# tranqkhue/bugcar_image_segmentation

Measured on AMD Instinct MI355X. Metric: frames/sec ENet 640x480 segmentation -> BEV occupancy grid (synthetic), whole job, higher is better.
Workload: dtype fp32; 1 GPU; config3/5: ENet 640x480 batch 64 per GPU, preprocess + forward + argmax/LUT + fused BEV warp/occgrid (1000x1000 BEV -> 200x200 cells); global_batch=64, per_gpu_batch=64, height=480, width=640, parallelism=frame-sharded dp1, streams_per_gpu=1, hip_graph=True, ranks=1, devices=1, backend=none (one process)

## Files before the change

### bugcar_image_segmentation_amd/_native.py

```python
from __future__ import annotations

import ctypes
import os
import threading
from pathlib import Path

import torch

_PKG = Path(__file__).resolve().parent
LIB_PATH = Path(os.environ.get("BUGSEG_LIB", _PKG / "libbugseg.so"))

OK, EINVAL, ENOMEM, EHIP, EFORMAT, ESTATE = 0, -1, -2, -3, -4, -5
FP32, BF16, F16 = 0, 1, 2
OUT_LOGITS_F32, OUT_CLASS15_U8, OUT_CLASS3_U8, OUT_BINARY_U8 = 0, 1, 2, 3
PRE_ENGINE, PRE_NCHW_F64, PRE_NCHW_F32, PRE_BGR_U8 = 0, 1, 2, 3

EXPORTED = ("bugseg_version", "bugseg_create", "bugseg_destroy", "bugseg_load_weights", "bugseg_num_classes",
            "bugseg_input_bytes", "bugseg_preprocess", "bugseg_nchw_to_input", "bugseg_enet_forward",
            "bugseg_enet_forward_bgr", "bugseg_enet_forward_bgr_ops",
            "bugseg_bev_occgrid", "bugseg_bev_workspace_bytes", "bugseg_bev_occgrid_ws", "bugseg_plan_info", "bugseg_plan_op", "bugseg_plan_launch_op",
            "bugseg_last_error",
            "bugseg_dl_create", "bugseg_dl_destroy", "bugseg_dl_load_weights", "bugseg_dl_set_plan",
            "bugseg_dl_forward", "bugseg_dl_launch_op", "bugseg_dl_read_buffer", "bugseg_dl_last_error",
            "bugseg_debug_parse_pack", "bugseg_debug_polar_tables", "bugseg_debug_ctx_info", "bugseg_debug_tile_walk", "bugseg_debug_set_spans", "bugseg_debug_pool_indices",
            "bugseg_dl_debug_check_plan")
DL_OP_FIELDS = 32


class BevParams(ctypes.Structure):
    _fields_ = [("M", ctypes.c_double * 9), ("in_rows", ctypes.c_int), ("in_cols", ctypes.c_int),
                ("warp_w", ctypes.c_int), ("warp_h", ctypes.c_int), ("occ_w_px", ctypes.c_int),
                ("occ_h_px", ctypes.c_int), ("occ_w", ctypes.c_int), ("occ_h", ctypes.c_int),
                ("left_x", ctypes.c_int), ("top_y", ctypes.c_int), ("ros_layout", ctypes.c_int),
                ("variant", ctypes.c_int), ("laserscan", ctypes.c_int)]


class BugsegError(RuntimeError):
    def __init__(self, code: int, msg: str):
        super().__init__(f"bugseg error {code}: {msg}")
        self.code = code


_lib = None
_lock = threading.Lock()


def load_library(path: Path | str | None = None) -> ctypes.CDLL:
    global _lib
    with _lock:
        if _lib is not None:
            return _lib
        p = Path(path) if path else LIB_PATH
        if not p.exists():
            raise FileNotFoundError(f"{p} not found: build it with `python -m bugcar_image_segmentation_amd.build` "
                                    "(or __graft_entry__.build())")
        lib = ctypes.CDLL(str(p))
        vp, i, sz, cp = ctypes.c_void_p, ctypes.c_int, ctypes.c_size_t, ctypes.c_char_p
        proto = {
            "bugseg_version": (i, []),
            "bugseg_create": (i, [i, i, ctypes.POINTER(vp)]),
            "bugseg_destroy": (i, [vp]),
            "bugseg_load_weights": (i, [vp, vp, sz]),
            "bugseg_num_classes": (i, [vp]),
            "bugseg_input_bytes": (sz, [vp, i, i, i]),
            "bugseg_preprocess": (i, [vp, vp, i, i, i, i, i, i, vp, vp]),
            "bugseg_nchw_to_input": (i, [vp, vp, i, i, i, i, vp, vp]),
            "bugseg_enet_forward": (i, [vp, vp, i, i, i, i, vp, vp]),
            "bugseg_enet_forward_bgr": (i, [vp, vp, i, i, i, i, vp, vp]),
            "bugseg_enet_forward_bgr_ops": (i, [vp, vp, i, i, i, i, vp, i, i, vp]),
            "bugseg_bev_occgrid": (i, [vp, vp, i, ctypes.POINTER(BevParams), vp, vp]),
            "bugseg_bev_workspace_bytes": (sz, [ctypes.POINTER(BevParams), i]),
            "bugseg_bev_occgrid_ws": (i, [vp, vp, i, ctypes.POINTER(BevParams), vp, vp, sz, vp]),
            "bugseg_plan_info": (i, [vp, i, i, i, i, i, ctypes.POINTER(i), ctypes.POINTER(ctypes.c_double),
                                     ctypes.POINTER(ctypes.c_double), ctypes.POINTER(ctypes.c_double)]),
            "bugseg_plan_op": (i, [vp, i, i, i, i, cp, i, ctypes.POINTER(ctypes.c_double),
                                   ctypes.POINTER(ctypes.c_double), ctypes.POINTER(ctypes.c_double)]),
            "bugseg_plan_launch_op": (i, [vp, i, i, i, i, vp]),
            "bugseg_last_error": (cp, [vp]),
            "bugseg_dl_create": (i, [i, i, ctypes.POINTER(vp)]),
            "bugseg_dl_destroy": (i, [vp]),
            "bugseg_dl_load_weights": (i, [vp, vp, sz]),
            "bugseg_dl_set_plan": (i, [vp, vp, i, vp, i, i, i, i]),
            "bugseg_dl_forward": (i, [vp, vp, i, i, i, vp, vp]),
            "bugseg_dl_launch_op": (i, [vp, i, vp]),
            "bugseg_dl_read_buffer": (i, [vp, i, vp, sz, vp]),
            "bugseg_dl_last_error": (cp, [vp]),
            "bugseg_debug_parse_pack": (i, [vp, sz, i, ctypes.POINTER(i)]),
            "bugseg_debug_polar_tables": (i, [i, i, i, vp, sz, vp, sz, ctypes.POINTER(i), ctypes.POINTER(i)]),
            "bugseg_debug_ctx_info": (i, [vp, i, i]),
            "bugseg_debug_tile_walk": (i, [i, i, i, vp, sz, vp]),
            "bugseg_debug_set_spans": (i, [vp, vp, i]),
            "bugseg_debug_pool_indices": (i, [vp, i, i, i, i, vp, sz, ctypes.POINTER(ctypes.c_int), vp]),
            "bugseg_dl_debug_check_plan": (i, [vp, i, vp, i, i, i, i, i, sz]),
        }
        for name, (res, args) in proto.items():
            f = getattr(lib, name)
            f.restype = res
            f.argtypes = args
        _lib = lib
        return lib


def check(code: int, ctx=None) -> None:
    if code != OK:
        lib = load_library()
        msg = lib.bugseg_last_error(ctx).decode(errors="replace")
        if code == EINVAL:
            raise ValueError(msg)
        raise BugsegError(code, msg)


def tile_walk(ntiles: int, grid: int, rev: int) -> list[list[int]]:
    lib = load_library()
    per_max = (ntiles + 7) // 8
    seq = (ctypes.c_int32 * (grid * per_max))()
    count = (ctypes.c_int32 * grid)()
    per = lib.bugseg_debug_tile_walk(ntiles, grid, rev, seq, len(seq), count)
    if per < 0:
        check(per)
    return [list(seq[b * per:b * per + count[b]]) for b in range(grid)]


def require_gpu() -> None:
    if not torch.cuda.is_available():
        raise RuntimeError("bugseg needs a HIP GPU (MI355X / gfx950); none is visible — there is no CPU fallback")


def stream_handle(stream: torch.cuda.Stream | None = None) -> int:
    s = stream if stream is not None else torch.cuda.current_stream()
    return int(s.cuda_stream)


class Context:

    def __init__(self, device: int | None = None, precision: int = FP32):
        require_gpu()
        self.lib = load_library()
        self.device = torch.cuda.current_device() if device is None else int(device)
        self.precision = precision
        h = ctypes.c_void_p()
        check(self.lib.bugseg_create(self.device, precision, ctypes.byref(h)))
        self.h = h

    def close(self) -> None:
        if getattr(self, "h", None) and self.h.value:
            self.lib.bugseg_destroy(self.h)
            self.h = ctypes.c_void_p()

    def __del__(self):
        try:
            self.close()
        except Exception:
            pass

    def load_weights(self, blob: bytes) -> None:
        buf = ctypes.create_string_buffer(blob, len(blob))
        check(self.lib.bugseg_load_weights(self.h, buf, len(blob)), self.h)

    @property
    def num_classes(self) -> int:
        return int(self.lib.bugseg_num_classes(self.h))

    def input_bytes(self, B: int, H: int, W: int) -> int:
        return int(self.lib.bugseg_input_bytes(self.h, B, H, W))

    def preprocess(self, bgr, B, H0, W0, H, W, layout, out, stream=None):
        check(self.lib.bugseg_preprocess(self.h, bgr.data_ptr(), B, H0, W0, H, W, layout, out.data_ptr(),
                                         stream_handle(stream)), self.h)

    def nchw_to_input(self, x, B, H, W, out, stream=None):
        check(self.lib.bugseg_nchw_to_input(self.h, x.data_ptr(), int(x.dtype == torch.float64), B, H, W,
                                            out.data_ptr(), stream_handle(stream)), self.h)

    def forward(self, x, B, H, W, out_kind, out, stream=None):
        check(self.lib.bugseg_enet_forward(self.h, x.data_ptr(), B, H, W, out_kind, out.data_ptr(),
                                           stream_handle(stream)), self.h)

    def forward_bgr(self, bgr, B, H, W, out_kind, out, stream=None):
        check(self.lib.bugseg_enet_forward_bgr(self.h, bgr.data_ptr(), B, H, W, out_kind, out.data_ptr(),
                                               stream_handle(stream)), self.h)

    def forward_bgr_ops(self, bgr, B, H, W, out_kind, out, first_op, last_op, stream=None):
        check(self.lib.bugseg_enet_forward_bgr_ops(self.h, bgr.data_ptr(), B, H, W, out_kind, out.data_ptr(),
                                                   first_op, last_op, stream_handle(stream)), self.h)

    def bev(self, seg, B, params: BevParams, out, stream=None):
        st = stream if stream is not None else torch.cuda.current_stream(seg.device)
        nws = int(self.lib.bugseg_bev_workspace_bytes(ctypes.byref(params), B))
        ws = None
        if nws:
            with torch.cuda.stream(st):
                ws = torch.empty(nws, dtype=torch.uint8, device=seg.device)
        check(self.lib.bugseg_bev_occgrid_ws(self.h, seg.data_ptr(), B, ctypes.byref(params), out.data_ptr(),
                                             0 if ws is None else ws.data_ptr(), nws, stream_handle(st)), self.h)

    def plan_info(self, B, H, W, out_kind, bgr_input=False):
        n = ctypes.c_int()
        lb = ctypes.c_double()
        pb = ctypes.c_double()
        fl = ctypes.c_double()
        check(self.lib.bugseg_plan_info(self.h, B, H, W, out_kind, int(bool(bgr_input)), ctypes.byref(n),
                                        ctypes.byref(lb), ctypes.byref(pb), ctypes.byref(fl)), self.h)
        return n.value, lb.value, pb.value, fl.value

    def plan_op(self, B, H, W, op):
        buf = ctypes.create_string_buffer(64)
        lb, pb, fl = ctypes.c_double(), ctypes.c_double(), ctypes.c_double()
        check(self.lib.bugseg_plan_op(self.h, B, H, W, op, buf, 64, ctypes.byref(lb), ctypes.byref(pb),
                                      ctypes.byref(fl)), self.h)
        return buf.value.decode(), lb.value, pb.value, fl.value

    def launch_op(self, B, H, W, op, stream=None):
        check(self.lib.bugseg_plan_launch_op(self.h, B, H, W, op, ctypes.c_void_p(stream_handle(stream))), self.h)

    def debug_info(self, what: int, arg: int = 0) -> int:
        return int(self.lib.bugseg_debug_ctx_info(self.h, what, arg))

    def set_spans(self, spans=None):
        if spans is None:
            check(self.lib.bugseg_debug_set_spans(self.h, ctypes.c_void_p(0), 0), self.h)
            return
        if not spans.is_cuda or spans.dtype != torch.int64 or not spans.is_contiguous() or spans.numel() % 512:
            raise ValueError("spans must be a contiguous CUDA int64 tensor of 512 words per op")
        check(self.lib.bugseg_debug_set_spans(self.h, ctypes.c_void_p(spans.data_ptr()), spans.numel() // 512), self.h)

    def pool_indices(self, B: int, H: int, W: int, block: int, shape: tuple, stream=None) -> torch.Tensor:
        out = torch.empty((B,) + tuple(shape), dtype=torch.uint8, device=torch.device("cuda", self.device))
        cs = ctypes.c_int(0)
        check(self.lib.bugseg_debug_pool_indices(self.h, B, H, W, block, ctypes.c_void_p(out.data_ptr()), out.numel(),
                                                 ctypes.byref(cs), ctypes.c_void_p(stream_handle(stream))), self.h)
        if cs.value != shape[-1]:
            raise ValueError(f"index tensor has channel stride {cs.value}, not {shape[-1]}")
        return out


_shared: dict[int, Context] = {}


def shared_context(device: int | None = None) -> Context:
    require_gpu()
    d = torch.cuda.current_device() if device is None else int(device)
    with _lock:
        c = _shared.get(d)
    if c is None:
        c = Context(d, FP32)
        with _lock:
            _shared.setdefault(d, c)
            c = _shared[d]
    return c


class DeepLabContext:

    def __init__(self, device: int | None = None, precision: int = BF16):
        require_gpu()
        self.lib = load_library()
        self.device = torch.cuda.current_device() if device is None else int(device)
        self.precision = precision
        h = ctypes.c_void_p()
        self._check(self.lib.bugseg_dl_create(self.device, precision, ctypes.byref(h)), None)
        self.h = h

    def _check(self, code, h):
        if code != OK:
            msg = self.lib.bugseg_dl_last_error(h).decode(errors="replace")
            if code == EINVAL:
                raise ValueError(msg)
# ... 36 lines not shown
```

### bugcar_image_segmentation_amd/csrc/bev_kernels.hip

```cpp
#include <cstdlib>
#include <type_traits>

#include "bugseg_internal.h"

namespace bugseg {

struct WarpTap { int sx, sy, ax, ay; bool x0, x1, y0, y1; };
__device__ __forceinline__ WarpTap warp_tap(const BevArgs &a, int x, int y) {
#pragma clang fp contract(off)
    const double *M = a.Mi;
    const int xb = (x / a.bw0) * a.bw0, x1 = x - xb;
    const double X0 = M[0] * (double)xb + M[1] * (double)y + M[2];
    const double Y0 = M[3] * (double)xb + M[4] * (double)y + M[5];
    const double W0 = M[6] * (double)xb + M[7] * (double)y + M[8];
    double W = W0 + M[6] * (double)x1;
    W = W != 0.0 ? 32.0 / W : 0.0;
    double fX = (X0 + M[0] * (double)x1) * W;
    double fY = (Y0 + M[3] * (double)x1) * W;
    fX = fmin(fmax(fX, -2147483648.0), 2147483647.0);
    fY = fmin(fmax(fY, -2147483648.0), 2147483647.0);
    const int X = (int)__builtin_rint(fX), Y = (int)__builtin_rint(fY);
    int sx = X >> 5, sy = Y >> 5;
    sx = sx < -32768 ? -32768 : (sx > 32767 ? 32767 : sx);
    sy = sy < -32768 ? -32768 : (sy > 32767 ? 32767 : sy);
// ... 250 lines not shown
    auto fetch = [&](int b) {
        const auto r = frame_rsrc(b);
#pragma unroll
        for (int i = 0; i < BEV_PF; ++i) pf[i] = __builtin_bit_cast(uint4, __builtin_amdgcn_raw_buffer_load_b128(r, (int)goff[i], 0, 0));
    };
    const int b0 = grp * fg;
    if (lds) {
        fetch(b0);
        for (int i = tid; i < 2 * bw + 16; i += 256) box[zpad + i] = 0;
    }
    const uint32_t inner = 0x739C0u;
    int tx = 0, ty = 0;
    cell_pixel(a, cx, cy, tx, ty);
    uint32_t wins[9];
#pragma unroll
    for (int qy = -1; qy <= 1; ++qy)
#pragma unroll
        for (int qx = -1; qx <= 1; ++qx) {
            const bool inside = (unsigned)(tx + qx) < (unsigned)a.occ_w_px && (unsigned)(ty + qy) < (unsigned)a.occ_h_px;
            const int sh = qy * 5 + qx;
            wins[(qy + 1) * 3 + qx + 1] = inside ? (sh >= 0 ? inner << sh : inner >> -sh) : 0xffffffffu;
        }
    for (int fi = 0; fi < fg; ++fi) {
        const int b = b0 + fi;
        if (b >= a.B) break;
        uint32_t msk = 0;
        int v = 0;
        if (lds) {
            __syncthreads();
#pragma unroll
            for (int i = 0; i < BEV_PF; ++i)
                if (tid + 256 * i < nch)
                    *reinterpret_cast<uint4 *>(box + 16 * (tid + 256 * i)) =
                        goff[i] == 0x80000000u ? make_uint4(0u, 0u, 0u, 0u)
                                               : make_uint4(inc4(pf[i].x), inc4(pf[i].y), inc4(pf[i].z), inc4(pf[i].w));
            __syncthreads();
            if (fi + 1 < fg && b + 1 < a.B) fetch(b + 1);
#pragma unroll 5
            for (int k = 0; k < BEV_WIN; ++k) {
                const uint32_t e = ek[k];
                const uint8_t *p = box + (e & 0xffffu);
                const uint32_t l0 = p[0], l1 = p[1], l2 = p[bw], l3 = p[bw + 1];
                const uint32_t ax = (e >> 16) & 31u, ay = (e >> 21) & 31u;
                const uint32_t wx = 32u + ax * 65535u, wy = 32u + ay * 65535u;
                const uint32_t top = dot2(l0 | l1 << 16, wx, 0u), bot = dot2(l2 | l3 << 16, wx, 0u);
                const int t = (int)(dot2(top | bot << 16, wy, 512u) >> 10);
                if (k == 0) v = t;
                msk |= (uint32_t)occupied(a, t) << BEV_ORDER[k];
            }
        } else {
            const auto seg = frame_rsrc(b);
#pragma unroll 1
            for (int k = 0; k < BEV_WIN; ++k) {
                const uint2 e = cell_ok ? ent(k) : make_uint2(0u, TAB_OUT);
                const int t = tab_value(seg, a.in_cols, e);
                if (k == 0) v = t;
                msk |= (uint32_t)occupied(a, t) << BEV_ORDER[k];
            }
        }
        if (!cell_ok) continue;
        msk |= outm;
        if (occupied(a, v)) {
            bool opened = false;
#pragma unroll
            for (int q = 0; q < 9; ++q) opened |= (msk & wins[q]) == wins[q];
            if (!opened) v = 2;
        }
        bev_emit(a, b, rem, cx, cy, cells, v);
    }
}

constexpr int BEV_BAND_CAP = 16384, BEV_BAND_PF = BEV_BAND_CAP / 16 / 256;
static_assert(BEV_BOXREC == 1 + BEV_BAND, "band record: header + one box per row part");
#ifndef BEV_MINP
#define BEV_MINP 1
#endif
constexpr int BEV_WL = 448;
static_assert(BEV_WL <= 2 * 256, "a thread takes at most two work-list records");

__global__ void __launch_bounds__(256) bev_bandbox_kernel(const BevArgs a, int4 *bbox) {
    __shared__ int red[BEV_BAND][4];
    __shared__ int4 pbox[BEV_BAND];
    __shared__ int np_rpp[2];
    const long cells = (long)a.occ_h * a.occ_w;
    const int band = blockIdx.x, r0 = band * BEV_BAND, r1 = min(a.occ_h, r0 + BEV_BAND);
    const int nr = r1 - r0, n = nr * a.occ_w;
    int ylo[BEV_BAND], yhi[BEV_BAND], xlo[BEV_BAND], xhi[BEV_BAND];
#pragma unroll
    for (int k = 0; k < BEV_BAND; ++k) { ylo[k] = xlo[k] = 1 << 30; yhi[k] = xhi[k] = -(1 << 30); }
    for (int i = threadIdx.x; i < n * BEV_WIN; i += 256) {
        const int c = i / BEV_WIN, k = i - c * BEV_WIN, ri = c / a.occ_w;
        const long rem = (long)r0 * a.occ_w + c;
        const uint2 e = slot_half(a.wtab[(long)(k >> 1) * cells + rem], k & 1);
        const uint32_t v = (e.y >> 10) & 15;
        const int sy = tap_sy(e), sx = tap_sx(e);
        int y_lo = 1 << 30, y_hi = -(1 << 30), x_lo = 1 << 30, x_hi = -(1 << 30);
        if (v & 3) { y_lo = min(y_lo, sy); y_hi = max(y_hi, sy); }
        if (v & 12) { y_lo = min(y_lo, sy + 1); y_hi = max(y_hi, sy + 1); }
        if (v & 5) { x_lo = min(x_lo, sx); x_hi = max(x_hi, sx); }
        if (v & 10) { x_lo = min(x_lo, sx + 1); x_hi = max(x_hi, sx + 1); }
#pragma unroll
        for (int q = 0; q < BEV_BAND; ++q)
            if (q == ri) { ylo[q] = min(ylo[q], y_lo); yhi[q] = max(yhi[q], y_hi); xlo[q] = min(xlo[q], x_lo); xhi[q] = max(xhi[q], x_hi); }
    }
    if (threadIdx.x < 4 * BEV_BAND) red[threadIdx.x >> 2][threadIdx.x & 3] = threadIdx.x & 1 ? -(1 << 30) : (1 << 30);
    __syncthreads();
#pragma unroll
    for (int q = 0; q < BEV_BAND; ++q) {
        atomicMin(&red[q][0], ylo[q]); atomicMax(&red[q][1], yhi[q]); atomicMin(&red[q][2], xlo[q]); atomicMax(&red[q][3], xhi[q]);
    }
    __syncthreads();
    if (threadIdx.x == 0) {
        auto boxof = [&](int q0, int q1) {
            int yl = 1 << 30, yh = -(1 << 30), xl = 1 << 30, xh = -(1 << 30);
            for (int q = q0; q < q1 && q < nr; ++q) {
                yl = min(yl, red[q][0]); yh = max(yh, red[q][1]); xl = min(xl, red[q][2]); xh = max(xh, red[q][3]);
            }
            int4 bx = make_int4(0, 0, 0, 16);
            if (yh >= yl) {
                const int y0 = yl - 1, bh = yh - yl + 3;
                const int xa = (xl - 1) & ~15, bw = ((xh + 17) & ~15) - xa;
                bx = make_int4(y0, xa, (long)bh * bw + 2 * bw + 16 <= BEV_BAND_CAP ? bh : -1, bw);
            }
            return bx;
        };
        int P = BEV_MINP;
        for (; P < BEV_BAND; P *= 2) {
            bool fit = true;
            for (int k = 0; k < P; ++k) fit = fit && boxof(k * (BEV_BAND / P), (k + 1) * (BEV_BAND / P)).z >= 0;
            if (fit) break;
        }
        int rpp = BEV_BAND / P;
        for (int k = 0; k < BEV_BAND; ++k) pbox[k] = k < P ? boxof(k * rpp, (k + 1) * rpp) : make_int4(0, 0, 0, 16);
        bool fit = true;
        for (int k = 0; k < P; ++k) fit = fit && pbox[k].z >= 0;
        if (!fit) {
            P = 1; rpp = BEV_BAND;
            pbox[0] = boxof(0, BEV_BAND);
            pbox[0].z = -1;
        }
        np_rpp[0] = P; np_rpp[1] = rpp;
        bbox[(size_t)band * BEV_BOXREC] = make_int4(P, rpp, 0, 0);
        for (int k = 0; k < BEV_BAND; ++k) bbox[(size_t)band * BEV_BOXREC + 1 + k] = pbox[k];
    }
    __syncthreads();
    const int rpp = np_rpp[1];
    uint32_t *ctab = reinterpret_cast<uint32_t *>(reinterpret_cast<unsigned char *>(a.wtab) + bev_ctab_offset(a.occ_w, a.occ_h));
    for (int i = threadIdx.x; i < n * BEV_SLOTS; i += 256) {
        const int c = i / BEV_SLOTS, q = i - c * BEV_SLOTS;
        const int4 bx = pbox[(c / a.occ_w) / rpp];
        if (bx.z < 0) continue;
        const long rem = (long)r0 * a.occ_w + c;
        uint4 *sp = a.wtab + (long)q * cells + rem;
        uint4 sv = *sp;
        auto put = [&](uint32_t x, uint32_t &y) {
            const uint2 e = make_uint2(x, y);
            const bool any = ((y >> 10) & 15) != 0;
            const int o = any ? (tap_sy(e) - bx.x) * bx.w + (tap_sx(e) - bx.y) : bx.z * bx.w;
            y = (y & 0x7fffu) | (uint32_t)o << 15;
        };
        put(sv.x, sv.y);
        put(sv.z, sv.w);
        *sp = sv;
        ctab[(long)(2 * q) * cells + rem] = sv.y;
        if (2 * q + 1 < BEV_WIN) ctab[(long)(2 * q + 1) * cells + rem] = sv.w;
    }
    __syncthreads();
    uint32_t *omask = ctab + (size_t)BEV_WIN * cells;
    for (int c = threadIdx.x; c < n; c += 256) {
        if (pbox[(c / a.occ_w) / rpp].z < 0) continue;
        const long rem = (long)r0 * a.occ_w + c;
        uint32_t m = 0;
        for (int k = 0; k < BEV_WIN; ++k)
            m |= (uint32_t)((ctab[(long)k * cells + rem] & TAB_OUT) != 0) << BEV_ORDER[k];
        omask[rem] = m;
    }
}

#ifndef BEV_ABL
#define BEV_ABL 0
#endif
__device__ __forceinline__ int bev_value_lds(const uint8_t *box, int bw, uint32_t ey) {
    const uint8_t *p = box + (ey >> 15);
    const uint32_t l0 = p[0], l1 = p[1], l2 = p[bw], l3 = p[bw + 1];
    const uint32_t ax = ey & 31u, ay = (ey >> 5) & 31u;
    const uint32_t wx = 32u + ax * 65535u, wy = 32u + ay * 65535u;
    const uint32_t top = dot2(l0 | l1 << 16, wx, 0u), bot = dot2(l2 | l3 << 16, wx, 0u);
    return (int)(dot2(top | bot << 16, wy, 512u) >> 10);
}
constexpr uint32_t BEV_INNER = 0x739C0u;
__device__ __forceinline__ bool bev_cell_pass1(const BevArgs &a, const uint8_t *box, int bw, const uint32_t (&e9)[9],
                                               uint32_t outm, int &v, uint32_t &m, uint32_t &cand) {
    int t9[9];
#pragma unroll
    for (int i = 0; i < 9; ++i) t9[i] = bev_value_lds(box, bw, e9[i]);
    v = t9[0];
    m = outm;
#pragma unroll
    for (int i = 0; i < 9; ++i) m |= (uint32_t)occupied(a, t9[i]) << BEV_ORDER[i];
    cand = 0;
    if (!(occupied(a, v) && (m & BEV_INNER) != BEV_INNER)) return true;
#pragma unroll
    for (int qi = 0; qi < 9; ++qi) {
        if (qi == 4) continue;
        const int qx = qi % 3 - 1, qy = qi / 3 - 1, sh = qy * 5 + qx;
        const uint32_t win = sh >= 0 ? BEV_INNER << sh : BEV_INNER >> -sh, wi = win & BEV_INNER;
        cand |= (!((outm >> B5(qx, qy)) & 1u) && (m & wi) == wi) ? 1u << qi : 0u;
    }
    if (cand == 0) { v = 2; return true; }
    return false;
}
__device__ __forceinline__ int bev_cell_pass2(const BevArgs &a, const uint8_t *box, int bw, int v, uint32_t m,
                                              uint32_t cand, uint32_t outm, const uint32_t *ring, long cells) {
    if constexpr (BEV_ABL & 1) return v;
    uint32_t rneed = 0;
#pragma unroll
    for (int qi = 0; qi < 9; ++qi) {
        const int qx = qi % 3 - 1, qy = qi / 3 - 1, sh = qy * 5 + qx;
        const uint32_t win = sh >= 0 ? BEV_INNER << sh : BEV_INNER >> -sh;
        rneed |= ((cand >> qi) & 1u) ? win & ~BEV_INNER & ~outm : 0u;
    }
    uint32_t er[BEV_WIN - 9];
#pragma unroll
    for (int k = 0; k < BEV_WIN - 9; ++k) er[k] = ring[(long)k * cells];
#pragma unroll
// ... 389 lines not shown
```

### bugcar_image_segmentation_amd/csrc/bneck_kernels.hip

```cpp
#include <algorithm>
#include <cstdlib>

#include <type_traits>

#include "bugseg_internal.h"
#ifndef BUGSEG_OUT_AUX
#define BUGSEG_OUT_AUX -1
#endif
#include "cls_common.h"

namespace bugseg {

#ifdef BUGSEG_STAMPS
__device__ unsigned long long *bugseg_stamps;
#define STAMP(k) do { if (tid == 0 && bugseg_stamps) bugseg_stamps[(size_t)tile * 8 + (k)] = __builtin_amdgcn_s_memtime(); } while (0)
#define STAMP_WG() do { if (tid == 0 && bugseg_stamps) bugseg_stamps[(size_t)tile * 8 + 7] = blockIdx.x; } while (0)
#define STAMP_ENTRY(k) do { if (threadIdx.x == 0 && bugseg_stamps) bugseg_stamps[(1u << 19) + 2u * blockIdx.x + (k)] = __builtin_amdgcn_s_memrealtime(); } while (0)
#else
#define STAMP_ENTRY(k) do {} while (0)
#define STAMP(k) do {} while (0)
#define STAMP_WG() do {} while (0)
#endif

__device__ __forceinline__ void vm_wait_upto(int n) {
// ... 368 lines not shown
    bool cshort[2] = {false, false};
    if constexpr (CLS) {
        const T *cw = reinterpret_cast<const T *>(a.cw);
        for (int q = tid; q < 512; q += NT) {
            const int bs = q >> 6, ln = q & 63;
            const T *src = cw + (size_t)cls_prow(bs >> 2, ln & 31) * 64 + (bs & 3) * 16 + 8 * (ln >> 5);
            if constexpr (sizeof(T) == 4) {
                cwl[q] = reinterpret_cast<const uint4 *>(src)[0];
                cwl[512 + q] = reinterpret_cast<const uint4 *>(src)[1];
            } else {
                cwl[q] = *reinterpret_cast<const uint4 *>(src);
            }
        }
        if (tid < 64) cbl[tid] = (tid & 15) < a.ncls ? a.cbias[tid] : -INFINITY;
        lut64 = cls_lut64(a.lut);
#pragma unroll
        for (int b = 0; b < 2; ++b) {
            CRaw w2_, w3_;
            const T *r = cw + (size_t)cls_prow(b, lane & 31) * 64 + 8 * (lane >> 5);
            ld8(w2_, r + 32);
            ld8(w3_, r + 48);
            cshort[b] = __ballot(nonzero(w2_) || nonzero(w3_)) == 0;
        }
    }
    const auto rxb = mkbuf(DN ? a.xin : a.x, DN ? a.xin_bytes : a.x_bytes);
    const auto rob = mkbuf(a.out, a.x_bytes);
    const auto rpb = mkbuf(a.pool, a.pool_bytes);
    const auto rib = mkbuf(a.idx_out, a.idx_bytes);
    auto act = [&](float4 v, const float *s) { return prelu4m(v, ld4f(s)); };
    const int dt = a.dt;
    constexpr bool tr = TR && !ASYM;

    constexpr bool F32 = sizeof(T) == 4;
    BneckRange rg0;
    if constexpr (F32 && SCL) rg0 = bneck_range<ASYM>(a.rg, rng_reduce(rlane));
    bool scl = rg0.scl;
    float xm = rg0.xm, b1m = rg0.b1m, o1m = rg0.o1m, b2m = rg0.b2m, o2m = rg0.o2m, b2bm = rg0.b2bm, o2bm = rg0.o2bm;
    float b3m = rg0.b3m, o3m = rg0.o3m;
    const int rs1 = rg0.rs1, re2b = rg0.re2b;
    float amo = 0.f;
    auto proj_mfma = [&](f32x4 (&acc)[NR1], const Raw (&xs)[KS1]) {
#pragma unroll
        for (int r = 0; r < NR1; ++r) acc[r] = bias4(cb1 + r * 16 + kq * 4);
        if constexpr (F32 && SCL) {
#pragma unroll
            for (int r = 0; r < NR1; ++r) acc[r] = mul4(acc[r], b1m);
#pragma unroll
            for (int s = 0; s < KS1; ++s) {
                const RawF xq = scale8(reinterpret_cast<const RawF &>(xs[s]), xm);
#pragma unroll
                for (int r = 0; r < NR1; ++r) {
                    WRaw wf;
                    ldw(wf, w1 + (r * 16 + col) * K1S + s * 32);
                    mma(acc[r], wf, xq);
                }
            }
#pragma unroll
            for (int r = 0; r < NR1; ++r) acc[r] = mul4(acc[r], o1m);
        } else {
#pragma unroll
            for (int s = 0; s < KS1; ++s)
#pragma unroll
                for (int r = 0; r < NR1; ++r) {
                    WRaw wf;
                    ldw(wf, w1 + (r * 16 + col) * K1S + s * 32);
                    mma(acc[r], wf, xs[s]);
                }
        }
    };

    const int G = gridDim.x, grp = blockIdx.x & 7, slot = blockIdx.x >> 3, nslots = G >> 3;
    const int CH = tile_walk_ch(a.ntiles);
    constexpr bool WALK1 = sizeof(T) == 4 && C == 128;
    const int lim = tile_walk_lim(grp, CH, a.ntiles);
    const int wword = WALK1 ? tile_walk_base(grp, CH, a.ntiles, a.rev) : tile_walk_mirror(grp, CH, a.ntiles, a.rev);
    auto tile_geom = [&](int tile, int &n, int &oy0, int &ox0) {
        int t = tile;
        const int txi = t % a.tiles_x; t /= a.tiles_x;
        const int tyi = t % a.tiles_y; t /= a.tiles_y;
        const int ph = t % a.phases;
        n = t / a.phases;
        const int py = RD ? ph : ph / dt, px = RD ? 0 : ph - py * dt;
        oy0 = py + dt * tyi * (tr ? TW : TH) - (CLS ? tyi : 0);
        ox0 = RD ? 0 : px + dt * txi * (tr ? TH : TW) - (CLS ? txi : 0);
    };
    Raw kx[KEEP ? NF2 : 1][KS1];
    bool kok[KEEP ? NF2 : 1];
#ifndef BNECK_PREF
#define BNECK_PREF 0
#endif
    constexpr bool PREF = BNECK_PREF && KEEP && REG3 && !DN;
    bool pref = false;
    for (int it = slot; it < (WALK1 ? lim : CH); it += nslots) {
        int tile;
        if constexpr (WALK1) {
            tile = tile_walk_at(wword, it);
        } else {
            tile = grp * CH + it;
            if (tile >= a.ntiles) break;
            tile = tile_walk_flip(wword, tile);
        }
        int n, oy0, ox0;
        tile_geom(tile, n, oy0, ox0);
        float tmo = 0.f;
        const bool has_next = PREF && it + nslots < lim;
        const int ntile = !has_next ? -1 : WALK1 ? tile_walk_at(wword, it + nslots) : tile_walk_flip(wword, grp * CH + it + nslots);
        int nn = 0, noy0 = 0, nox0 = 0;
        if (has_next) tile_geom(ntile, nn, noy0, nox0);
        const int dtx = RD ? 1 : dt;
        const uint32_t xn = (uint32_t)(n * a.H * a.W) * (uint32_t)(C * sizeof(T));
        const uint32_t xin_n = (uint32_t)(n * 4 * a.H * a.W) * (uint32_t)(CI * sizeof(T));
        auto pix_off = [&](int f, int pi, int choff) -> uint32_t {
            const int i = (f * 16) / TW, j = (f * 16) % TW + pi;
            const int y = oy0 + dt * (tr ? j : i), x = ox0 + dtx * (tr ? i : j);
            const bool ok = y < a.H && x < a.W;
            uint32_t v = xn + ((__umul24((uint32_t)y, (uint32_t)a.W) + (uint32_t)x) * C + choff) * (uint32_t)sizeof(T);
            asm volatile("" : "+v"(v));
            return ok ? v : OOB;
        };
        auto pix_base = [&](int f, int pi) -> uint32_t { return pix_off(f, pi, 0); };
        const auto rrb = DN ? rpb : rxb;
        const uint32_t pn = (uint32_t)(n * a.H * a.W) * (uint32_t)(CI * sizeof(T));
        auto res_off = [&](int f, int pi, int ch) -> uint32_t {
            if constexpr (!DN) {
                return pix_off(f, pi, ch);
            } else {
                const int i = (f * 16) / TW, j = (f * 16) % TW + pi;
                const int y = oy0 + dt * i, x = ox0 + dtx * j;
                const bool ok = y < a.H && x < a.W && ch < CI;
                uint32_t v = pn + ((__umul24((uint32_t)y, (uint32_t)a.W) + (uint32_t)x) * CI + ch) * (uint32_t)sizeof(T);
                asm volatile("" : "+v"(v));
                return ok ? v : OOB;
            }
        };
        auto pool_store = [&](const Raw (&xs)[KS1], bool interior, int y, int x, uint4 (&pk)[NPK * PKW]) {
            if constexpr (DN) {
                if (__ballot(interior) == 0) return;
                auto elems = [&](const Raw &r, float (&e)[8]) {
                    if constexpr (sizeof(T) == 2) {
                        const float4 lo = unpack4<T>((u32x2_t){r.v.x, r.v.y}), hi = unpack4<T>((u32x2_t){r.v.z, r.v.w});
                        e[0] = lo.x; e[1] = lo.y; e[2] = lo.z; e[3] = lo.w; e[4] = hi.x; e[5] = hi.y; e[6] = hi.z; e[7] = hi.w;
                    } else {
                        const RawF &f = reinterpret_cast<const RawF &>(r);
                        e[0] = f.a.x; e[1] = f.a.y; e[2] = f.a.z; e[3] = f.a.w; e[4] = f.b.x; e[5] = f.b.y; e[6] = f.b.z; e[7] = f.b.w;
                    }
                };
                const uint32_t pix = (uint32_t)((n * a.H + y) * a.W + x);
                auto emit = [&](int cc, const float (&bv)[8], const int (&bp)[8], bool wr, int kslot, bool kval) {
                    uint32_t pw[8 * sizeof(T) / 4];
                    if constexpr (sizeof(T) == 2) {
                        const u32x2_t lo = pack4<T>(make_float4(bv[0], bv[1], bv[2], bv[3]));
                        const u32x2_t hi = pack4<T>(make_float4(bv[4], bv[5], bv[6], bv[7]));
                        pw[0] = lo.x; pw[1] = lo.y; pw[2] = hi.x; pw[3] = hi.y;
                    } else {
#pragma unroll
                        for (int i = 0; i < 8; ++i) pw[i] = __float_as_uint(bv[i]);
                    }
                    uint32_t lo = 0, hi = 0;
#pragma unroll
                    for (int i = 0; i < 4; ++i) {
                        lo |= (uint32_t)(bp[i] & 3) << (8 * i);
                        hi |= (uint32_t)(bp[4 + i] & 3) << (8 * i);
                    }
                    if constexpr (DKEEP) {
                        pk[kslot * PKW] = kval ? make_uint4(pw[0], pw[1], pw[2], pw[3]) : make_uint4(0u, 0u, 0u, 0u);
                        if constexpr (PKW == 2)
// ... 986 lines not shown
```

### bugcar_image_segmentation_amd/csrc/bugseg_internal.h

```cpp
#pragma once
#include <hip/hip_runtime.h>
#include <stdint.h>
#include <stddef.h>

namespace bugseg {

enum Epi {
    EPI_PLAIN = 0,
    EPI_RESADD = 1,
    EPI_RESPOOL = 2,
    EPI_RESUNPOOL = 3,
    EPI_INIT = 4,
    EPI_SHUFFLE = 5,
    EPI_CLASSES = 6,
    EPI_INIT_BGR = 7,
    EPI_COUNT = 8
};

enum Prec { PREC_F32 = 0, PREC_BF16 = 1, PREC_F16 = 2 };
inline constexpr int prec_es(int prec) { return prec == PREC_F32 ? 4 : 2; }

constexpr int RNG_SLOTS = 256;
struct RangeArgs {
    const float *amax_in;
    float *amax_out;
    float amax_static;
    int sw[4];
    float n[3], c[3];
    int off;
};
int range_weight_exp(double m);
hipError_t launch_amax(const float *x, size_t n, float *slots, hipStream_t s);

struct ConvArgs {
    const void *in;
    int B, Hin, Win, CinS;
    int Hg, Wg;
    int stride;
    int M;
    int Ksteps, Kpad, Npad;
    const void *w;
    const int *gtab;
    const float *bias, *slope1, *slope2, *pscale;
    int cconv, cpool, pool_k;
    const void *res;
    int resH, resW, resC, resCS;
    const uint8_t *idx_in;
    uint8_t *idx_out;
    int idxCS;
    void *out;
    int Hout, Wout, outC;
    int coutP;
    int ncls;
    const uint8_t *lut;
    int lut_kind;
    uint8_t *cls_out;
    float *logits_out;
    const double *nlut;
    float naff[6];
    int naff_on;
    int pool_scan;
    int ntiles;
    int rev;
    int stg_elems;
    int stage_ok;
    uint32_t mHWg, mWg; int sHWg, sWg;
    uint32_t in_bytes, out_bytes, res_bytes, idx_bytes;
    int cpr_sh;
    int slopes_le1;
    RangeArgs rg;
    unsigned long long *span;
};

__host__ __device__ inline int tile_walk_ch(int ntiles) { return (ntiles + 7) >> 3; }
__host__ __device__ inline int tile_walk_lim(int grp, int CH, int ntiles) {
    const int rest = ntiles - grp * CH;
    return rest < CH ? rest : CH;
}
__host__ __device__ inline int tile_walk_base(int grp, int CH, int ntiles, int rev) {
    return rev ? ~(grp * CH + tile_walk_lim(grp, CH, ntiles)) : grp * CH;
}
__host__ __device__ inline int tile_walk_at(int base, int it) {
    const int s = base >> 31;
    return (base ^ s) + (it ^ s);
}
__host__ __device__ inline int tile_walk(int grp, int it, int CH, int ntiles, int rev) {
    if (it >= tile_walk_lim(grp, CH, ntiles)) return -1;
    return tile_walk_at(tile_walk_base(grp, CH, ntiles, rev), it);
}
__host__ __device__ inline int tile_walk_mirror(int grp, int CH, int ntiles, int rev) {
    return rev ? 2 * grp * CH + tile_walk_lim(grp, CH, ntiles) - 1 : -1;
}
__host__ __device__ inline int tile_walk_flip(int mirror, int t) { return mirror < 0 ? t : mirror - t; }

void fastdiv(uint32_t d, uint32_t &m, int &s);

int device_cus();
int occupancy_per_cu(const void *f, int threads, size_t lds);
hipError_t allow_dynamic_lds(const void *f);

hipError_t launch_conv(int prec, int nr, int epi, const ConvArgs &a, hipStream_t s);
int conv_tile_pixels(int nr);
size_t conv_lds_bytes(int prec, const ConvArgs &a);

bool cls_supported(const ConvArgs &a);
hipError_t launch_cls(int prec, const ConvArgs &a, hipStream_t s);

hipError_t launch_init(int prec, bool bgr, const ConvArgs &a, hipStream_t s);
constexpr int NAFF_R = 64;
hipError_t launch_naff_search(int prec, const double *nlut, const float *base, uint8_t *ok, hipStream_t s);

struct BneckArgs {
    const void *x;
    void *out;
    int B, H, W;
    int dt, phases;
    int tr;
    int tiles_x, tiles_y, ntiles;
    int rev;
    const void *w1, *w2, *w2b, *w3;
    const float *b1, *s1, *b2, *s2, *b2b, *s2b, *b3, *s3, *s_out;
    uint32_t x_bytes;
    int slopes_le1;
    const void *xin;
    void *pool;
    uint8_t *idx_out;
    int idxCS;
    uint32_t xin_bytes, pool_bytes, idx_bytes;
    RangeArgs rg;
    unsigned long long *span;
    const void *cw;
    const float *cbias;
    uint8_t *cls_out;
    uint32_t cls_bytes;
    const uint8_t *lut;
    int lut_kind, ncls, csw;
};
int bneck_variants(int C);
bool bneck_keeps_c64(int prec, int v);
void bneck_shape(int C, int v, int &th, int &tw, int &nw, int *rd = nullptr);
size_t bneck_lds_bytes(int prec, int C, bool asym, int v, int cin = 0, bool cls = false);
int bneck_slots_per_cu(int prec, int C, bool asym, int v, bool tr, int cin = 0);
hipError_t launch_bneck(int prec, int C, bool asym, int v, const BneckArgs &a, hipStream_t s, int cin = 0);
hipError_t launch_bneck_cls(int prec, const BneckArgs &a, hipStream_t s);
constexpr int BNECK2_V = 5;
size_t bneck2_lds_bytes();
int bneck2_slots_per_cu();
hipError_t launch_bneck2(const BneckArgs &a, hipStream_t s);

struct UpArgs {
    const void *x;
    const uint8_t *idx;
    void *out;
    int M, h, w, idxCS;
    int rev;
    uint32_t mHW, mW; int sHW, sW;
    const void *w1, *w2, *w3;
    const float *b1, *s1, *b2, *s2, *b3, *s3, *s_out;
    uint32_t x_bytes, idx_bytes, out_bytes;
    int slopes_le1;
    RangeArgs rg;
    unsigned long long *span;
};
bool up_supported(int cin, int it, int cout);
hipError_t launch_up(int prec, int cin, int it, int cout, const UpArgs &a, hipStream_t s);

struct PreArgs {
    const uint8_t *bgr;
    int B, H0, W0, H, W;
    int mode;
    const int *xofs;
    const short *xa;
    const int *yofs;
    const short *yb;
    int vec_end;
    const double *lut;
    int out_layout;
    int prec;
    void *out;
};
hipError_t launch_preprocess(const PreArgs &a, hipStream_t s);

struct NchwArgs {
    const void *x; int is_f64; int B, H, W; int prec; void *out;
};
hipError_t launch_nchw_to_input(const NchwArgs &a, hipStream_t s);

struct BevArgs {
    const uint8_t *seg;
    int B, in_rows, in_cols;
    double Mi[9];
    int bw0;
    int warp_w, warp_h, occ_w_px, occ_h_px, occ_w, occ_h, left_x, top_y;
    double ifx, ify;
    int ros_layout;
    int variant;
    int8_t *out;
    int laserscan;
    uint8_t *cells;
    const int32_t *fmap;
    const int32_t *imap;
    int pw, ph;
    int32_t *rmin;
    int hit;
    uint4 *wtab;
    int nitems;
};
hipError_t launch_bev(const BevArgs &a, hipStream_t s);
hipError_t launch_bev_table(const BevArgs &a, hipStream_t s);
size_t bev_table_bytes(int occ_w, int occ_h);

constexpr int BEV_BAND = 4;
__host__ __device__ inline int bev_bands(int occ_h) { return (occ_h + BEV_BAND - 1) / BEV_BAND; }
constexpr int BEV_WIN = 25, BEV_SLOTS = 13;
constexpr int BEV_BOXREC = 5;
__host__ __device__ inline size_t bev_records_offset(int occ_w, int occ_h) { return (size_t)occ_w * occ_h * BEV_SLOTS * 16; }
__host__ __device__ inline size_t bev_ctab_offset(int occ_w, int occ_h) {
    return (bev_records_offset(occ_w, occ_h) + (size_t)bev_bands(occ_h) * BEV_BOXREC * 16 + 255) & ~(size_t)255;
}
__host__ __device__ inline size_t bev_items_offset(int occ_w, int occ_h) {
    return (bev_ctab_offset(occ_w, occ_h) + (size_t)occ_w * occ_h * (BEV_WIN + 1) * 4 + 255) & ~(size_t)255;
}

}
```

### bugcar_image_segmentation_amd/csrc/bugseg_runtime.cpp

```cpp
#include <cmath>
#include <cstdio>
#include <cstring>
#include <string>
#include <vector>
#include <algorithm>
#include <cstdlib>
#include <mutex>

#include "bugseg_internal.h"
#include "../../include/bugseg.h"

using namespace bugseg;

namespace {
std::mutex g_occ_mu;
struct OccKey { int dev; const void *f; int threads; size_t lds; int val; };
std::vector<OccKey> g_occ;
int current_device() {
    int d = 0;
    return hipGetDevice(&d) == hipSuccess ? d : 0;
}
}
int bugseg::device_cus() {
    const int dev = current_device();
// ... 6 lines not shown
    return n;
}
int bugseg::occupancy_per_cu(const void *f, int threads, size_t lds) {
    const int dev = current_device();
    std::lock_guard<std::mutex> lk(g_occ_mu);
    for (const OccKey &k : g_occ)
        if (k.dev == dev && k.f == f && k.threads == threads && k.lds == lds) return k.val;
    int n = 0;
    if (hipOccupancyMaxActiveBlocksPerMultiprocessor(&n, f, threads, lds) != hipSuccess || n < 0) n = 0;
    g_occ.push_back({dev, f, threads, lds, n});
    return n;
}
hipError_t bugseg::allow_dynamic_lds(const void *f) {
    const int dev = current_device();
    std::lock_guard<std::mutex> lk(g_occ_mu);
    for (const OccKey &k : g_occ)
        if (k.dev == dev && k.f == f && k.threads == -1) return hipSuccess;
    hipError_t e = hipFuncSetAttribute(f, hipFuncAttributeMaxDynamicSharedMemorySize, 160 * 1024);
    if (e == hipSuccess) g_occ.push_back({dev, f, -1, 0, 1});
    return e;
}

int bugseg::range_weight_exp(double m) {
    if (!(m > 0) || !std::isfinite(m)) return 0;
    int e = 0;
    (void)std::frexp(m, &e);
    const int l = e - 1;
    if (l >= -2 && l < 15) return 0;
    return std::max(-40, std::min(40, 14 - l));
}

namespace {

thread_local std::string g_thread_err;

struct UnitDesc {
    int kind = 0, cout = 0, cin = 0, kh = 0, kw = 0, stride = 1, pad_h = 0, pad_w = 0, dil_h = 1, dil_w = 1, out_pad = 0;
    float eps = 0.f;
    std::vector<float> w, b, gamma, beta, mean, var, slope;
};

struct BlockDesc {
    int type = 0;
    int attrs[8] = {0};
    std::vector<UnitDesc> units;
    std::vector<std::vector<float>> extra;
};

enum { BT_INITIAL = 1, BT_REGULAR = 2, BT_DOWN = 3, BT_UP = 4, BT_FULLCONV = 5 };

struct Packed {
    int Npad = 0, Kpad = 0, Ksteps = 0, nr = 0;
    int CinS = 0;
    int stride = 1;
    int cout = 0;
    int coutP = 0;
    int phases = 1;
    double macs_per_px = 0;
    size_t o_w = 0, o_gtab = 0, o_bias = 0, o_s1 = 0, o_s2 = 0, o_ps = 0;
    int sw = 0;
    std::vector<float> rabs, rbias, rslope;
};

struct Op {
    int kind = 0;
    ConvArgs a;
    int nr = 0, epi = 0;
    BneckArgs bn;
    UpArgs up;
    int up_cin = 0, up_it = 0, up_cout = 0;
    int bn_c = 0, bn_var = 0, bn_cin = 0;
    bool bn_asym = false;
    double bytes = 0, flops = 0;
    double layer_bytes = -1;
    int launches = 1;
    int pos = 0;
    Op() {
        std::memset(&a, 0, sizeof(a));
        std::memset(&bn, 0, sizeof(bn));
        std::memset(&up, 0, sizeof(up));
    }
};

struct Plan {
    int B = 0, H = 0, W = 0;
    std::vector<Op> ops;
    float *words = nullptr;
    size_t words_bytes = 0;
    void *arena = nullptr;
    size_t arena_bytes = 0;
    bool pinned = false;
    std::vector<unsigned char *> idx;
    std::vector<size_t> idx_bytes;
    bool cls_ok = false, cls_on = false;
    int tile_order = 0;
};

#ifndef BUGSEG_TILE_ORDER_DEFAULT
#define BUGSEG_TILE_ORDER_DEFAULT 1
#endif

inline int round_up(int v, int m) { return (v + m - 1) / m * m; }
inline int pow2_nr(int npad) {
    int nr = npad / 16;
    int p = 1;
    while (p < nr) p <<= 1;
    return p;
}

}

struct bugseg_ctx {
    int device = 0;
    int prec = PREC_F32;
    float naff[6] = {};
    bool naff_on = false;
    float norm_amax = 0.f;
    bool range_off = false;
    unsigned long long *spans = nullptr;
    int spans_ops = 0;
    std::string err;
    bool loaded = false;
    int ncls = 0;
    std::vector<BlockDesc> blocks;
    std::vector<Packed> packed;
    std::vector<std::vector<int>> block_convs;
    std::vector<unsigned char> host_w;
    void *dev_w = nullptr;
    void *dev_luts = nullptr;
    Plan plan;
    struct PreTab { int key[4] = {0, 0, 0, 0}; void *tab = nullptr; bool pinned = false; };
    std::vector<PreTab> pre_tabs;
    hipStream_t setup = nullptr;
    struct PolarTab { int key[3] = {0, 0, -1}; int pw = 0, ph = 0; void *tab = nullptr; bool pinned = false; };
    std::vector<PolarTab> polar_tabs;
    struct LsScratch { void *stream = nullptr; void *p = nullptr; size_t bytes = 0; uint64_t used = 0; bool pinned = false; };
    std::vector<LsScratch> ls_scratch;
    uint64_t use_clock = 0;
    struct BevTab { std::vector<unsigned char> key; uint4 *tab = nullptr; bool pinned = false; int nitems = 0; };
    std::vector<BevTab> bev_tabs;
    std::vector<void *> graveyard;
};

namespace {

int fail(bugseg_ctx *c, int code, const std::string &m) {
    if (c) c->err = m;
    else g_thread_err = m;
    return code;
}

bool stream_capturing(void *stream) {
    hipStreamCaptureStatus st = hipStreamCaptureStatusNone;
    if (hipStreamIsCapturing((hipStream_t)stream, &st) != hipSuccess) return true;
    return st != hipStreamCaptureStatusNone;
}

struct RelaxCapture {
    hipStreamCaptureMode m = hipStreamCaptureModeRelaxed;
    RelaxCapture() { (void)hipThreadExchangeStreamCaptureMode(&m); }
    ~RelaxCapture() { (void)hipThreadExchangeStreamCaptureMode(&m); }
};

hipStream_t setup_stream(bugseg_ctx *c) {
    if (!c->setup && hipStreamCreateWithFlags(&c->setup, hipStreamNonBlocking) != hipSuccess) c->setup = nullptr;
    return c->setup;
}

void retire(bugseg_ctx *c, void *p, bool capturing) {
    if (!p) return;
    if (capturing) { c->graveyard.push_back(p); return; }
    (void)hipDeviceSynchronize();
    (void)hipFree(p);
}

struct DeviceGuard {
    int prev = -1;
    explicit DeviceGuard(int dev) {
        if (hipGetDevice(&prev) != hipSuccess) prev = -1;
        if (prev != dev) (void)hipSetDevice(dev);
    }
    ~DeviceGuard() {
        int cur = -1;
        if (prev >= 0 && hipGetDevice(&cur) == hipSuccess && cur != prev) (void)hipSetDevice(prev);
    }
};

struct Reader {
    const unsigned char *p, *end;
    bool ok = true;
    template <typename T> T get() {
        T v{};
        if (p + sizeof(T) > end) { ok = false; return v; }
        std::memcpy(&v, p, sizeof(T));
        p += sizeof(T);
        return v;
    }
    std::vector<float> tensor() {
        uint32_t n = get<uint32_t>();
        std::vector<float> v;
        if (!ok || (size_t)(end - p) / 4 < (size_t)n) { ok = false; return v; }
        v.resize(n);
        if (n) std::memcpy(v.data(), p, (size_t)n * 4);
        p += (size_t)n * 4;
        return v;
    }
};

bool parse_blob(const void *blob, size_t bytes, std::vector<BlockDesc> &out, int &ncls, std::string &why) {
    Reader r{(const unsigned char *)blob, (const unsigned char *)blob + bytes};
    char magic[4];
    for (int i = 0; i < 4; ++i) magic[i] = r.get<char>();
    if (!r.ok || std::memcmp(magic, "BSG1", 4) != 0) { why = "bad magic (expected BSG1)"; return false; }
    uint32_t ver = r.get<uint32_t>(), nb = r.get<uint32_t>(), nc = r.get<uint32_t>();
    if (!r.ok || ver != 1) { why = "unsupported blob version"; return false; }
    if (nb == 0 || nb > 4096 || nc == 0 || nc > 16) { why = "bad block/class count"; return false; }
    ncls = (int)nc;
    for (uint32_t b = 0; b < nb; ++b) {
        BlockDesc bd;
        bd.type = (int)r.get<uint32_t>();
        for (int i = 0; i < 8; ++i) bd.attrs[i] = r.get<int32_t>();
        uint32_t nu = r.get<uint32_t>();
// ... 682 lines not shown
                        const Packed &p1 = P(0), &p2 = P(1), &p3 = P(nu - 1), &p2b = P(nu == 4 ? 2 : 1);
                        q.x = curp; q.out = dst; q.B = B; q.H = cur.H; q.W = cur.W;
                        q.dt = dd; q.phases = trd ? dd : dd * dd; q.tr = ttr;
                        q.tiles_y = ty; q.tiles_x = tx;
                        q.ntiles = B * q.phases * ty * tx;
                        q.w1 = dw + p1.o_w; q.b1 = (const float *)(dw + p1.o_bias); q.s1 = (const float *)(dw + p1.o_s1);
                        q.w2 = dw + p2.o_w; q.b2 = (const float *)(dw + p2.o_bias); q.s2 = (const float *)(dw + p2.o_s1);
                        q.w2b = dw + p2b.o_w; q.b2b = (const float *)(dw + p2b.o_bias); q.s2b = (const float *)(dw + p2b.o_s1);
                        q.w3 = dw + p3.o_w; q.b3 = (const float *)(dw + p3.o_bias); q.s3 = (const float *)(dw + p3.o_s1);
                        q.s_out = (const float *)(dw + p3.o_s2);
                        q.rg.amax_in = words_of(curp);
                        q.rg.off = ctx->range_off;
                        q.rg.sw[0] = p1.sw; q.rg.sw[1] = p2.sw; q.rg.sw[2] = p2b.sw; q.rg.sw[3] = p3.sw;
                        row_bound(p1, 0, p1.cout, q.rg.n[0], q.rg.c[0]);
                        row_bound(p2, 0, p2.cout, q.rg.n[1], q.rg.c[1]);
                        row_bound(p2b, 0, p2b.cout, q.rg.n[2], q.rg.c[2]);
                        q.rg.amax_out = take_words();
                        wrote(dst, q.rg.amax_out);
                        q.slopes_le1 = 1;
                        const std::pair<size_t, int> slopes[] = {{p1.o_s1, p1.Npad}, {p2.o_s1, p2.Npad}, {p2b.o_s1, p2b.Npad},
                                                                 {p3.o_s1, p3.Npad}, {p3.o_s2, p3.Npad}};
                        for (const auto &sv : slopes) {
                            const float *sl = (const float *)(ctx->host_w.data() + sv.first);
                            for (int c = 0; c < sv.second; ++c)
                                if (!(sl[c] <= 1.f)) q.slopes_le1 = 0;
                        }
                        double fl = 0, wb = 0, lb = 0;
                        const double px = (double)B * cur.H * cur.W;
                        for (int i = 0; i < nu; ++i) {
                            fl += 2.0 * P(i).macs_per_px * px;
                            wb += (double)P(i).Npad * P(i).Kpad * es;
                            lb += px * (cstore(b.units[i].cin) + cstore(b.units[i].cout)) * es;
                        }
                        op.flops = fl;
                        op.bytes = 2.0 * px * cur.C * es + wb;
                        op.layer_bytes = lb + px * cur.C * es + wb;
                        ops.push_back(op);
                    }
                    break;
                }
                for (int i = 0; i < nu; ++i) {
                    const UnitDesc &u = b.units[i];
                    const bool last = i + 1 == nu;
                    Shape so{s.H, s.W, cstore(u.cout)};
                    unsigned char *o = last ? dst : T[i % 3];
                    if (!last) szT = std::max(szT, tbytes(so));
                    else szX = std::max(szX, tbytes(so));
                    if (fill) {
                        Op op;
                        conv(P(i), last ? EPI_RESADD : EPI_PLAIN, src, s, so, o, so, op);
                        if (last) {
                            op.a.res = curp; op.a.resH = cur.H; op.a.resW = cur.W; op.a.resC = b.attrs[0]; op.a.resCS = cur.C;
                            op.bytes += (double)B * cur.H * cur.W * cur.C * es;
                        }
                        ops.push_back(op);
                    }
                    s = so;
                    src = o;
                }
                cur = s;
                break;
            }
            case BT_UP: {
                const int ref = b.attrs[2];
                Shape sm{cur.H, cur.W, cstore(P(0).cout)}, s1{cur.H, cur.W, cstore(P(1).cout)};
                Shape st{cur.H * 2, cur.W * 2, cstore(P(2).cout)}, so{cur.H * 2, cur.W * 2, cstore(P(3).cout)};
                szM = std::max(szM, tbytes(sm));
                szT = std::max({szT, tbytes(s1), tbytes(st)});
                szX = std::max(szX, tbytes(so));
                const int cin_b = b.attrs[0], cout_b = b.attrs[1], it_b = P(1).cout;
                const char *nf = std::getenv("BUGSEG_NO_FUSE");
                const bool fuse_up = ids.size() >= 5 && up_supported(cin_b, it_b, cout_b) && cur.C == cin_b &&
                                     so.C == cout_b && !(nf && *nf && *nf != '0');
                if (fuse_up) {
                    if (fill) {
                        Op op;
                        op.kind = 2;
                        op.up_cin = cin_b; op.up_it = it_b; op.up_cout = cout_b;
                        UpArgs &q = op.up;
                        const unsigned char *dw = (const unsigned char *)ctx->dev_w;
                        const Packed &p1 = P(4), &p2 = P(2), &p3 = P(3);
                        q.x = curp; q.idx = idx[ref]; q.out = dst;
                        q.M = B * cur.H * cur.W; q.h = cur.H; q.w = cur.W;
                        q.idxCS = cstore(ctx->blocks[ref].attrs[0]);
                        fastdiv((uint32_t)(cur.H * cur.W), q.mHW, q.sHW);
                        fastdiv((uint32_t)cur.W, q.mW, q.sW);
                        q.w1 = dw + p1.o_w; q.b1 = (const float *)(dw + p1.o_bias); q.s1 = (const float *)(dw + p1.o_s1);
                        q.w2 = dw + p2.o_w; q.b2 = (const float *)(dw + p2.o_bias); q.s2 = (const float *)(dw + p2.o_s1);
                        q.w3 = dw + p3.o_w; q.b3 = (const float *)(dw + p3.o_bias); q.s3 = (const float *)(dw + p3.o_s1);
                        q.s_out = (const float *)(dw + p3.o_s2);
                        q.rg.amax_in = words_of(curp);
                        q.rg.off = ctx->range_off;
                        q.rg.sw[0] = p1.sw; q.rg.sw[1] = p2.sw; q.rg.sw[2] = p3.sw;
                        row_bound(p1, cout_b, cout_b + it_b, q.rg.n[0], q.rg.c[0]);
                        row_bound(p2, 0, p2.Npad, q.rg.n[1], q.rg.c[1]);
                        q.rg.amax_out = take_words();
                        wrote(dst, q.rg.amax_out);
                        q.x_bytes = (uint32_t)std::min<size_t>((size_t)B * cur.H * cur.W * cur.C * es, 0x7fffffff);
                        q.idx_bytes = (uint32_t)std::min<size_t>((size_t)B * cur.H * cur.W * q.idxCS, 0x7fffffff);
                        q.out_bytes = (uint32_t)std::min<size_t>((size_t)B * so.H * so.W * so.C * es, 0x7fffffff);
                        q.slopes_le1 = 1;
                        const std::pair<size_t, int> sl[] = {{p1.o_s1, p1.Npad}, {p2.o_s1, p2.Npad}, {p3.o_s1, p3.Npad},
                                                             {p3.o_s2, p3.Npad}};
                        for (const auto &v : sl) {
                            const float *f = (const float *)(ctx->host_w.data() + v.first);
                            for (int c = 0; c < v.second; ++c)
                                if (!(f[c] <= 1.f)) q.slopes_le1 = 0;
                        }
                        const double px = (double)B * cur.H * cur.W;
                        double wb = 0, fl = 0;
                        for (int i = 0; i < 4; ++i) { wb += (double)P(i).Npad * P(i).Kpad * es; fl += 2.0 * P(i).macs_per_px * px; }
                        op.flops = fl;
                        op.bytes = px * cur.C * es + px * q.idxCS + 4.0 * px * so.C * es + wb;
                        op.layer_bytes = px * cur.C * es * 2 + px * (sm.C + s1.C) * es + px * s1.C * es + 4.0 * px * st.C * es * 2 +
                                         px * sm.C * es + px * q.idxCS + 4.0 * px * so.C * es + wb;
                        ops.push_back(op);
                    }
                    cur = so;
                    break;
                }
                const bool pair = ids.size() == 6;
                Shape sp{cur.H, cur.W, pair ? sm.C + s1.C : sm.C};
                szM = std::max(szM, tbytes(sp));
                if (fill && pair) {
                    Op om1, ot, o2;
                    conv(P(4), EPI_PLAIN, curp, cur, sp, Mb, sp, om1);
                    conv(P(5), EPI_SHUFFLE, Mb, sp, sp, T[1], st, ot);
                    ot.bytes -= (double)B * sp.H * sp.W * sm.C * es;
                    conv(P(3), EPI_RESUNPOOL, T[1], st, so, dst, so, o2);
                    o2.a.res = Mb; o2.a.resH = sp.H; o2.a.resW = sp.W; o2.a.resC = b.attrs[1]; o2.a.resCS = sp.C;
                    o2.a.idx_in = idx[ref]; o2.a.idxCS = cstore(ctx->blocks[ref].attrs[0]);
                    o2.bytes += (double)B * sm.H * sm.W * sm.C * es + (double)B * sm.H * sm.W * o2.a.idxCS;
                    ops.push_back(om1); ops.push_back(ot); ops.push_back(o2);
                } else if (fill) {
                    Op om, o1, ot, o2;
                    conv(P(0), EPI_PLAIN, curp, cur, sm, Mb, sm, om);
                    conv(P(1), EPI_PLAIN, curp, cur, s1, T[0], s1, o1);
                    conv(P(2), EPI_SHUFFLE, T[0], s1, s1, T[1], st, ot);
                    conv(P(3), EPI_RESUNPOOL, T[1], st, so, dst, so, o2);
                    o2.a.res = Mb; o2.a.resH = sm.H; o2.a.resW = sm.W; o2.a.resC = b.attrs[1]; o2.a.resCS = sm.C;
                    o2.a.idx_in = idx[ref]; o2.a.idxCS = cstore(ctx->blocks[ref].attrs[0]);
                    o2.bytes += (double)B * sm.H * sm.W * sm.C * es + (double)B * sm.H * sm.W * o2.a.idxCS;
                    ops.push_back(om); ops.push_back(o1); ops.push_back(ot); ops.push_back(o2);
                }
                cur = so;
                break;
            }
            case BT_FULLCONV: {
                Shape so{cur.H * 2, cur.W * 2, P(0).cout};
                if (so.H != H || so.W != W) { why = "network does not return to the input resolution"; return false; }
                if (fill) {
                    Op op;
                    conv(P(0), EPI_CLASSES, curp, cur, cur, nullptr, so, op);
                    op.a.ncls = ctx->ncls;
                    ops.push_back(op);
                }
                cur = so;
                break;
            }
            }
            if (b.type != BT_FULLCONV) {
                curp = dst;
                xi ^= 1;
            }
        }
        return true;
    }
};

bool finish_conv_args(ConvArgs &a, int epi, size_t es) {
    fastdiv((uint32_t)(a.Hg * a.Wg), a.mHWg, a.sHWg);
    fastdiv((uint32_t)a.Wg, a.mWg, a.sWg);
    const double in_b = (double)a.B * a.Hin * a.Win * a.CinS * es;
    const double out_b = epi == EPI_CLASSES ? 0.0 : (double)a.B * a.Hout * a.Wout * a.outC * es;
    const double res_b = a.res ? (double)a.B * a.resH * a.resW * a.resCS * es : 0.0;
    const double idx_b = a.idx_out ? (double)a.M * a.idxCS : a.idx_in ? (double)a.B * a.resH * a.resW * a.idxCS : 0.0;
    const double lim = 2147483648.0;
    if (in_b >= lim || out_b >= lim || res_b >= lim || idx_b >= lim ||
        (epi == EPI_CLASSES && (double)a.B * a.Hout * a.Wout * a.ncls * 4.0 >= 4.0 * lim))
        return false;
    a.in_bytes = (uint32_t)in_b; a.out_bytes = (uint32_t)out_b;
    a.res_bytes = (uint32_t)res_b; a.idx_bytes = (uint32_t)idx_b;
    const int epc = 16 / (int)es, cpr = a.outC / epc;
    a.cpr_sh = -1;
    if (a.outC % epc == 0 && cpr > 0 && (cpr & (cpr - 1)) == 0)
        for (a.cpr_sh = 0; (1 << a.cpr_sh) < cpr; ++a.cpr_sh) {}
    a.stage_ok = a.cpr_sh >= 0 && (epi != EPI_SHUFFLE || (a.Wg % 16 == 0 && a.M % 16 == 0));
    return true;
}

bool build_plan(bugseg_ctx *ctx, int B, int H, int W, std::string &why, void *stream = nullptr) {
    Plan &pl = ctx->plan;
    if (pl.arena && pl.B == B && pl.H == H && pl.W == W) return true;
    Walker w{ctx, B, H, W};
    if (!w.run(false, why)) return false;
    auto al = [](size_t v) { return (v + 4095) / 4096 * 4096; };
    size_t total = 2 * al(w.szX) + 3 * al(w.szT) + al(w.szM);
    for (size_t s : w.szIdx) total += al(s);
    const size_t words_bytes = ctx->prec == PREC_F32 ? (size_t)Walker::max_words(ctx->blocks.size()) * RNG_SLOTS * 4 : 0;
    total += al(words_bytes);
    const bool cap = stream_capturing(stream);
    RelaxCapture relax;
    if (pl.arena) {
        retire(ctx, pl.arena, cap || pl.pinned);
        pl.arena = nullptr;
        pl.pinned = false;
    }
    if (hipMalloc(&pl.arena, total) != hipSuccess) { why = "hipMalloc of the activation arena failed"; pl.arena = nullptr; return false; }
    unsigned char *p = (unsigned char *)pl.arena;
    w.X[0] = p; p += al(w.szX);
    w.X[1] = p; p += al(w.szX);
    for (int i = 0; i < 3; ++i) { w.T[i] = p; p += al(w.szT); }
    w.Mb = p; p += al(w.szM);
    w.idx.assign(w.szIdx.size(), nullptr);
    for (size_t i = 0; i < w.szIdx.size(); ++i) if (w.szIdx[i]) { w.idx[i] = p; p += al(w.szIdx[i]); }
    w.words = words_bytes ? (float *)p : nullptr;
    p += al(words_bytes);
    if (!w.run(true, why)) return false;
    if (words_bytes && w.nwords > Walker::max_words(ctx->blocks.size())) { why = "range words: plan too long"; return false; }
    for (Op &op : w.ops) {
        if (op.kind == 1) {
            const double bytes = (double)op.bn.B * op.bn.H * op.bn.W * op.bn_c * w.es;
            const double in_bytes = op.bn_cin ? 4.0 * op.bn.B * op.bn.H * op.bn.W * op.bn_cin * w.es : 0.0;
            if (bytes >= 2147483648.0 || in_bytes >= 2147483648.0) { why = "batch too large for 32-bit tensor offsets"; return false; }
            op.bn.x_bytes = (uint32_t)bytes;
            continue;
        }
        if (!finish_conv_args(op.a, op.epi, w.es)) { why = "batch too large for 32-bit tensor offsets"; return false; }
    }
    pl.ops = std::move(w.ops);
    int issued = 0;
    for (Op &op : pl.ops) { op.pos = issued; issued += op.launches; }
    pl.tile_order = BUGSEG_TILE_ORDER_DEFAULT;
    if (const char *to = std::getenv("BUGSEG_TILE_ORDER"))
        if (*to >= '0' && *to <= '2' && !to[1]) pl.tile_order = *to - '0';
    pl.cls_ok = false;
    pl.cls_on = false;
    if (pl.ops.size() >= 2) {
        const Op &l = pl.ops.back(), &q = pl.ops[pl.ops.size() - 2];
        const char *fe = std::getenv("BUGSEG_CLS_FUSE");
        pl.cls_ok = fe && *fe == '1' && l.kind == 0 && l.epi == EPI_CLASSES && cls_supported(l.a) &&
                    !std::getenv("BUGSEG_CLS_CONV") && q.kind == 1 && q.bn_c == 16 && !q.bn_asym && q.bn_cin == 0 &&
                    q.bn.dt == 1 && q.bn.phases == 1 && q.bn.out == l.a.in && l.a.B == q.bn.B && l.a.Hin == q.bn.H &&
                    l.a.Win == q.bn.W && (double)B * l.a.Hout * l.a.Wout < 2147483648.0;
    }
    pl.idx = w.idx;
    pl.idx_bytes = w.szIdx;
    pl.words = w.words;
    pl.words_bytes = words_bytes;
    pl.B = B; pl.H = H; pl.W = W;
    pl.arena_bytes = total;
    return true;
}

void linear_coeffs(int dsize, int ssize, double scale, int *ofs, short *a01) {
#pragma clang fp contract(off)
    for (int d = 0; d < dsize; ++d) {
        float f = (float)((d + 0.5) * scale - 0.5);
        int s = (int)std::floor(f);
        f -= (float)s;
        if (s < 0) { f = 0.f; s = 0; }
        if (s >= ssize - 1) { f = 0.f; s = ssize - 1; }
        ofs[d] = s;
        long v0 = std::lrintf((1.f - f) * 2048.f), v1 = std::lrintf(f * 2048.f);
        a01[2 * d] = (short)std::min(32767L, std::max(-32768L, v0));
        a01[2 * d + 1] = (short)std::min(32767L, std::max(-32768L, v1));
    }
}

}

extern "C" {

int bugseg_version(void) { return 100; }

const char *bugseg_last_error(const bugseg_ctx *ctx) { return ctx ? ctx->err.c_str() : g_thread_err.c_str(); }

int bugseg_create(int device, int precision, bugseg_ctx **out) {
    if (!out) return fail(nullptr, BUGSEG_EINVAL, "out is NULL");
    *out = nullptr;
    if (precision != BUGSEG_FP32 && precision != BUGSEG_BF16 && precision != BUGSEG_F16)
        return fail(nullptr, BUGSEG_EINVAL, "precision must be BUGSEG_FP32, BUGSEG_BF16 or BUGSEG_F16");
    int n = 0;
    if (hipGetDeviceCount(&n) != hipSuccess || device < 0 || device >= n)
        return fail(nullptr, BUGSEG_EINVAL, "no such HIP device: " + std::to_string(device));
    bugseg_ctx *c = new (std::nothrow) bugseg_ctx();
    if (!c) return fail(nullptr, BUGSEG_ENOMEM, "out of host memory");
    c->device = device;
    c->prec = precision == BUGSEG_BF16 ? PREC_BF16 : precision == BUGSEG_F16 ? PREC_F16 : PREC_F32;
    DeviceGuard g(device);
    unsigned char tab[32 + 3 * 256 * 8];
    const uint8_t lut3[16] = {1, 1, 0, 2, 2, 2, 2, 2, 2, 0, 2, 2, 2, 2, 2, 2};
    const uint8_t lutb[16] = {1, 1, 0, 0, 0, 0, 0, 0, 0, 0, 0, 0, 0, 0, 0, 0};
    std::memcpy(tab, lut3, 16);
    std::memcpy(tab + 16, lutb, 16);
    const double mean[3] = {0.485, 0.456, 0.406}, stdv[3] = {0.229, 0.224, 0.225};
    for (int ch = 0; ch < 3; ++ch)
        for (int v = 0; v < 256; ++v) {
            const double x = ((double)v / 256.0 - mean[ch]) / stdv[ch];
            std::memcpy(tab + 32 + (ch * 256 + v) * 8, &x, 8);
            c->norm_amax = std::max(c->norm_amax, (float)std::fabs(x) * 1.0001f);
        }

    {
        RelaxCapture relax;
        hipStream_t s = setup_stream(c);
        hipError_t e = s ? hipMalloc(&c->dev_luts, sizeof(tab)) : hipErrorInvalidValue;
        if (e == hipSuccess) e = hipMemcpyAsync(c->dev_luts, tab, sizeof(tab), hipMemcpyHostToDevice, s);
        if (e == hipSuccess) e = hipStreamSynchronize(s);
        if (e == hipSuccess && c->prec != PREC_F32) {
            float base[6];
            for (int ch = 0; ch < 3; ++ch) {
                base[ch] = (float)(1.0 / (256.0 * stdv[ch]));
                base[3 + ch] = (float)(-mean[ch] / stdv[ch]);
            }
            constexpr int N = 2 * NAFF_R + 1;
            std::vector<uint8_t> okh((size_t)3 * N * N);
            uint8_t *okd = nullptr;
            hipError_t e2 = hipMalloc(&okd, okh.size());
            if (e2 == hipSuccess) e2 = launch_naff_search(c->prec, (const double *)((const unsigned char *)c->dev_luts + 32), base, okd, s);
            if (e2 == hipSuccess) e2 = hipMemcpyAsync(okh.data(), okd, okh.size(), hipMemcpyDeviceToHost, s);
            if (e2 == hipSuccess) e2 = hipStreamSynchronize(s);
            if (okd) (void)hipFree(okd);
            bool all = e2 == hipSuccess;
            for (int ch = 0; ch < 3 && all; ++ch) {
                int best = -1, bestd = 1 << 30;
                for (int k = 0; k < N * N; ++k) {
                    const int da = k / N - NAFF_R, db = k % N - NAFF_R, d = std::max(std::abs(da), std::abs(db));
                    if (okh[(size_t)ch * N * N + k] && d < bestd) { best = k; bestd = d; }
                }
                if (best < 0) { all = false; break; }
                int32_t ia, ib;
                std::memcpy(&ia, &base[ch], 4);
                std::memcpy(&ib, &base[3 + ch], 4);
                ia += best / N - NAFF_R;
// ... 91 lines not shown
        const double eps = 2.220446049250313e-16;
        if (std::fabs(sx - isx) < eps && std::fabs(sy - isy) < eps && isx == 2 && isy == 2) {
            a.mode = 1;
        } else {
            a.mode = 2;
            const int key[4] = {H0, W0, H, W};
            const size_t need = (size_t)W * 4 + (size_t)W * 4 + (size_t)H * 4 + (size_t)H * 4;
            const bool cap = stream_capturing(stream);
            bugseg_ctx::PreTab *hit = nullptr;
            for (auto &t : ctx->pre_tabs)
                if (std::memcmp(t.key, key, sizeof(key)) == 0) hit = &t;
            if (!hit) {
                std::vector<unsigned char> h(need);
                int *xo = (int *)h.data();
                short *xa = (short *)(h.data() + (size_t)W * 4);
                int *yo = (int *)(h.data() + (size_t)W * 8);
                short *yb = (short *)(h.data() + (size_t)W * 8 + (size_t)H * 4);
                linear_coeffs(W, W0, sx, xo, xa);
                linear_coeffs(H, H0, sy, yo, yb);
                if (ctx->pre_tabs.size() >= 4) {
                    for (size_t i = 0; i < ctx->pre_tabs.size(); ++i)
                        if (!ctx->pre_tabs[i].pinned) {
                            retire(ctx, ctx->pre_tabs[i].tab, cap);
                            ctx->pre_tabs.erase(ctx->pre_tabs.begin() + (long)i);
                            break;
                        }
                }
                bugseg_ctx::PreTab t;
                std::memcpy(t.key, key, sizeof(key));
                RelaxCapture relax;
                hipStream_t st = setup_stream(ctx);
                hipError_t e = st ? hipMalloc(&t.tab, need) : hipErrorInvalidValue;
                if (e == hipSuccess) e = hipMemcpyAsync(t.tab, h.data(), need, hipMemcpyHostToDevice, st);
                if (e == hipSuccess) e = hipStreamSynchronize(st);
                if (e != hipSuccess) {
                    if (t.tab) (void)hipFree(t.tab);
                    return fail(ctx, BUGSEG_EHIP, std::string("resize table upload failed: ") + hipGetErrorString(e));
                }
                ctx->pre_tabs.push_back(t);
                hit = &ctx->pre_tabs.back();
            }
            if (cap) hit->pinned = true;
            unsigned char *t = (unsigned char *)hit->tab;
            a.xofs = (const int *)t;
            a.xa = (const short *)(t + (size_t)W * 4);
            a.yofs = (const int *)(t + (size_t)W * 8);
            a.yb = (const short *)(t + (size_t)W * 8 + (size_t)H * 4);
        }
    }
    hipError_t e = launch_preprocess(a, (hipStream_t)stream);
    if (e != hipSuccess) return fail(ctx, BUGSEG_EHIP, std::string("preprocess launch: ") + hipGetErrorString(e));
    return BUGSEG_OK;
}

int bugseg_nchw_to_input(bugseg_ctx *ctx, const void *x, int is_f64, int B, int H, int W, void *out, void *stream) {
    if (!ctx || !x || !out) return fail(ctx, BUGSEG_EINVAL, "NULL argument");
    if (B <= 0 || H <= 0 || W <= 0) return fail(ctx, BUGSEG_EINVAL, "bad shape");
    DeviceGuard g(ctx->device);
    NchwArgs a{x, is_f64 ? 1 : 0, B, H, W, ctx->prec, out};
    hipError_t e = launch_nchw_to_input(a, (hipStream_t)stream);
    if (e != hipSuccess) return fail(ctx, BUGSEG_EHIP, std::string("layout launch: ") + hipGetErrorString(e));
    return BUGSEG_OK;
}

static BneckArgs cls_fused_args(const Plan &pl) {
    const Op &q = pl.ops[pl.ops.size() - 2], &l = pl.ops.back();
    BneckArgs a = q.bn;
    a.rg.amax_out = nullptr;
    a.tr = 0;
    a.tiles_y = (a.H + 14) / 15;
    a.tiles_x = (a.W + 14) / 15;
    a.ntiles = a.B * a.tiles_y * a.tiles_x;
    a.cw = l.a.w;
    a.cbias = l.a.bias;
    a.cls_out = l.a.cls_out;
    a.cls_bytes = (uint32_t)((size_t)l.a.B * l.a.Hout * l.a.Wout);
    a.lut = l.a.lut;
    a.lut_kind = l.a.lut_kind;
    a.ncls = l.a.ncls;
    a.csw = l.a.rg.sw[0];
    return a;
}

static hipError_t launch_op(const bugseg_ctx *ctx, int i, hipStream_t s) {
    const Plan &pl = ctx->plan;
    const Op &o = pl.ops[(size_t)i];
    const int rev = pl.tile_order == 2 ? 1 : pl.tile_order == 1 ? (o.pos & 1) : 0;
    unsigned long long *sp = ctx->spans && i < ctx->spans_ops ? ctx->spans + 512 * (size_t)i : nullptr;
    if (pl.cls_on && i + 2 == (int)pl.ops.size()) { BneckArgs q = cls_fused_args(pl); q.span = sp; q.rev = rev; return launch_bneck_cls(ctx->prec, q, s); }
    if (pl.cls_on && i + 1 == (int)pl.ops.size()) return hipSuccess;
    if (o.kind == 1) { BneckArgs q = o.bn; q.span = sp; q.rev = rev; return launch_bneck(ctx->prec, o.bn_c, o.bn_asym, o.bn_var, q, s, o.bn_cin); }
    if (o.kind == 2) { UpArgs q = o.up; q.span = sp; q.rev = rev; return launch_up(ctx->prec, o.up_cin, o.up_it, o.up_cout, q, s); }
    ConvArgs q = o.a;
    q.span = sp;
    q.rev = rev;
    return launch_conv(ctx->prec, o.nr, o.epi, q, s);
}

static int enet_forward(bugseg_ctx *ctx, const void *in, bool bgr, int B, int H, int W, int out_kind, void *out,
                        void *stream, int first_op = 0, int last_op = -1) {
    if (!ctx || !in || !out) return fail(ctx, BUGSEG_EINVAL, "NULL argument");
    if (!ctx->loaded) return fail(ctx, BUGSEG_ESTATE, "no weights loaded");
    if (out_kind < BUGSEG_OUT_LOGITS_F32 || out_kind > BUGSEG_OUT_BINARY_U8) return fail(ctx, BUGSEG_EINVAL, "bad out_kind");
    DeviceGuard g(ctx->device);
    std::string why;
    if (!build_plan(ctx, B, H, W, why, stream)) return fail(ctx, BUGSEG_EINVAL, why);
    Plan &pl = ctx->plan;
    if (stream_capturing(stream)) pl.pinned = true;
    Op &first = pl.ops.front();
    first.a.in = in;
    first.epi = bgr ? EPI_INIT_BGR : EPI_INIT;
    first.a.nlut = bgr ? (const double *)((const unsigned char *)ctx->dev_luts + 32) : nullptr;
    first.a.naff_on = bgr && ctx->naff_on && !std::getenv("BUGSEG_INIT_TABLE");
    std::memcpy(first.a.naff, ctx->naff, sizeof(ctx->naff));
    first.a.rg.amax_in = bgr ? nullptr : pl.words;
    first.a.rg.amax_static = bgr ? ctx->norm_amax : 0.f;
    ConvArgs &last = pl.ops.back().a;
    last.cls_out = nullptr; last.logits_out = nullptr; last.lut = nullptr; last.lut_kind = 0;
    const uint8_t *luts = (const uint8_t *)ctx->dev_luts;
    switch (out_kind) {
    case BUGSEG_OUT_LOGITS_F32: last.logits_out = (float *)out; break;
    case BUGSEG_OUT_CLASS15_U8: last.cls_out = (uint8_t *)out; break;
    case BUGSEG_OUT_CLASS3_U8: last.cls_out = (uint8_t *)out; last.lut = luts; last.lut_kind = 1; break;
    case BUGSEG_OUT_BINARY_U8: last.cls_out = (uint8_t *)out; last.lut = luts + 16; last.lut_kind = 2; break;
    }
    const int nops = (int)pl.ops.size();
    if (last_op < 0 || last_op > nops) last_op = nops;
    if (first_op < 0 || first_op > last_op) return fail(ctx, BUGSEG_EINVAL, "bad op range");
    if (pl.words && first_op == 0) {
        hipError_t e = hipMemsetAsync(pl.words, 0, pl.words_bytes, (hipStream_t)stream);
        if (e == hipSuccess && !bgr) e = launch_amax((const float *)in, (size_t)B * H * W * 8, pl.words, (hipStream_t)stream);
        if (e != hipSuccess) return fail(ctx, BUGSEG_EHIP, std::string("range words: ") + hipGetErrorString(e));
    }
    pl.cls_on = pl.cls_ok && out_kind != BUGSEG_OUT_LOGITS_F32 && first_op <= nops - 2 && last_op == nops;
    for (int i = first_op; i < last_op; ++i) {
        hipError_t e = launch_op(ctx, i, (hipStream_t)stream);
        if (e != hipSuccess) return fail(ctx, BUGSEG_EHIP, "conv launch " + std::to_string(i) + ": " + hipGetErrorString(e));
    }
    return BUGSEG_OK;
}

int bugseg_enet_forward(bugseg_ctx *ctx, const void *in, int B, int H, int W, int out_kind, void *out, void *stream) {
    return enet_forward(ctx, in, false, B, H, W, out_kind, out, stream);
}

int bugseg_enet_forward_bgr(bugseg_ctx *ctx, const uint8_t *bgr, int B, int H, int W, int out_kind, void *out,
                            void *stream) {
    return enet_forward(ctx, bgr, true, B, H, W, out_kind, out, stream);
}

int bugseg_enet_forward_bgr_ops(bugseg_ctx *ctx, const uint8_t *bgr, int B, int H, int W, int out_kind, void *out,
                                int first_op, int last_op, void *stream) {
    return enet_forward(ctx, bgr, true, B, H, W, out_kind, out, stream, first_op, last_op);
}

}

namespace {

#pragma clang fp contract(off)
const float kAtanP1 = 0.9997878412794807f * (float)(180 / 3.1415926535897932384626433832795);
const float kAtanP3 = -0.3258083974640975f * (float)(180 / 3.1415926535897932384626433832795);
const float kAtanP5 = 0.1555786518463281f * (float)(180 / 3.1415926535897932384626433832795);
const float kAtanP7 = -0.04432655554792128f * (float)(180 / 3.1415926535897932384626433832795);

float fast_atan_rad(float y, float x) {
    const float ax = std::fabs(x), ay = std::fabs(y);
    const float c = std::min(ax, ay) / (std::max(ax, ay) + (float)2.220446049250313e-16);
    const float cc = c * c;
    float a = std::fma(std::fma(std::fma(cc, kAtanP7, kAtanP5), cc, kAtanP3), cc, kAtanP1) * c;
    if (!(ax >= ay)) a = 90.f - a;
    if (x < 0) a = 180.f - a;
    if (y < 0) a = 360.f - a;
    return a * (float)(3.1415926535897932384626433832795 / 180);
}

int round_short(float v) {
    const long r = std::lrint(v);
    return (int)(r < -32768 ? -32768 : r > 32767 ? 32767 : r);
}

void polar_tables(int pw, int ph, double max_radius, float cx, float cy, int w, int h, std::vector<int32_t> &fmap,
                  std::vector<int32_t> &imap) {
    const double CV_2PI = 6.283185307179586476925286766559;
    const double Kangle = CV_2PI / ph, Kmag = max_radius / pw;
    fmap.resize((size_t)pw * ph);
    for (int phi = 0; phi < ph; ++phi) {
        const double KKy = Kangle * phi, cp = std::cos(KKy), sp = std::sin(KKy);
        for (int rho = 0; rho < pw; ++rho) {
            const float r = (float)(rho * Kmag);
            const float mx = (float)(r * cp + (double)cx), my = (float)(r * sp + (double)cy);
            const int sx = round_short(mx), sy = round_short(my);
            fmap[(size_t)phi * pw + rho] = ((unsigned)sx < (unsigned)w && (unsigned)sy < (unsigned)h) ? (sx | (sy << 16)) : -1;
        }
    }
    imap.resize((size_t)w * h);
    for (int y = 0; y < h; ++y)
        for (int x = 0; x < w; ++x) {
            const float bx = (float)x - cx, by = (float)y - cy;
            const float mag = std::sqrt(std::fma(bx, bx, by * by));
            const float ang = fast_atan_rad(by, bx);
            const double rho = mag / Kmag, phi = ang / Kangle;
            const float mx = (float)rho, my = (float)phi + 1;
            const int X = round_short(mx), Y = round_short(my);
            int32_t v = -1;
            if ((unsigned)X < (unsigned)pw && (unsigned)Y < (unsigned)(ph + 2)) {
                const int row = Y == 0 ? ph - 1 : (Y == ph + 1 ? 0 : Y - 1);
                v = X | (row << 16);
            }
            imap[(size_t)y * w + x] = v;
        }
}
#pragma clang fp contract(on)

bool polar_dims(const bugseg_bev_params *p, int &pw, int &ph) {
    const int w = p->occ_w, h = p->occ_h, L = std::max(w, h);
    pw = p->variant ? w : (int)std::lrint((double)L);
    ph = p->variant ? h : (int)std::lrint((double)L * 3.1415926535897932384626433832795);
    return pw > 0 && ph > 0 && pw <= 32767 && ph <= 32767 && w <= 32767 && h <= 32767;
}

size_t ls_cells_bytes(int B, const bugseg_bev_params *p) { return ((size_t)B * p->occ_w * p->occ_h + 255) & ~(size_t)255; }
size_t ls_workspace_bytes(int B, const bugseg_bev_params *p, int ph) {
    return ls_cells_bytes(B, p) + (size_t)B * ph * sizeof(int32_t);
}

int prepare_polar(bugseg_ctx *ctx, const bugseg_bev_params *p, BevArgs &a, bool cap) {
    const int w = p->occ_w, h = p->occ_h, L = std::max(w, h);
    int pw, ph;
    if (!polar_dims(p, pw, ph)) return fail(ctx, BUGSEG_EINVAL, "laserscan grid too large for the polar tables");
    bugseg_ctx::PolarTab *hit = nullptr;
    for (auto &t : ctx->polar_tabs)
        if (t.key[0] == w && t.key[1] == h && t.key[2] == p->variant) hit = &t;
    if (!hit) {
        std::vector<int32_t> fmap, imap;
        polar_tables(pw, ph, (double)L, (float)(w / 2.0 - 1), (float)h, w, h, fmap, imap);
        if (ctx->polar_tabs.size() >= 4) {
            for (size_t i = 0; i < ctx->polar_tabs.size(); ++i)
                if (!ctx->polar_tabs[i].pinned) {
                    retire(ctx, ctx->polar_tabs[i].tab, cap);
                    ctx->polar_tabs.erase(ctx->polar_tabs.begin() + (long)i);
                    break;
                }
        }
        RelaxCapture relax;
        hipStream_t s = setup_stream(ctx);
        if (!s) return fail(ctx, BUGSEG_EHIP, "could not create the table-build stream");
        bugseg_ctx::PolarTab t;
        t.key[0] = w; t.key[1] = h; t.key[2] = p->variant;
        t.pw = pw; t.ph = ph;
        const size_t bytes = (fmap.size() + imap.size()) * sizeof(int32_t);
        if (hipMalloc(&t.tab, bytes) != hipSuccess) return fail(ctx, BUGSEG_ENOMEM, "polar table allocation failed");
        hipError_t e = hipMemcpyAsync(t.tab, fmap.data(), fmap.size() * 4, hipMemcpyHostToDevice, s);
        if (e == hipSuccess)
            e = hipMemcpyAsync((int32_t *)t.tab + fmap.size(), imap.data(), imap.size() * 4, hipMemcpyHostToDevice, s);
        if (e == hipSuccess) e = hipStreamSynchronize(s);
        if (e != hipSuccess) {
            (void)hipFree(t.tab);
            return fail(ctx, BUGSEG_EHIP, std::string("polar table upload: ") + hipGetErrorString(e));
        }
        ctx->polar_tabs.push_back(t);
        hit = &ctx->polar_tabs.back();
    }
    if (cap) hit->pinned = true;
    a.laserscan = 1;
    a.fmap = (const int32_t *)hit->tab;
    a.imap = (const int32_t *)hit->tab + (size_t)pw * ph;
    a.pw = pw; a.ph = ph;
    a.hit = p->variant ? 100 : 3;
    return BUGSEG_OK;
}

int internal_scratch(bugseg_ctx *ctx, void *stream, size_t need, bool cap, void *&out) {
    bugseg_ctx::LsScratch *sc = nullptr;
    for (auto &x : ctx->ls_scratch) if (x.stream == stream) sc = &x;
    if (!sc) {
        if (ctx->ls_scratch.size() >= 8) {
            long victim = -1;
            for (size_t i = 0; i < ctx->ls_scratch.size(); ++i)
                if (!ctx->ls_scratch[i].pinned && (victim < 0 || ctx->ls_scratch[i].used < ctx->ls_scratch[(size_t)victim].used))
                    victim = (long)i;
            if (victim >= 0) {
                retire(ctx, ctx->ls_scratch[(size_t)victim].p, cap);
                ctx->ls_scratch.erase(ctx->ls_scratch.begin() + victim);
            }
        }
        ctx->ls_scratch.push_back(bugseg_ctx::LsScratch());
        sc = &ctx->ls_scratch.back();
        sc->stream = stream;
    }
    sc->used = ++ctx->use_clock;
    if (need > sc->bytes) {
        retire(ctx, sc->p, cap || sc->pinned);
        sc->p = nullptr;
        sc->bytes = 0;
        RelaxCapture relax;
        if (hipMalloc(&sc->p, need) != hipSuccess) return fail(ctx, BUGSEG_ENOMEM, "laserscan scratch allocation failed");
        sc->bytes = need;
    }
    if (cap) sc->pinned = true;
    out = sc->p;
    return BUGSEG_OK;
}

int bev_occgrid(bugseg_ctx *ctx, const uint8_t *seg, int B, const bugseg_bev_params *p, int8_t *out, bool own_ws,
                void *ws, size_t ws_bytes, void *stream) {
    if (!ctx || !seg || !p || !out) return fail(ctx, BUGSEG_EINVAL, "NULL argument");
    if (B <= 0 || p->in_rows <= 0 || p->in_cols <= 0 || p->warp_w <= 0 || p->warp_h <= 0 || p->occ_w <= 0 ||
        p->occ_h <= 0 || p->occ_w_px <= 0 || p->occ_h_px <= 0)
        return fail(ctx, BUGSEG_EINVAL, "bad BEV geometry");
    if (p->variant != 0 && p->variant != 1) return fail(ctx, BUGSEG_EINVAL, "variant must be 0 or 1");
    if (p->laserscan != 0 && p->laserscan != 1) return fail(ctx, BUGSEG_EINVAL, "laserscan must be 0 or 1");
    DeviceGuard g(ctx->device);
    BevArgs a;
    std::memset(&a, 0, sizeof(a));
    a.seg = seg; a.B = B; a.in_rows = p->in_rows; a.in_cols = p->in_cols;
    {
#pragma clang fp contract(off)
        const double *S = p->M;
        double d = S[0] * (S[4] * S[8] - S[5] * S[7]) - S[1] * (S[3] * S[8] - S[5] * S[6]) + S[2] * (S[3] * S[7] - S[4] * S[6]);
        if (d != 0.0) {
            d = 1.0 / d;
            a.Mi[0] = (S[4] * S[8] - S[5] * S[7]) * d;
            a.Mi[1] = (S[2] * S[7] - S[1] * S[8]) * d;
            a.Mi[2] = (S[1] * S[5] - S[2] * S[4]) * d;
            a.Mi[3] = (S[5] * S[6] - S[3] * S[8]) * d;
            a.Mi[4] = (S[0] * S[8] - S[2] * S[6]) * d;
            a.Mi[5] = (S[2] * S[3] - S[0] * S[5]) * d;
            a.Mi[6] = (S[3] * S[7] - S[4] * S[6]) * d;
            a.Mi[7] = (S[1] * S[6] - S[0] * S[7]) * d;
            a.Mi[8] = (S[0] * S[4] - S[1] * S[3]) * d;
        }
    }
    const int bh0 = std::min(16, p->warp_h);
    a.bw0 = std::min(1024 / bh0, p->warp_w);
    a.warp_w = p->warp_w; a.warp_h = p->warp_h;
    a.occ_w_px = p->occ_w_px; a.occ_h_px = p->occ_h_px; a.occ_w = p->occ_w; a.occ_h = p->occ_h;
    a.left_x = p->left_x; a.top_y = p->top_y;
    a.ifx = 1.0 / ((double)p->occ_w / p->occ_w_px);
    a.ify = 1.0 / ((double)p->occ_h / p->occ_h_px);
    a.ros_layout = p->ros_layout;
    a.variant = p->variant;
    a.out = out;
    if (p->laserscan) {
        int pw, ph;
        if (!polar_dims(p, pw, ph)) return fail(ctx, BUGSEG_EINVAL, "laserscan grid too large for the polar tables");
        if (!own_ws && (!ws || ws_bytes < ls_workspace_bytes(B, p, ph)))
            return fail(ctx, BUGSEG_EINVAL, "laserscan workspace missing or smaller than bugseg_bev_workspace_bytes()");
    }
    const bool cap = stream_capturing(stream);
    {
        std::vector<unsigned char> key(sizeof(double) * 11 + sizeof(int) * 12);
        unsigned char *kp = key.data();
        auto put = [&](const void *v, size_t n) { std::memcpy(kp, v, n); kp += n; };
        put(a.Mi, sizeof(a.Mi)); put(&a.ifx, sizeof(double)); put(&a.ify, sizeof(double));
        const int ik[12] = {a.in_rows, a.in_cols, a.bw0, a.warp_w, a.warp_h, a.occ_w_px, a.occ_h_px, a.occ_w, a.occ_h,
                            a.left_x, a.top_y, 0};
        put(ik, sizeof(ik));
        bugseg_ctx::BevTab *hit = nullptr;
        for (auto &t : ctx->bev_tabs) if (t.key == key) hit = &t;
        if (!hit) {
            const size_t cells = (size_t)a.occ_h * a.occ_w;
            if (cells * BEV_SLOTS > (size_t)1 << 31) return fail(ctx, BUGSEG_EINVAL, "occupancy grid too large");
            if (ctx->bev_tabs.size() >= 4) {
                for (size_t i = 0; i < ctx->bev_tabs.size(); ++i)
                    if (!ctx->bev_tabs[i].pinned) {
                        retire(ctx, ctx->bev_tabs[i].tab, cap);
                        ctx->bev_tabs.erase(ctx->bev_tabs.begin() + (long)i);
                        break;
                    }
            }
            RelaxCapture relax;
            hipStream_t s = setup_stream(ctx);
            if (!s) return fail(ctx, BUGSEG_EHIP, "could not create the table-build stream");
            bugseg_ctx::BevTab t;
            t.key = key;
            if (hipMalloc(&t.tab, bev_table_bytes(a.occ_w, a.occ_h)) != hipSuccess)
                return fail(ctx, BUGSEG_ENOMEM, "BEV table allocation failed");
            a.wtab = t.tab;
            hipError_t e = launch_bev_table(a, s);
            if (e == hipSuccess) e = hipStreamSynchronize(s);
            const int nb = bev_bands(a.occ_h);
            std::vector<int4> rec((size_t)nb * BEV_BOXREC);
            std::vector<int2> items;
            if (e == hipSuccess)
                e = hipMemcpyAsync(rec.data(), (unsigned char *)t.tab + bev_records_offset(a.occ_w, a.occ_h),
                                   rec.size() * sizeof(int4), hipMemcpyDeviceToHost, s);
            if (e == hipSuccess) e = hipStreamSynchronize(s);
            if (e == hipSuccess) {
                const char *nf = std::getenv("BUGSEG_BEV_NEAR_FIRST");
                const bool near_first = nf && std::atoi(nf) != 0;
                for (int i = 0; i < nb; ++i) {
                    const int b = near_first ? nb - 1 - i : i;
                    for (int k = 0; k < std::max(1, std::min(BEV_BAND, rec[(size_t)b * BEV_BOXREC].x)); ++k) items.push_back(make_int2(b, k));
                }
                e = hipMemcpyAsync((unsigned char *)t.tab + bev_items_offset(a.occ_w, a.occ_h), items.data(),
                                   items.size() * sizeof(int2), hipMemcpyHostToDevice, s);
            }
            if (e == hipSuccess) e = hipStreamSynchronize(s);
            t.nitems = (int)items.size();
            if (e != hipSuccess) {
                (void)hipFree(t.tab);
                return fail(ctx, BUGSEG_EHIP, std::string("BEV table: ") + hipGetErrorString(e));
            }

            ctx->bev_tabs.push_back(std::move(t));
            hit = &ctx->bev_tabs.back();
        }
        if (cap) hit->pinned = true;
        a.wtab = hit->tab;
        a.nitems = hit->nitems;
    }
    if (p->laserscan) {
        int rc = prepare_polar(ctx, p, a, cap);
        if (rc != BUGSEG_OK) return rc;
        if (own_ws) {
            rc = internal_scratch(ctx, stream, ls_workspace_bytes(B, p, a.ph), cap, ws);
            if (rc != BUGSEG_OK) return rc;
        }
        a.cells = (uint8_t *)ws;
        a.rmin = (int32_t *)((unsigned char *)ws + ls_cells_bytes(B, p));
    }
    hipError_t e = launch_bev(a, (hipStream_t)stream);
    if (e != hipSuccess) return fail(ctx, BUGSEG_EHIP, std::string("bev launch: ") + hipGetErrorString(e));
    return BUGSEG_OK;
}

}

extern "C" {

int bugseg_bev_occgrid(bugseg_ctx *ctx, const uint8_t *seg, int B, const bugseg_bev_params *p, int8_t *out, void *stream) {
    return bev_occgrid(ctx, seg, B, p, out, true, nullptr, 0, stream);
}

size_t bugseg_bev_workspace_bytes(const bugseg_bev_params *p, int B) {
    int pw, ph;
    if (!p || B <= 0 || p->occ_w <= 0 || p->occ_h <= 0 || !p->laserscan || !polar_dims(p, pw, ph)) return 0;
    return ls_workspace_bytes(B, p, ph);
}

int bugseg_bev_occgrid_ws(bugseg_ctx *ctx, const uint8_t *seg, int B, const bugseg_bev_params *p, int8_t *out,
                          void *workspace, size_t workspace_bytes, void *stream) {
    return bev_occgrid(ctx, seg, B, p, out, false, workspace, workspace_bytes, stream);
}

int bugseg_debug_parse_pack(const void *blob, size_t bytes, int precision, int *ncls) {
    if (!blob) return fail(nullptr, BUGSEG_EINVAL, "NULL blob");
    bugseg_ctx c;
    c.prec = precision == BUGSEG_BF16 ? PREC_BF16 : precision == BUGSEG_F16 ? PREC_F16 : PREC_F32;
    std::string why;
    if (!parse_blob(blob, bytes, c.blocks, c.ncls, why)) return fail(nullptr, BUGSEG_EFORMAT, "weight blob: " + why);
    if (!pack_all(&c, why)) return fail(nullptr, BUGSEG_EFORMAT, "weight blob: " + why);
    if (ncls) *ncls = c.ncls;
    return BUGSEG_OK;
}

int bugseg_debug_set_spans(bugseg_ctx *ctx, void *spans, int n_ops) {
    if (!ctx) return fail(ctx, BUGSEG_EINVAL, "NULL ctx");
    if (spans && n_ops <= 0) return fail(ctx, BUGSEG_EINVAL, "spans: n_ops must be positive");
    ctx->spans = (unsigned long long *)spans;
    ctx->spans_ops = spans ? n_ops : 0;
    return BUGSEG_OK;
}

int bugseg_debug_pool_indices(bugseg_ctx *ctx, int B, int H, int W, int block, void *dst, size_t bytes, int *idx_cs,
                              void *stream) {
    if (!ctx || !dst) return fail(ctx, BUGSEG_EINVAL, "NULL argument");
    if (!ctx->loaded) return fail(ctx, BUGSEG_ESTATE, "no weights loaded");
    Plan &pl = ctx->plan;
    if (!pl.arena || pl.B != B || pl.H != H || pl.W != W) return fail(ctx, BUGSEG_ESTATE, "no forward has run at these dimensions");
    if (block < 0 || block >= (int)pl.idx.size() || !pl.idx[(size_t)block])
        return fail(ctx, BUGSEG_EINVAL, "block " + std::to_string(block) + " is not a downsampling block");
    if (bytes != pl.idx_bytes[(size_t)block])
        return fail(ctx, BUGSEG_EINVAL, "index tensor is " + std::to_string(pl.idx_bytes[(size_t)block]) + " bytes");
    if (idx_cs) *idx_cs = cstore(ctx->blocks[(size_t)block].attrs[0]);
    DeviceGuard g(ctx->device);
    hipError_t e = hipMemcpyAsync(dst, pl.idx[(size_t)block], bytes, hipMemcpyDeviceToDevice, (hipStream_t)stream);
    if (e != hipSuccess) return fail(ctx, BUGSEG_EHIP, std::string("pool indices copy: ") + hipGetErrorString(e));
    return BUGSEG_OK;
}

int bugseg_debug_tile_walk(int ntiles, int grid, int rev, int32_t *seq, size_t seq_n, int32_t *count) {
    if (!seq || !count) return fail(nullptr, BUGSEG_EINVAL, "NULL argument");
    if (ntiles <= 0 || grid <= 0 || grid % 8 || (rev != 0 && rev != 1))
        return fail(nullptr, BUGSEG_EINVAL, "tile walk: ntiles > 0, grid a positive multiple of 8, rev 0 or 1");
    const int nslots = grid >> 3, CH = tile_walk_ch(ntiles), per = (CH + nslots - 1) / nslots;
    if (seq_n < (size_t)grid * per) return fail(nullptr, BUGSEG_EINVAL, "tile walk: seq too small");
    for (int b = 0; b < grid; ++b) {
        const int grp = b & 7, slot = b >> 3;
        int n = 0;
        for (int it = slot; it < CH; it += nslots) {
            const int tile = tile_walk(grp, it, CH, ntiles, rev);
            if (tile < 0) break;
            if (tile_walk_at(tile_walk_base(grp, CH, ntiles, rev), it) != tile ||
                tile_walk_flip(tile_walk_mirror(grp, CH, ntiles, rev), grp * CH + it) != tile)
                return fail(nullptr, BUGSEG_ESTATE, "tile walk: the kernels' forms disagree with tile_walk");
            seq[(size_t)b * per + n++] = tile;
        }
        count[b] = n;
        for (int k = n; k < per; ++k) seq[(size_t)b * per + k] = -1;
    }
    return per;
}

int bugseg_debug_ctx_info(const bugseg_ctx *ctx, int what, int arg) {
    if (!ctx) return -1;
    switch (what) {
    case 0: return ctx->naff_on ? 1 : 0;
    case 1: return ctx->range_off ? 1 : 0;
    case 2: return arg >= 0 && arg < (int)ctx->packed.size() ? ctx->packed[(size_t)arg].sw : -1000;
    default: return -1;
    }
}

int bugseg_debug_polar_tables(int w, int h, int variant, int32_t *fmap, size_t fmap_n, int32_t *imap, size_t imap_n,
                              int *pw_out, int *ph_out) {
    if (w <= 0 || h <= 0 || w > 32767 || h > 32767) return fail(nullptr, BUGSEG_EINVAL, "bad grid");
    const int L = std::max(w, h);
    const int pw = variant ? w : (int)std::lrint((double)L);
    const int ph = variant ? h : (int)std::lrint((double)L * 3.1415926535897932384626433832795);
    if (ph > 32767) return fail(nullptr, BUGSEG_EINVAL, "grid too large for the polar tables");
    std::vector<int32_t> f, im;
    polar_tables(pw, ph, (double)L, (float)(w / 2.0 - 1), (float)h, w, h, f, im);
    if (pw_out) *pw_out = pw;
    if (ph_out) *ph_out = ph;
    if (fmap) std::memcpy(fmap, f.data(), std::min(fmap_n, f.size()) * sizeof(int32_t));
    if (imap) std::memcpy(imap, im.data(), std::min(imap_n, im.size()) * sizeof(int32_t));
    return BUGSEG_OK;
}

int bugseg_plan_info(bugseg_ctx *ctx, int B, int H, int W, int out_kind, int bgr_input, int *n_launches, double *alg_bytes,
                     double *plan_bytes, double *flops) {
    if (!ctx) return fail(ctx, BUGSEG_EINVAL, "NULL ctx");
    if (!ctx->loaded) return fail(ctx, BUGSEG_ESTATE, "no weights loaded");
    DeviceGuard g(ctx->device);
    std::string why;
    if (!build_plan(ctx, B, H, W, why)) return fail(ctx, BUGSEG_EINVAL, why);
    double lb = 0, pb = 0, fl = 0;
    for (const Op &op : ctx->plan.ops) {
        pb += op.bytes;
        lb += op.layer_bytes >= 0 ? op.layer_bytes : op.bytes;
        fl += op.flops;
    }
    const double fin = out_kind == BUGSEG_OUT_LOGITS_F32 ? (double)B * H * W * ctx->ncls * 4 : (double)B * H * W;
    if (ctx->plan.cls_ok && out_kind != BUGSEG_OUT_LOGITS_F32) {
        const Op &q = ctx->plan.ops[ctx->plan.ops.size() - 2];
        pb -= 2.0 * q.bn.B * q.bn.H * q.bn.W * q.bn_c * prec_es(ctx->prec);
    }
    double adj = bgr_input ? (double)B * H * W * (8.0 * prec_es(ctx->prec) - 3.0) : 0.0;
    if (n_launches) *n_launches = (int)ctx->plan.ops.size();
    if (alg_bytes) *alg_bytes = lb + fin - adj;
    if (plan_bytes) *plan_bytes = pb + fin - adj;
    if (flops) *flops = fl;
    return BUGSEG_OK;
}

int bugseg_plan_op(bugseg_ctx *ctx, int B, int H, int W, int op, char *kernel, int kernel_len, double *alg_bytes,
                   double *plan_bytes, double *flops) {
    if (!ctx) return fail(ctx, BUGSEG_EINVAL, "NULL ctx");
    if (!ctx->loaded) return fail(ctx, BUGSEG_ESTATE, "no weights loaded");
    Plan &pl = ctx->plan;
    if (!pl.arena || pl.B != B || pl.H != H || pl.W != W) return fail(ctx, BUGSEG_ESTATE, "no forward has run at these dimensions");
    if (op < 0 || op >= (int)pl.ops.size()) return fail(ctx, BUGSEG_EINVAL, "op index out of range");
    const Op &o = pl.ops[op];
    const int nops = (int)pl.ops.size();
    std::string tag;
    if (pl.cls_on && op + 1 == nops) {
        if (kernel && kernel_len > 0) std::snprintf(kernel, (size_t)kernel_len, "fused");
        if (alg_bytes) *alg_bytes = 0;
        if (plan_bytes) *plan_bytes = 0;
        if (flops) *flops = 0;
        return BUGSEG_OK;
    }
    if (pl.cls_on && op + 2 == nops) {
        const Op &l = pl.ops.back();
        const double outb = (double)o.bn.B * o.bn.H * o.bn.W * o.bn_c * prec_es(ctx->prec);
        const double fin = (double)B * H * W;
        if (kernel && kernel_len > 0) std::snprintf(kernel, (size_t)kernel_len, "bneck C16+classes 16x16");
        const double lb_b = o.layer_bytes >= 0 ? o.layer_bytes : o.bytes, lb_l = l.layer_bytes >= 0 ? l.layer_bytes : l.bytes;
        if (alg_bytes) *alg_bytes = lb_b + lb_l + fin;
        if (plan_bytes) *plan_bytes = o.bytes - outb + (l.bytes - outb) + fin;
        if (flops) *flops = o.flops + l.flops;
        return BUGSEG_OK;
    }
    if (o.kind == 2) {
        tag = "up C" + std::to_string(o.up_cout);
    } else if (o.kind == 1) {
// ... 44 lines not shown
```

### bugcar_image_segmentation_amd/csrc/cls_kernels.hip

```cpp
#include "bugseg_internal.h"
#include "cls_common.h"

namespace bugseg {

#ifndef CLS_ABL
#define CLS_ABL 0
#endif
#ifndef CLS_AUX
#define CLS_AUX 0
#endif
#ifndef CLS_SPLIT1
#define CLS_SPLIT1 0
#endif
#ifndef CLS_BIAS_REG
#define CLS_BIAS_REG 1
#endif
template <typename T, bool LOGITS, int LK = 0>
#ifndef CLS_OCC_F32
#define CLS_OCC_F32 1
#endif
__global__ void __launch_bounds__(256, sizeof(T) == 2 ? 4 : CLS_OCC_F32) cls_kernel(const ConvArgs a) {
    span_enter(a.span);
    constexpr int CLS_TAPS = 4;
    using Raw = typename Tr<T>::Raw;
    using WRaw = typename WTr<T>::Raw;
    constexpr int ES = (int)sizeof(T);
    __shared__ float sbias[64];
    const int tid = threadIdx.x, lane = tid & 63, col = lane & 31, h = lane >> 5;
    const int wave = __builtin_amdgcn_readfirstlane(tid >> 6);
    if (tid < 64) sbias[tid] = (tid & 15) < a.ncls ? a.bias[tid] : -INFINITY;
    const uint64_t lut64 = cls_lut64(a.lut);

    WRaw wr[2][CLS_TAPS];
    {
        const T *w = reinterpret_cast<const T *>(a.w);
#pragma unroll
        for (int b = 0; b < 2; ++b) {
            const int prow = cls_prow(b, col);
#pragma unroll
            for (int s = 0; s < CLS_TAPS; ++s) {
                ld8(wr[b][s], w + (size_t)prow * a.Kpad + s * 16 + 8 * h);
            }
        }
    }
    bool short_blk[2];
#pragma unroll
    for (int b = 0; b < 2; ++b) short_blk[b] = __ballot(nonzero(wr[b][2]) || nonzero(wr[b][3])) == 0;
    __syncthreads();

    auto ldbias = [&](int b) {
        int boff = (2 * b + h) * 16;
        asm volatile("" : "+v"(boff));
        const float4 *bb = reinterpret_cast<const float4 *>(sbias + boff);
        f32x16 v;
#pragma unroll
        for (int j = 0; j < 4; ++j) {
            const float4 q = bb[j];
            v[4 * j] = q.x; v[4 * j + 1] = q.y; v[4 * j + 2] = q.z; v[4 * j + 3] = q.w;
        }
        return v;
    };
    constexpr bool BREG = CLS_BIAS_REG && !LOGITS && sizeof(T) == 2;
    f32x16 bvec;
    if constexpr (BREG) bvec = ldbias(0);
    constexpr bool F32 = ES == 4;
    bool scl = false;
    float xm = 1.f, bm = 1.f, om = 1.f;
    if constexpr (F32) {
        if (!a.rg.off) {
            const int sx = rng_exp_meas(rng_read(a.rg)), e = sx + a.rg.sw[0];
            scl = (sx | e) != 0;
            xm = rng_pow2(sx); bm = rng_pow2(e); om = rng_pow2(-e);
        }
    }
    const auto rin = mkbuf(a.in, a.in_bytes);
    const int HWg = a.Hg * a.Wg;
    const size_t plane = (size_t)a.Hout * a.Wout;
    const int groups = (a.M + 31) >> 5;
    const int xcd = blockIdx.x & 7, nw = (gridDim.x >> 3) * 4, wi = (blockIdx.x >> 3) * 4 + wave;
    const int C = (groups + 7) >> 3, g0 = xcd * C, g1 = g0 + C < groups ? g0 + C : groups;
    auto grp_of = [&](int k) -> int { return !a.rev ? g0 + k : k < g1 - g0 ? g1 - 1 - k : groups; };
    const uint32_t pixB = (uint32_t)(a.CinS * ES), rowB = (uint32_t)a.Win * pixB;

    struct Px { uint32_t p; int n, y, x; bool ok; };
    auto pixel = [&](int g) -> Px {
        const uint32_t p0 = (uint32_t)g * 32u;
        const int n0 = (int)(__umulhi(p0, a.mHWg) >> a.sHWg);
        const uint32_t r = p0 - (uint32_t)(n0 * HWg);
        const int y0 = (int)(__umulhi(r, a.mWg) >> a.sWg), x0 = (int)r - y0 * a.Wg;
        Px q;
        q.p = p0 + (uint32_t)col;
        q.ok = (int)q.p < a.M;
        q.x = x0 + col;
        const bool wrap = q.x >= a.Wg;
        q.x = wrap ? q.x - a.Wg : q.x;
        q.y = y0 + (wrap ? 1 : 0);
        const bool wrapn = q.y >= a.Hg;
        q.y = wrapn ? 0 : q.y;
        q.n = n0 + (wrapn ? 1 : 0);
        return q;
    };
    auto load = [&](int g, Raw (&xf)[CLS_TAPS], Px &q) {
        q = pixel(g);
        if constexpr ((CLS_ABL & 8) != 0) {
#pragma unroll
            for (int s = 0; s < CLS_TAPS; ++s) zero(xf[s]);
            if constexpr (sizeof(T) == 2) xf[0].v.x = (uint32_t)g;
            return;
        }
        const uint32_t base = q.p * pixB + (uint32_t)(8 * h * ES);
        const bool okx = q.x + 1 < a.Win, oky = q.y + 1 < a.Hin;
        const int v00 = (int)(q.ok ? base : OOB), v01 = (int)(q.ok && okx ? base : OOB);
        const int v10 = (int)(q.ok && oky ? base : OOB), v11 = (int)(q.ok && okx && oky ? base : OOB);
        const int vo[CLS_TAPS] = {v00, v01, v10, v11};
#pragma unroll
        for (int s = 0; s < CLS_TAPS; ++s) {
            const int d = (int)((uint32_t)(s >> 1) * rowB + (uint32_t)(s & 1) * pixB);
            if constexpr (sizeof(T) == 2) {
                xf[s].v = __builtin_bit_cast(uint4, __builtin_amdgcn_raw_buffer_load_b128(rin, vo[s], d, 0));
            } else {
                reinterpret_cast<RawF &>(xf[s]).a =
                    __builtin_bit_cast(float4, __builtin_amdgcn_raw_buffer_load_b128(rin, vo[s], d, 0));
                reinterpret_cast<RawF &>(xf[s]).b =
                    __builtin_bit_cast(float4, __builtin_amdgcn_raw_buffer_load_b128(rin, vo[s], d + 16, 0));
            }
        }
    };

    const auto rcls = mkbuf(a.cls_out, (uint32_t)((size_t)a.B * plane));
    auto step = [&](int k, const Raw (&cur)[CLS_TAPS], Raw (&nxt)[CLS_TAPS], const Px &q, Px &qn) {
        load(grp_of(k + nw), nxt, qn);
        constexpr bool S1 = F32 && CLS_SPLIT1;
        f16x8 sxh[S1 ? CLS_TAPS : 1], sxl[S1 ? CLS_TAPS : 1];
        if constexpr (S1) {
#pragma unroll
            for (int s = 0; s < CLS_TAPS; ++s) {
                RawF xq = reinterpret_cast<const RawF &>(cur[s]);
                if (scl) mul8(xq, xm);
                split_f16(xq, sxh[s], sxl[s]);
            }
        }
        auto taps = [&](int b, f32x16 &acc, auto sc) {
            auto tap = [&](int s) {
                if constexpr (S1) {
                    if constexpr (F32) mma32s(acc, reinterpret_cast<const RawS &>(wr[b][s]), sxh[s], sxl[s]);
                    return;
                }
                Raw xq = cur[s];
                if constexpr (decltype(sc)::value) mul8(reinterpret_cast<RawF &>(xq), xm);
                mma32(acc, wr[b][s], xq);
            };
            tap(0);
            tap(1);
            if (!short_blk[b]) {
                tap(2);
                tap(3);
            }
        };
        auto block = [&](int b, f32x16 &acc) {
            acc = BREG ? bvec : ldbias(b);
            if constexpr ((CLS_ABL & 1) != 0 && sizeof(T) == 2) { acc[0] += __builtin_bit_cast(float, cur[0].v.x & 1u); return; }
            bool done = false;
            if constexpr (F32) {
                if (scl) {
#pragma unroll
                    for (int c = 0; c < 16; ++c) acc[c] *= bm;
                    taps(b, acc, std::true_type());
#pragma unroll
                    for (int c = 0; c < 16; ++c) acc[c] *= om;
                    done = true;
                }
            }
            if (!done) taps(b, acc, std::false_type());
            if (LOGITS && q.ok) {
                float *lo = a.logits_out + (size_t)q.n * a.ncls * plane + (size_t)(2 * q.y + b) * a.Wout + 2 * q.x + h;
#pragma unroll
                for (int c = 0; c < 16; ++c)
                    if (c < a.ncls) lo[(size_t)c * plane] = acc[c];
            }
        };
        int cls[2];
        f32x16 acc[2];
        block(0, acc[0]);
        block(1, acc[1]);
        cls_argmax<LK>(acc, lut64, cls);
        if constexpr ((CLS_ABL & 2) != 0)
            for (int b = 0; b < 2; ++b) cls[b] = acc[b][b] > acc[b][5] ? 1 : 0;
        if (a.cls_out) {
            uint32_t c0 = (uint32_t)cls[0], c1 = (uint32_t)cls[1];
            pl32swap(c0, c1);
            const uint32_t o = 4u * q.p - 2u * (uint32_t)q.x + (uint32_t)(2 * h * a.Wg);
            if (!(CLS_ABL & 4) || c0 == 77)
                __builtin_amdgcn_raw_buffer_store_b16((unsigned short)(c0 | (c1 << 8)), rcls, q.ok ? (int)o : (int)OOB, 0, CLS_AUX);
        }
    };
    Raw xa[CLS_TAPS], xb[CLS_TAPS];
    Px qa, qb;
    int k = wi;
    if (k < g1 - g0) load(grp_of(k), xa, qa);
    while (k < g1 - g0) {
        step(k, xa, xb, qa, qb);
        k += nw;
        if (k >= g1 - g0) break;
        step(k, xb, xa, qb, qa);
        k += nw;
    }
    span_exit(a.span);
}

bool cls_supported(const ConvArgs &a) {
    return a.CinS == 16 && a.Npad == 64 && a.Kpad == 64 && a.ncls >= 1 && a.ncls <= 16 && a.Wg >= 32 &&
           a.Hout == 2 * a.Hg && a.Wout == 2 * a.Wg && a.Hg == a.Hin && a.Wg == a.Win;
}

template <typename T>
static const void *cls_fun(bool lg, int lk) {
    if (lg) return (const void *)cls_kernel<T, true, 0>;
    return lk == 1 ? (const void *)cls_kernel<T, false, 1> : lk == 2 ? (const void *)cls_kernel<T, false, 2>
                   : (const void *)cls_kernel<T, false, 0>;
}

hipError_t launch_cls(int prec, const ConvArgs &a, hipStream_t s) {
    const int groups = (a.M + 31) / 32;
    const bool lg = a.logits_out != nullptr;
    const int lk = a.lut && (a.lut_kind == 1 || a.lut_kind == 2) ? a.lut_kind : 0;
    const void *f = prec == PREC_BF16 ? cls_fun<__bf16>(lg, lk) : prec == PREC_F16 ? cls_fun<_Float16>(lg, lk) : cls_fun<float>(lg, lk);
    const int per = occupancy_per_cu(f, 256, 0);
    const int cap = device_cus() * (per > 0 ? per : 4);
    int g = (groups + 3) / 4;
    g = g < cap ? g : cap;
    g = (g + 7) & ~7;
    void *args[] = {const_cast<ConvArgs *>(&a)};
    return hipLaunchKernel(f, dim3(g), dim3(256), args, 0, s);
}

}
```

### bugcar_image_segmentation_amd/csrc/up_kernels.hip

```cpp
#include "bugseg_internal.h"
#include "mfma_common.h"

namespace bugseg {


#ifndef UP_NT128
#define UP_NT128 512
#endif
template <typename T, int CIN>
__host__ __device__ constexpr int up_threads() { return sizeof(T) == 2 && CIN >= 128 ? UP_NT128 : 256; }

template <typename T, int CIN, int I, int COUT>
__global__ void __launch_bounds__((up_threads<T, CIN>()), (sizeof(T) == 2 ? (CIN >= 128 ? (UP_NT128 == 512 ? 4 : 2) : 3) : 1)) up_kernel(const UpArgs a) {
    span_enter(a.span);
    using Raw = typename Tr<T>::Raw;
    using WRaw = typename WTr<T>::Raw;
    constexpr int ES = (int)sizeof(T);
#ifndef UP_NT_F32
#define UP_NT_F32 1
#endif
#ifndef UP_AUX_F32_LOW
#define UP_AUX_F32_LOW 0
#endif
#ifndef UP_NT_2B
#define UP_NT_2B 0
#endif
    constexpr int OAUX = (sizeof(T) == 4 && (UP_NT_F32 == 2 || (UP_NT_F32 == 1 && CIN >= 128))) || (sizeof(T) == 2 && UP_NT_2B && CIN >= 128) ? 2
                       : sizeof(T) == 4 && CIN < 128 ? UP_AUX_F32_LOW
                       : OUT_AUX_SEL(CIN >= 128 ? 16 : 0);
    constexpr int NR1 = (COUT + I) / 16;
    constexpr int NM = COUT / 16, NE = I / 16;
    constexpr int KS1 = CIN / 32;
    constexpr int NR2 = 4 * I / 16;
    constexpr int NR3 = COUT / 16;
    static_assert(COUT % 16 == 0 && I % 16 == 0 && CIN % 32 == 0 && I <= 32, "up_kernel shape");
    constexpr bool SWAP = ES == 2 && NR3 % 2 == 0;
#ifndef UP_F32_LINES
#define UP_F32_LINES 1
#endif
#ifndef UP_F32_LINES16
#define UP_F32_LINES16 0
#endif
    constexpr bool LINES = ES == 4 && NR3 % 2 == 0 && UP_F32_LINES;
    constexpr bool LINES16 = ES == 4 && NR3 == 1 && UP_F32_LINES16;
    static_assert(NM <= 4 && NE <= 4, "main / e1 launches must carry their bias in the accumulator");
    constexpr bool B1ACC = true;
    constexpr bool B2ACC = bias_in_acc(NR2, 1), B3ACC = bias_in_acc(NR3, 1);
    constexpr int UPAD = ES == 2 ? 16 : 16 / ES;
    constexpr int K1S = CIN + UPAD, K2S = 32 + UPAD, K3S = 32 + UPAD;
    auto wch = [](int, int c, int) -> int { return c * 8; };
    extern __shared__ __attribute__((aligned(16))) unsigned char smem[];
    T *w1s = reinterpret_cast<T *>(smem);
    T *w2s = w1s + NR1 * 16 * K1S;
    T *w3s = w2s + NR2 * 16 * K2S;
    float *cb1 = reinterpret_cast<float *>(w3s + NR3 * 16 * K3S), *cs1 = cb1 + NR1 * 16;
    float *cb2 = cs1 + NR1 * 16, *cs2 = cb2 + NR2 * 16;
    float *cb3 = cs2 + NR2 * 16, *cs3 = cb3 + NR3 * 16, *cso = cs3 + NR3 * 16;
    constexpr int NT = up_threads<T, CIN>();
    const int tid = threadIdx.x;
    {
        auto stage = [&](T *dst, const void *src, int rows, int kpad, int kstride) {
            const int cpr = kpad * ES / 16;
            const uint4 *s = reinterpret_cast<const uint4 *>(src);
            for (int i = tid; i < rows * cpr; i += NT) {
                const int r = i / cpr, c = i - r * cpr;
                *reinterpret_cast<uint4 *>(dst + (size_t)r * kstride + c * (16 / ES)) = s[i];
            }
        };
        stage(w1s, a.w1, NR1 * 16, CIN, K1S);
        stage(w2s, a.w2, NR2 * 16, 32, K2S);
        stage(w3s, a.w3, NR3 * 16, 32, K3S);
        for (int i = tid; i < NR1 * 16; i += NT) { cb1[i] = a.b1[i]; cs1[i] = a.s1[i]; }
        for (int i = tid; i < NR2 * 16; i += NT) { cb2[i] = a.b2[i]; cs2[i] = a.s2[i]; }
        for (int i = tid; i < NR3 * 16; i += NT) { cb3[i] = a.b3[i]; cs3[i] = a.s3[i]; cso[i] = a.s_out[i]; }
    }
    __syncthreads();
    const int lane = tid & 63, col = lane & 15, kq = lane >> 4;
    const bool fast = a.slopes_le1;
    auto act = [&](float4 v, const float *s) { return fast ? prelu4m(v, ld4f(s)) : prelu4(v, ld4f(s)); };
    const auto rx = mkbuf(a.x, a.x_bytes);
    const auto ri = mkbuf(a.idx, a.idx_bytes);
    const auto ro = mkbuf(a.out, a.out_bytes);
    const int hw = a.h * a.w;
    const int nfrag = (a.M + 15) >> 4;
    const int gw = blockIdx.x * (NT / 64) + __builtin_amdgcn_readfirstlane(tid >> 6), nw = gridDim.x * (NT / 64);
    constexpr bool F32 = ES == 4;
    bool scl = false;
    float xm = 1.f, b1m = 1.f, m1m = 1.f, o1m = 1.f, b2m = 1.f, o2m = 1.f, b3m = 1.f, o3m = 1.f;
    float amo = 0.f;
    if constexpr (F32) {
      const RangeArgs &g = a.rg;
      if (!g.off) {
        const float amx = rng_read(g);
        const int sx = rng_exp_meas(amx), e1 = sx + g.sw[0];
        const float Br = g.n[0] * amx + g.c[0];
        const int sr = rng_exp_bound(Br, e1), e2 = sr + g.sw[1];
        const int st = rng_exp_bound(g.n[1] * Br + g.c[1], e2), e3 = st + g.sw[2];
        scl = e3 != 0;
        xm = rng_pow2(sx); b1m = rng_pow2(e1); m1m = rng_pow2(-e1); o1m = rng_pow2(sr - e1);
        b2m = rng_pow2(e2); o2m = rng_pow2(st - e2); b3m = rng_pow2(e3); o3m = rng_pow2(-e3);
      }
    }
    auto bias_m = [&](const float *p, float m) -> f32x4 {
        f32x4 b = bias4(p);
        if constexpr (F32) b = mul4(b, m);
        return b;
    };

    Raw xn[KS1];
    uint32_t idn[NM];
    auto load = [&](int f) {
        const int p = f * 16 + col;
        const bool pv = p < a.M;
#pragma unroll
        for (int s = 0; s < KS1; ++s) bld8(xn[s], rx, pv ? (uint32_t)(p * CIN + s * 32 + kq * 8) * ES : OOB);
#pragma unroll
        for (int r = 0; r < NM; ++r)
            idn[r] = __builtin_amdgcn_raw_buffer_load_b32(ri, pv ? (int)(p * a.idxCS + r * 16 + kq * 4) : (int)OOB, 0, 0);
    };
    auto frag_of = [&](int k) -> int { return a.rev ? nfrag - 1 - k : k; };
    if (gw < nfrag) load(frag_of(gw));
    for (int k = gw; k < nfrag; k += nw) {
        const int f = frag_of(k);
        int wofs = 0;
        if constexpr (CIN >= 128) asm volatile("" : "+v"(wofs));
        const T *w1 = w1s + wofs, *w2 = w2s + wofs, *w3 = w3s + wofs;
        const int p = f * 16 + col;
        const bool pv = p < a.M;
        const uint32_t pp = pv ? (uint32_t)p : 0u;
        const int n = (int)fdiv(pp, a.mHW, a.sHW), rr = (int)pp - n * hw;
        const int y = (int)fdiv((uint32_t)rr, a.mW, a.sW), x = rr - y * a.w;

        Raw xf[KS1];
        uint32_t id[NM];
#pragma unroll
        for (int s = 0; s < KS1; ++s) xf[s] = xn[s];
#pragma unroll
        for (int r = 0; r < NM; ++r) id[r] = idn[r];
        if (k + nw < nfrag) load(frag_of(k + nw));
        f32x4 acc1[NR1];
        static_assert(B1ACC, "GEMM 1 starts from the bias");
#pragma unroll
        for (int r = 0; r < NR1; ++r) acc1[r] = bias_m(cb1 + r * 16 + kq * 4, b1m);
#pragma unroll
        for (int s = 0; s < KS1; ++s) {
            Raw xq = xf[s];
            if constexpr (F32) xq = scale8(xf[s], xm);
#pragma unroll
            for (int r = 0; r < NR1; ++r) {
                WRaw wf;
                ld8(wf, w1 + (r * 16 + col) * K1S + wch(col, s * 4 + kq, CIN));
                mma(acc1[r], wf, xq);
            }
        }
        if constexpr (F32) {
#pragma unroll
            for (int r = 0; r < NR1; ++r) acc1[r] = mul4(acc1[r], r < NM ? m1m : o1m);
        }
        auto ep1 = [&](int r) {
            const int c = r * 16 + kq * 4;
            return round_t(act(f4(acc1[r]), cs1 + c), (const T *)nullptr);
        };
        float4 mv[NM];
#pragma unroll
        for (int r = 0; r < NM; ++r) mv[r] = ep1(r);
        Raw bop2;
        to_bop(bop2, ep1(NM), NE > 1 ? ep1(NM + 1) : make_float4(0.f, 0.f, 0.f, 0.f));

        const uint32_t obase = pv ? (uint32_t)((n * 2 * a.h + 2 * y) * (2 * a.w) + 2 * x) : 0u;
        uint32_t obase_o = 0u;
        bool pv_o = false;
        if constexpr (LINES || LINES16) {
            const int po = f * 16 + (col ^ 8);
            pv_o = po < a.M;
            const uint32_t ppo = pv_o ? (uint32_t)po : 0u;
            const int no = (int)fdiv(ppo, a.mHW, a.sHW), rro = (int)ppo - no * hw;
            const int yo = (int)fdiv((uint32_t)rro, a.mW, a.sW), xo = rro - yo * a.w;
            obase_o = pv_o ? (uint32_t)((no * 2 * a.h + 2 * yo) * (2 * a.w) + 2 * xo) : 0u;
        }
        float4 ev_prev = make_float4(0.f, 0.f, 0.f, 0.f);
#pragma unroll 1
        for (int ph = 0; ph < 4; ++ph) {
            f32x4 acc2[NE];
#pragma unroll
            for (int e = 0; e < NE; ++e) {
                const int r2 = ph * NE + e;
                static_assert(B2ACC, "the tconv starts from the bias");
                acc2[e] = bias_m(cb2 + r2 * 16 + kq * 4, b2m);
                WRaw wf;
                ld8(wf, w2 + (r2 * 16 + col) * K2S + wch(col, kq, 32));
                mma(acc2[e], wf, bop2);
                if constexpr (F32) acc2[e] = mul4(acc2[e], o2m);
            }
            auto ep2 = [&](int e) {
                const int c = (ph * NE + e) * 16 + kq * 4;
                return round_t(act(f4(acc2[e]), cs2 + c), (const T *)nullptr);
            };
            Raw bop3;
            to_bop(bop3, ep2(0), NE > 1 ? ep2(1) : make_float4(0.f, 0.f, 0.f, 0.f));
            const uint32_t pho = (uint32_t)((ph >> 1) * 2 * a.w + (ph & 1));
            const uint32_t opix = obase + pho;
            auto ep3 = [&](int r) {
                const int c = r * 16 + kq * 4;
                static_assert(B3ACC, "the expansion starts from the bias");
                f32x4 acc = bias_m(cb3 + c, b3m);
                WRaw wf;
                ld8(wf, w3 + (r * 16 + col) * K3S + wch(col, kq, 32));
                mma(acc, wf, bop3);
                float4 v = f4(acc);
                if constexpr (F32) {
                    if (scl) v = mul4(v, o3m);
                }
                v = act(v, cs3 + c);
                const uint32_t w = id[r];
                const uint32_t pos = (uint32_t)ph;
                v.x += ((w & 0xff) == pos) ? mv[r].x : 0.f;
                v.y += (((w >> 8) & 0xff) == pos) ? mv[r].y : 0.f;
                v.z += (((w >> 16) & 0xff) == pos) ? mv[r].z : 0.f;
                v.w += (((w >> 24) & 0xff) == pos) ? mv[r].w : 0.f;
                return act(v, cso + c);
            };
            if constexpr (SWAP) {
#pragma unroll
                for (int t = 0; t < NR3 / 2; ++t) {
                    const u32x2_t p0 = pack4<T>(ep3(2 * t)), p1 = pack4<T>(ep3(2 * t + 1));
                    uint32_t x0 = p0.x, x1 = p0.y, y0 = p1.x, y1 = p1.y;
                    pl16swap(x0, y0);
                    pl16swap(x1, y1);
                    const int ch = (2 * t + (kq & 1)) * 16 + 8 * (kq >> 1);
                    bst16o<OAUX>(ro, pv ? (opix * COUT + ch) * ES : OOB, make_uint4(x0, x1, y0, y1));
                }
            } else if constexpr (LINES16) {
                const float4 v = ep3(0);
                rng_acc4(amo, v);
                if ((ph & 1) == 0) {
                    ev_prev = v;
                } else {
                    const bool lo8 = col < 8;
                    const uint32_t phe = pho - 1u;
                    const uint32_t pa = (lo8 ? obase : obase_o) + phe, pb = (lo8 ? obase_o : obase) + phe;
                    const bool va = lo8 ? pv : pv_o, vb = lo8 ? pv_o : pv;
                    const uint4 u0 = __builtin_bit_cast(uint4, ev_prev), u1 = __builtin_bit_cast(uint4, v);
                    const uint4 xs = lo8 ? u1 : u0;
                    uint4 ys;
                    ys.x = (uint32_t)__builtin_amdgcn_update_dpp(0, (int)xs.x, 0x128, 0xf, 0xf, false);
                    ys.y = (uint32_t)__builtin_amdgcn_update_dpp(0, (int)xs.y, 0x128, 0xf, 0xf, false);
                    ys.z = (uint32_t)__builtin_amdgcn_update_dpp(0, (int)xs.z, 0x128, 0xf, 0xf, false);
                    ys.w = (uint32_t)__builtin_amdgcn_update_dpp(0, (int)xs.w, 0x128, 0xf, 0xf, false);
                    const int ch = (lo8 ? 0 : 16) + kq * 4;
                    bst16o<OAUX>(ro, va ? (pa * COUT + ch) * ES : OOB, lo8 ? u0 : ys);
                    bst16o<OAUX>(ro, vb ? (pb * COUT + ch) * ES : OOB, lo8 ? ys : u1);
                }
            } else if constexpr (LINES) {
                const bool lo8 = col < 8;
                const uint32_t pa = lo8 ? obase + pho : obase_o + pho, pb = lo8 ? obase_o + pho : obase + pho;
                const bool va = lo8 ? pv : pv_o, vb = lo8 ? pv_o : pv;
                const int hc = lo8 ? 0 : 16;
#pragma unroll
                for (int t = 0; t < NR3 / 2; ++t) {
// ... 89 lines not shown
```

### bugcar_image_segmentation_amd/hostio.py

```python
from __future__ import annotations

import numpy as np
import torch

from .hostio_ring import SlotRing


class HostStream:
    def __init__(self, pipe, batch: int, frame_hw: tuple[int, int] | None = None, depth: int = 2, graph: bool = True):
        if int(batch) != batch or batch < 1:
            raise ValueError("batch must be an integer >= 1")
        self._ring = SlotRing(depth)
        self.pipe = pipe
        self.batch = B = int(batch)
        self.depth = self._ring.depth
        self.graph = bool(graph)
        H0, W0 = (pipe.H, pipe.W) if frame_hw is None else (int(frame_hw[0]), int(frame_hw[1]))
        if H0 < 1 or W0 < 1:
            raise ValueError("frame_hw must be positive")
        self.frame_shape = (B, H0, W0, 3)
        self.grid_shape = tuple(pipe._grid_shape(B))
        self.device = dev = torch.device("cuda", pipe.model.ctx.device)
        self._compute = torch.cuda.current_stream(dev)
        self._cin = torch.cuda.Stream(device=dev)
        self._cout = torch.cuda.Stream(device=dev)
        n = self.depth
        self._pin_frames = [torch.empty(self.frame_shape, dtype=torch.uint8, pin_memory=True) for _ in range(n)]
        self._pin_grids = [torch.empty(self.grid_shape, dtype=torch.int8, pin_memory=True) for _ in range(n)]
        self._np_frames = [t.numpy() for t in self._pin_frames]
        self._np_grids = [t.numpy() for t in self._pin_grids]
        with torch.cuda.stream(self._compute):
            self._dev_frames = [torch.zeros(self.frame_shape, dtype=torch.uint8, device=dev) for _ in range(n)]
            self._dev_grids = [torch.empty(self.grid_shape, dtype=torch.int8, device=dev) for _ in range(n)]
            self._steps = []
            if self.graph:
                for s in range(n):
                    replay, _ = pipe.capture(self._dev_frames[s], out=self._dev_grids[s])
                    self._steps.append(replay)
                self._keep = (pipe._x, pipe._seg, pipe._grid, dict(getattr(pipe, "_pairs", {})))
        self._in_done = [torch.cuda.Event() for _ in range(n)]
        self._in_used = [False] * n
        self._step_done = [torch.cuda.Event() for _ in range(n)]
        self._out_done = [torch.cuda.Event() for _ in range(n)]
        self._closed = False

    @property
    def outstanding(self) -> int:
        return self._ring.outstanding

    @property
    def steps_put(self) -> int:
        return self._ring._put

    def _check_open(self):
        if self._closed:
            raise RuntimeError("HostStream is closed")

    def next_frames(self) -> np.ndarray:
        self._check_open()
        s = self._ring.put_slot
        if self._in_used[s]:
            self._in_done[s].synchronize()
        return self._np_frames[s]

    def put(self, frames=None) -> int:
        self._check_open()
        if frames is not None:
            frames = np.asarray(frames)
            if frames.dtype != np.uint8 or tuple(frames.shape) != self.frame_shape:
                raise ValueError(f"frames must be a uint8 array of shape {self.frame_shape}, got {frames.dtype} "
                                 f"{tuple(frames.shape)}")
        if self._ring.full:
            self._ring.put()
        if frames is not None:
            np.copyto(self.next_frames(), frames)
        s, seq = self._ring.put()
        with torch.cuda.stream(self._cin):
            self._dev_frames[s].copy_(self._pin_frames[s], non_blocking=True)
            self._in_done[s].record(self._cin)
        self._in_used[s] = True
        self._compute.wait_event(self._in_done[s])
        with torch.cuda.stream(self._compute):
            if self.graph:
                self._steps[s]()
            else:
                self.pipe.run(self._dev_frames[s], out=self._dev_grids[s])
            self._step_done[s].record(self._compute)
        self._cout.wait_event(self._step_done[s])
        with torch.cuda.stream(self._cout):
            self._pin_grids[s].copy_(self._dev_grids[s], non_blocking=True)
            self._out_done[s].record(self._cout)
        return seq

    def get(self, copy: bool = False) -> np.ndarray:
        self._check_open()
        s, _seq = self._ring.peek()
        self._out_done[s].synchronize()
        self._ring.get()
        g = self._np_grids[s]
        return g.copy() if copy else g

    def map(self, batches):
        if self.outstanding:
            raise RuntimeError("map() needs a stream with no outstanding step")
        for frames in batches:
            if self._ring.full:
                yield self.get(copy=True)
            self.put(frames)
        while self.outstanding:
            yield self.get(copy=True)

    def close(self) -> None:
        if self._closed:
            return
        self._closed = True
        for st in (self._cin, self._compute, self._cout):
            st.synchronize()
        self._steps = []
        self._keep = None
        self._np_frames = self._np_grids = None
        self._pin_frames = self._pin_grids = self._dev_frames = self._dev_grids = None

# ... 13 lines not shown
```

### bugcar_image_segmentation_amd/pipeline.py

```python
from __future__ import annotations

import numpy as np
import torch

from . import _native as N
from .bev import bev_transform_tools
from .models import ENET


class OccupancyPipeline:

    def __init__(self, model: ENET, bev: bev_transform_tools, grid_w_m: float, grid_h_m: float, cell_m: float,
                 model_hw: tuple[int, int] | None = None, ros_layout: bool = False, streams: int = 1,
                 binary: bool = False, stream_priority: int = 0, chain_forwards: bool = False, shard_offset: int = 0):
        self.model = model
        self.binary = binary
        self.bev = bev
        self.grid = (grid_w_m, grid_h_m, cell_m)
        self.H, self.W = model_hw if model_hw is not None else (ENET.INPUT_HEIGHT, ENET.INPUT_WIDTH)
        self.ros_layout = ros_layout
        if (self.H, self.W) != (bev.input_width, bev.input_height):
            raise ValueError(f"model output {self.H}x{self.W} must equal the calibration's input image size "
                             f"{bev.input_width}x{bev.input_height} (bev.py:169)")
        if streams < 1:
            raise ValueError("streams must be >= 1")
        self.streams = streams
        self.stream_priority = stream_priority
        self.chain_forwards = chain_forwards
        self.shard_offset = int(shard_offset)
        self._ctxs = [model.ctx]
        self._streams = []
        self._x = None
        self._seg = None
        self._grid = None

    def _shard_ctxs(self, dev: torch.device):
        while len(self._ctxs) < self.streams:
            c = N.Context(dev.index, self.model.ctx.precision)
            c.load_weights(self.model.blob)
            self._ctxs.append(c)
            self._streams.append(torch.cuda.Stream(device=dev, priority=self.stream_priority))
        return self._ctxs, self._streams

    def _bufs(self, B: int, dev: torch.device):
        if self._x is None or self._x.shape[0] != B or self._x.device != dev:
            self._x = torch.empty((B, self.H, self.W, 3), dtype=torch.uint8, device=dev)
            self._seg = torch.empty((B, self.H, self.W), dtype=torch.uint8, device=dev)
            self._grid = torch.empty(self._grid_shape(B), dtype=torch.int8, device=dev)
        return self._x, self._seg, self._grid

    def _params(self):
        return self.bev.occupancy_params(*self.grid, ros_layout=self.ros_layout, binary=self.binary)

    def _grid_shape(self, B):
        p = self._params()
        shape = (B, p.occ_w, p.occ_h) if self.ros_layout else (B, p.occ_h, p.occ_w)
        return ((2,) + shape) if self.binary and p.laserscan else shape

    def run(self, frames_bgr: torch.Tensor, out: torch.Tensor | None = None) -> torch.Tensor:
        if frames_bgr.dim() != 4 or frames_bgr.shape[3] != 3 or frames_bgr.dtype != torch.uint8 or not frames_bgr.is_cuda:
            raise ValueError("frames must be a (B, H0, W0, 3) uint8 device tensor")
        B, H0, W0 = frames_bgr.shape[:3]
        x, seg, grid = self._bufs(B, frames_bgr.device)
        if grid.shape != self._grid_shape(B):
            self._grid = grid = torch.empty(self._grid_shape(B), dtype=torch.int8, device=frames_bgr.device)
        frames = frames_bgr.contiguous()
        out = grid if out is None else out
        if tuple(out.shape) != tuple(grid.shape) or out.dtype != torch.int8 or not out.is_contiguous():
            raise ValueError(f"out must be a contiguous int8 tensor of shape {tuple(grid.shape)}")
        p = self._params()
        if self.streams == 1 or B < self.streams:
            self._run_shard(self.model.ctx, frames, x, seg, out, p, None)
            return out
        pair = self.binary and bool(p.laserscan)
        ctxs, streams = self._shard_ctxs(frames.device)
        main = torch.cuda.current_stream(frames.device)
        ready = main.record_event()
        bounds = [B * i // self.streams for i in range(self.streams + 1)]
        for i in range(self.streams):
            s, e = bounds[i], bounds[i + 1]
            st = main if i == 0 else streams[i - 1]
            if i:
                st.wait_event(ready)
            split_done = self.chain_forwards or (self.shard_offset > 0 and i + 1 < self.streams)
            with torch.cuda.stream(st):
                if self.shard_offset > 0 and i + 1 < self.streams:
                    self._run_forward(ctxs[i], frames[s:e], x[s:e], seg[s:e], st, split=self.shard_offset)
                    ready = self._split_event
                elif self.chain_forwards:
                    self._run_forward(ctxs[i], frames[s:e], x[s:e], seg[s:e], st)
                    ready = torch.cuda.Event()
                    ready.record(st)
                if pair:
                    tmp = self._pair_buf(i, (2, e - s) + tuple(out.shape[2:]), out.device)
                    self._run_shard(ctxs[i], frames[s:e], x[s:e], seg[s:e], tmp, p, st, forward=not split_done)
                    out[:, s:e].copy_(tmp)
                else:
                    self._run_shard(ctxs[i], frames[s:e], x[s:e], seg[s:e], out[s:e], p, st, forward=not split_done)
        for st in streams[: self.streams - 1]:
            main.wait_stream(st)
        return out

    def _pair_buf(self, i, shape, dev):
        if not hasattr(self, "_pairs"):
            self._pairs = {}
        t = self._pairs.get(i)
        if t is None or tuple(t.shape) != shape or t.device != dev:
            t = self._pairs[i] = torch.empty(shape, dtype=torch.int8, device=dev)
        return t

    def capture(self, frames_bgr: torch.Tensor, out: torch.Tensor | None = None, warm: bool = True):
        dev = frames_bgr.device
        if warm:
            self.run(frames_bgr, out)
        elif self.streams > 1 and frames_bgr.shape[0] >= self.streams:
            self._shard_ctxs(dev)
        torch.cuda.synchronize(dev)
        graph = torch.cuda.CUDAGraph()
        with torch.cuda.graph(graph):
            res = self.run(frames_bgr, out)
        return graph.replay, res

    def host_stream(self, batch: int, frame_hw: tuple[int, int] | None = None, depth: int = 2, graph: bool = True):
        from .hostio import HostStream
        return HostStream(self, batch, frame_hw=frame_hw, depth=depth, graph=graph)

    def run_host(self, frames_np) -> np.ndarray:
        f = np.asarray(frames_np)
        if f.ndim != 4 or f.shape[3] != 3 or f.dtype != np.uint8:
            raise ValueError("frames must be a (B, H0, W0, 3) uint8 array")
        if not hasattr(self, "_host"):
            self._host = {}
        key, stamp = tuple(f.shape[:3]), bytes(self._params())
        hit = self._host.get(key)
        if hit is None or hit[0] != stamp:
            if hit is not None:
                hit[1].close()
            hit = self._host[key] = (stamp, self.host_stream(f.shape[0], frame_hw=f.shape[1:3], depth=1))
        hit[1].put(f)
        return hit[1].get(copy=True)

    def _run_forward(self, ctx, frames, x, seg, stream, split=0):
        B, H0, W0 = frames.shape[:3]
        if (H0, W0) != (self.H, self.W):
            ctx.preprocess(frames, B, H0, W0, self.H, self.W, N.PRE_BGR_U8, x, stream)
            frames = x
        kind = N.OUT_BINARY_U8 if self.binary else N.OUT_CLASS3_U8
        if split <= 0:
            ctx.forward_bgr(frames, B, self.H, self.W, kind, seg, stream)
            return
        ctx.forward_bgr_ops(frames, B, self.H, self.W, kind, seg, 0, split, stream)
        self._split_event = torch.cuda.Event()
        self._split_event.record(stream)
        ctx.forward_bgr_ops(frames, B, self.H, self.W, kind, seg, split, -1, stream)

    def _run_shard(self, ctx, frames, x, seg, out, p, stream, forward=True):
        if forward:
            self._run_forward(ctx, frames, x, seg, stream)
        ctx.bev(seg, frames.shape[0], p, out, stream)
```

### include/bugseg.h

```cpp
#ifndef BUGSEG_H
#define BUGSEG_H

#include <stddef.h>
#include <stdint.h>

#ifdef __cplusplus
extern "C" {
#endif

typedef struct bugseg_ctx bugseg_ctx;

enum {
    BUGSEG_OK = 0,
    BUGSEG_EINVAL = -1,
    BUGSEG_ENOMEM = -2,
    BUGSEG_EHIP = -3,
    BUGSEG_EFORMAT = -4,
    BUGSEG_ESTATE = -5
};

enum { BUGSEG_FP32 = 0, BUGSEG_BF16 = 1, BUGSEG_F16 = 2 };

enum {
    BUGSEG_OUT_LOGITS_F32 = 0,
    BUGSEG_OUT_CLASS15_U8 = 1,
    BUGSEG_OUT_CLASS3_U8 = 2,
    BUGSEG_OUT_BINARY_U8 = 3
};

enum {
    BUGSEG_PRE_ENGINE = 0,
    BUGSEG_PRE_NCHW_F64 = 1,
    BUGSEG_PRE_NCHW_F32 = 2,
    BUGSEG_PRE_BGR_U8 = 3
};

typedef struct {
    double M[9];
    int in_rows;
    int in_cols;
    int warp_w;
    int warp_h;
    int occ_w_px;
    int occ_h_px;
    int occ_w;
    int occ_h;
    int left_x;
    int top_y;
    int ros_layout;
    int variant;
    int laserscan;
} bugseg_bev_params;

int bugseg_version(void);

int bugseg_create(int device, int precision, bugseg_ctx **out);
int bugseg_destroy(bugseg_ctx *ctx);

int bugseg_load_weights(bugseg_ctx *ctx, const void *blob, size_t bytes);

int bugseg_num_classes(const bugseg_ctx *ctx);

size_t bugseg_input_bytes(const bugseg_ctx *ctx, int B, int H, int W);

int bugseg_preprocess(bugseg_ctx *ctx, const uint8_t *bgr_dev, int B, int H0, int W0, int H, int W,
                      int out_layout, void *out_dev, void *stream);

int bugseg_nchw_to_input(bugseg_ctx *ctx, const void *x_dev, int is_f64, int B, int H, int W,
                         void *out_dev, void *stream);

int bugseg_enet_forward(bugseg_ctx *ctx, const void *in_dev, int B, int H, int W, int out_kind,
                        void *out_dev, void *stream);

int bugseg_enet_forward_bgr(bugseg_ctx *ctx, const uint8_t *bgr_dev, int B, int H, int W, int out_kind,
                            void *out_dev, void *stream);

int bugseg_enet_forward_bgr_ops(bugseg_ctx *ctx, const uint8_t *bgr_dev, int B, int H, int W, int out_kind,
                                void *out_dev, int first_op, int last_op, void *stream);

int bugseg_bev_occgrid(bugseg_ctx *ctx, const uint8_t *seg_dev, int B, const bugseg_bev_params *p,
                       int8_t *out_dev, void *stream);

size_t bugseg_bev_workspace_bytes(const bugseg_bev_params *p, int B);
int bugseg_bev_occgrid_ws(bugseg_ctx *ctx, const uint8_t *seg_dev, int B, const bugseg_bev_params *p,
                          int8_t *out_dev, void *workspace_dev, size_t workspace_bytes, void *stream);

int bugseg_plan_info(bugseg_ctx *ctx, int B, int H, int W, int out_kind, int bgr_input, int *n_launches,
                     double *alg_bytes, double *plan_bytes, double *flops);

int bugseg_plan_op(bugseg_ctx *ctx, int B, int H, int W, int op, char *kernel, int kernel_len, double *alg_bytes,
                   double *plan_bytes, double *flops);
int bugseg_plan_launch_op(bugseg_ctx *ctx, int B, int H, int W, int op, void *stream);

const char *bugseg_last_error(const bugseg_ctx *ctx);

int bugseg_debug_parse_pack(const void *blob, size_t bytes, int precision, int *ncls);
int bugseg_debug_polar_tables(int w, int h, int variant, int32_t *fmap, size_t fmap_n, int32_t *imap, size_t imap_n,
                              int *pw, int *ph);
int bugseg_debug_tile_walk(int ntiles, int grid, int rev, int32_t *seq, size_t seq_n, int32_t *count);
int bugseg_debug_ctx_info(const bugseg_ctx *ctx, int what, int arg);
int bugseg_debug_set_spans(bugseg_ctx *ctx, void *spans, int n_ops);
int bugseg_debug_pool_indices(bugseg_ctx *ctx, int B, int H, int W, int block, void *dst, size_t bytes, int *idx_cs,
                              void *stream);

#define BUGSEG_DL_OP_FIELDS 32
typedef struct bugseg_dl bugseg_dl;

int bugseg_dl_create(int device, int precision, bugseg_dl **out);
int bugseg_dl_destroy(bugseg_dl *dl);
int bugseg_dl_load_weights(bugseg_dl *dl, const void *blob, size_t bytes);
int bugseg_dl_set_plan(bugseg_dl *dl, const int32_t *ops, int nops, const uint64_t *buf_bytes, int nbufs,
                       int B, int Hc, int Wc);
int bugseg_dl_forward(bugseg_dl *dl, const uint8_t *rgb_dev, int B, int H, int W, int64_t *out_dev, void *stream);
int bugseg_dl_launch_op(bugseg_dl *dl, int op, void *stream);
int bugseg_dl_read_buffer(bugseg_dl *dl, int buf, void *dst_dev, size_t bytes, void *stream);
const char *bugseg_dl_last_error(const bugseg_dl *dl);
int bugseg_dl_debug_check_plan(const int32_t *ops, int nops, const uint64_t *buf_bytes, int nbufs, int B, int Hc, int Wc,
                               int precision, size_t w_bytes);

#ifdef __cplusplus
}
#endif
#endif
```

Measured before the change: 20040 frames/s.

## Restrict decoder tail ops to image rows the BEV warp actually samples

Computes from the BEV homography the source row range that the occupancy grid reads, then propagates row windows back through the last six decoder ops (upsample, bottlenecks, classifier conv) and launches them only over those rows. The full segmentation map is recomputed lazily if anyone reads it, so the skipped rows are not observable through the pipeline output. The aim is to cut decoder work for rows above the horizon or outside the warp. In exchange it adds window-plan bookkeeping, new kernel offsets, and a correctness risk at window edges.

```diff
diff --git a/bugcar_image_segmentation_amd/_native.py b/bugcar_image_segmentation_amd/_native.py
--- a/bugcar_image_segmentation_amd/_native.py
+++ b/bugcar_image_segmentation_amd/_native.py
@@ -17,7 +17,8 @@
 
 EXPORTED = ("bugseg_version", "bugseg_create", "bugseg_destroy", "bugseg_load_weights", "bugseg_num_classes",
             "bugseg_input_bytes", "bugseg_preprocess", "bugseg_nchw_to_input", "bugseg_enet_forward",
-            "bugseg_enet_forward_bgr", "bugseg_enet_forward_bgr_ops",
+            "bugseg_enet_forward_bgr", "bugseg_enet_forward_bgr_ops", "bugseg_enet_forward_bgr_rows",
+            "bugseg_bev_source_rows", "bugseg_debug_row_windows", "bugseg_debug_poison_arena",
             "bugseg_bev_occgrid", "bugseg_bev_workspace_bytes", "bugseg_bev_occgrid_ws", "bugseg_plan_info", "bugseg_plan_op", "bugseg_plan_launch_op",
             "bugseg_last_error",
             "bugseg_dl_create", "bugseg_dl_destroy", "bugseg_dl_load_weights", "bugseg_dl_set_plan",
@@ -68,6 +69,10 @@
             "bugseg_enet_forward": (i, [vp, vp, i, i, i, i, vp, vp]),
             "bugseg_enet_forward_bgr": (i, [vp, vp, i, i, i, i, vp, vp]),
             "bugseg_enet_forward_bgr_ops": (i, [vp, vp, i, i, i, i, vp, i, i, vp]),
+            "bugseg_enet_forward_bgr_rows": (i, [vp, vp, i, i, i, i, vp, i, i, i, i, vp]),
+            "bugseg_bev_source_rows": (i, [vp, ctypes.POINTER(BevParams), i, i, ctypes.POINTER(i), ctypes.POINTER(i)]),
+            "bugseg_debug_row_windows": (i, [i, i, i, i, i, i, vp]),
+            "bugseg_debug_poison_arena": (i, [vp, i, vp]),
             "bugseg_bev_occgrid": (i, [vp, vp, i, ctypes.POINTER(BevParams), vp, vp]),
             "bugseg_bev_workspace_bytes": (sz, [ctypes.POINTER(BevParams), i]),
             "bugseg_bev_occgrid_ws": (i, [vp, vp, i, ctypes.POINTER(BevParams), vp, vp, sz, vp]),
@@ -121,6 +126,13 @@
     return [list(seq[b * per:b * per + count[b]]) for b in range(grid)]
 
 
+def row_windows(H: int, W: int, row0: int, row1: int, tile_rows_c64: int = 8, tile_rows_c16: int = 16) -> list[tuple[int, int]]:
+    lib = load_library()
+    win = (ctypes.c_int32 * 12)()
+    check(lib.bugseg_debug_row_windows(H, W, row0, row1, tile_rows_c64, tile_rows_c16, win))
+    return [(win[2 * k], win[2 * k + 1]) for k in range(6)]
+
+
 def require_gpu() -> None:
     if not torch.cuda.is_available():
         raise RuntimeError("bugseg needs a HIP GPU (MI355X / gfx950); none is visible — there is no CPU fallback")
@@ -183,6 +195,20 @@
     def forward_bgr_ops(self, bgr, B, H, W, out_kind, out, first_op, last_op, stream=None):
         check(self.lib.bugseg_enet_forward_bgr_ops(self.h, bgr.data_ptr(), B, H, W, out_kind, out.data_ptr(),
                                                    first_op, last_op, stream_handle(stream)), self.h)
+
+    def forward_bgr_rows(self, bgr, B, H, W, out_kind, out, rows, first_op=0, last_op=-1, stream=None):
+        check(self.lib.bugseg_enet_forward_bgr_rows(self.h, bgr.data_ptr(), B, H, W, out_kind, out.data_ptr(),
+                                                    int(rows[0]), int(rows[1]), first_op, last_op,
+                                                    stream_handle(stream)), self.h)
+
+    def bev_source_rows(self, params: BevParams, rows: int, cols: int) -> tuple[int, int]:
+        r0, r1 = ctypes.c_int(0), ctypes.c_int(0)
+        check(self.lib.bugseg_bev_source_rows(self.h, ctypes.byref(params), rows, cols, ctypes.byref(r0),
+                                              ctypes.byref(r1)), self.h)
+        return r0.value, r1.value
+
+    def poison_arena(self, byte: int, stream=None) -> None:
+        check(self.lib.bugseg_debug_poison_arena(self.h, int(byte), ctypes.c_void_p(stream_handle(stream))), self.h)
 
     def bev(self, seg, B, params: BevParams, out, stream=None):
         st = stream if stream is not None else torch.cuda.current_stream(seg.device)
diff --git a/bugcar_image_segmentation_amd/csrc/bev_kernels.hip b/bugcar_image_segmentation_amd/csrc/bev_kernels.hip
--- a/bugcar_image_segmentation_amd/csrc/bev_kernels.hip
+++ b/bugcar_image_segmentation_amd/csrc/bev_kernels.hip
@@ -356,12 +356,14 @@
     __shared__ int red[BEV_BAND][4];
     __shared__ int4 pbox[BEV_BAND];
     __shared__ int np_rpp[2];
+    __shared__ int sred[2];
     const long cells = (long)a.occ_h * a.occ_w;
     const int band = blockIdx.x, r0 = band * BEV_BAND, r1 = min(a.occ_h, r0 + BEV_BAND);
     const int nr = r1 - r0, n = nr * a.occ_w;
     int ylo[BEV_BAND], yhi[BEV_BAND], xlo[BEV_BAND], xhi[BEV_BAND];
 #pragma unroll
     for (int k = 0; k < BEV_BAND; ++k) { ylo[k] = xlo[k] = 1 << 30; yhi[k] = xhi[k] = -(1 << 30); }
+    int slo = 1 << 30, shi = -(1 << 30);
     for (int i = threadIdx.x; i < n * BEV_WIN; i += 256) {
         const int c = i / BEV_WIN, k = i - c * BEV_WIN, ri = c / a.occ_w;
         const long rem = (long)r0 * a.occ_w + c;
@@ -373,12 +375,20 @@
         if (v & 12) { y_lo = min(y_lo, sy + 1); y_hi = max(y_hi, sy + 1); }
         if (v & 5) { x_lo = min(x_lo, sx); x_hi = max(x_hi, sx); }
         if (v & 10) { x_lo = min(x_lo, sx + 1); x_hi = max(x_hi, sx + 1); }
+        {
+            const bool ax = (e.y & 31u) != 0, ay = ((e.y >> 5) & 31u) != 0;
+            if ((v & 1) || ((v & 2) && ax)) { slo = min(slo, sy); shi = max(shi, sy); }
+            if (ay && ((v & 4) || ((v & 8) && ax))) { slo = min(slo, sy + 1); shi = max(shi, sy + 1); }
+        }
 #pragma unroll
         for (int q = 0; q < BEV_BAND; ++q)
             if (q == ri) { ylo[q] = min(ylo[q], y_lo); yhi[q] = max(yhi[q], y_hi); xlo[q] = min(xlo[q], x_lo); xhi[q] = max(xhi[q], x_hi); }
     }
     if (threadIdx.x < 4 * BEV_BAND) red[threadIdx.x >> 2][threadIdx.x & 3] = threadIdx.x & 1 ? -(1 << 30) : (1 << 30);
+    if (threadIdx.x < 2) sred[threadIdx.x] = threadIdx.x ? -(1 << 30) : (1 << 30);
     __syncthreads();
+    atomicMin(&sred[0], slo);
+    atomicMax(&sred[1], shi);
 #pragma unroll
     for (int q = 0; q < BEV_BAND; ++q) {
         atomicMin(&red[q][0], ylo[q]); atomicMax(&red[q][1], yhi[q]); atomicMin(&red[q][2], xlo[q]); atomicMax(&red[q][3], xhi[q]);
@@ -414,7 +424,7 @@
             pbox[0].z = -1;
         }
         np_rpp[0] = P; np_rpp[1] = rpp;
-        bbox[(size_t)band * BEV_BOXREC] = make_int4(P, rpp, 0, 0);
+        bbox[(size_t)band * BEV_BOXREC] = make_int4(P, rpp, sred[0], sred[1]);
         for (int k = 0; k < BEV_BAND; ++k) bbox[(size_t)band * BEV_BOXREC + 1 + k] = pbox[k];
     }
     __syncthreads();
diff --git a/bugcar_image_segmentation_amd/csrc/bneck_kernels.hip b/bugcar_image_segmentation_amd/csrc/bneck_kernels.hip
--- a/bugcar_image_segmentation_amd/csrc/bneck_kernels.hip
+++ b/bugcar_image_segmentation_amd/csrc/bneck_kernels.hip
@@ -474,6 +474,7 @@
         n = t / a.phases;
         const int py = RD ? ph : ph / dt, px = RD ? 0 : ph - py * dt;
         oy0 = py + dt * tyi * (tr ? TW : TH) - (CLS ? tyi : 0);
+        if constexpr (C != 128 && !DN && !CLS) oy0 += a.oy_base;
         ox0 = RD ? 0 : px + dt * txi * (tr ? TH : TW) - (CLS ? txi : 0);
     };
     Raw kx[KEEP ? NF2 : 1][KS1];
diff --git a/bugcar_image_segmentation_amd/csrc/bugseg_internal.h b/bugcar_image_segmentation_amd/csrc/bugseg_internal.h
--- a/bugcar_image_segmentation_amd/csrc/bugseg_internal.h
+++ b/bugcar_image_segmentation_amd/csrc/bugseg_internal.h
@@ -70,6 +70,7 @@
     int slopes_le1;
     RangeArgs rg;
     unsigned long long *span;
+    int wy0, wrows, orow0, orow1;
 };
 
 __host__ __device__ inline int tile_walk_ch(int ntiles) { return (ntiles + 7) >> 3; }
@@ -135,6 +136,7 @@
     uint32_t cls_bytes;
     const uint8_t *lut;
     int lut_kind, ncls, csw;
+    int oy_base;
 };
 int bneck_variants(int C);
 bool bneck_keeps_c64(int prec, int v);
@@ -161,6 +163,7 @@
     int slopes_le1;
     RangeArgs rg;
     unsigned long long *span;
+    int y0, hwin;
 };
 bool up_supported(int cin, int it, int cout);
 hipError_t launch_up(int prec, int cin, int it, int cout, const UpArgs &a, hipStream_t s);
diff --git a/bugcar_image_segmentation_amd/csrc/bugseg_runtime.cpp b/bugcar_image_segmentation_amd/csrc/bugseg_runtime.cpp
--- a/bugcar_image_segmentation_amd/csrc/bugseg_runtime.cpp
+++ b/bugcar_image_segmentation_amd/csrc/bugseg_runtime.cpp
@@ -112,9 +112,15 @@
     }
 };
 
+constexpr int WIN_OPS = 6;
+struct WinOp { int y0 = 0, y1 = 0, var = 0, tr = 0, te = 1, tiles_x = 0; };
+struct WinPlan { int row0 = 0, row1 = 0; WinOp op[WIN_OPS]; };
+
 struct Plan {
     int B = 0, H = 0, W = 0;
     std::vector<Op> ops;
+    std::vector<WinPlan> wins;
+    size_t act_bytes = 0;
     float *words = nullptr;
     size_t words_bytes = 0;
     void *arena = nullptr;
@@ -167,7 +173,7 @@
     struct LsScratch { void *stream = nullptr; void *p = nullptr; size_t bytes = 0; uint64_t used = 0; bool pinned = false; };
     std::vector<LsScratch> ls_scratch;
     uint64_t use_clock = 0;
-    struct BevTab { std::vector<unsigned char> key; uint4 *tab = nullptr; bool pinned = false; int nitems = 0; };
+    struct BevTab { std::vector<unsigned char> key; uint4 *tab = nullptr; bool pinned = false; int nitems = 0; int row0 = 0, row1 = 0; };
     std::vector<BevTab> bev_tabs;
     std::vector<void *> graveyard;
 };
@@ -1016,6 +1022,7 @@
                         const Packed &p1 = P(4), &p2 = P(2), &p3 = P(3);
                         q.x = curp; q.idx = idx[ref]; q.out = dst;
                         q.M = B * cur.H * cur.W; q.h = cur.H; q.w = cur.W;
+                        q.y0 = 0; q.hwin = cur.H;
                         q.idxCS = cstore(ctx->blocks[ref].attrs[0]);
                         fastdiv((uint32_t)(cur.H * cur.W), q.mHW, q.sHW);
                         fastdiv((uint32_t)cur.W, q.mW, q.sW);
@@ -1105,6 +1112,7 @@
 bool finish_conv_args(ConvArgs &a, int epi, size_t es) {
     fastdiv((uint32_t)(a.Hg * a.Wg), a.mHWg, a.sHWg);
     fastdiv((uint32_t)a.Wg, a.mWg, a.sWg);
+    a.wy0 = 0; a.wrows = a.Hg; a.orow0 = 0; a.orow1 = a.Hout;
     const double in_b = (double)a.B * a.Hin * a.Win * a.CinS * es;
     const double out_b = epi == EPI_CLASSES ? 0.0 : (double)a.B * a.Hout * a.Wout * a.outC * es;
     const double res_b = a.res ? (double)a.B * a.resH * a.resW * a.resCS * es : 0.0;
@@ -1184,7 +1192,67 @@
     pl.words_bytes = words_bytes;
     pl.B = B; pl.H = H; pl.W = W;
     pl.arena_bytes = total;
+    pl.act_bytes = total - al(words_bytes);
+    pl.wins.clear();
     return true;
+}
+
+template <typename F>
+void row_windows(int H, int row0, int row1, F tile_rows, int (*win)[2]) {
+    const int h2 = H / 2, h4 = H / 4, h8 = H / 8;
+    int a = row0, b = row1;
+    auto set = [&](int k) { win[k][0] = a; win[k][1] = b; };
+    auto halve = [&](int h) { a >>= 1; b = std::min((b + 1) >> 1, h); };
+    auto grow = [&](int h) { a = std::max(a - 1, 0); b = std::min(b + 1, h); };
+    auto tiles = [&](int k, int h) {
+        const int t = std::max(1, tile_rows(k, a, b));
+        b = std::min(a + (b - a + t - 1) / t * t, h);
+    };
+    halve(h2); set(5);
+    b = std::min(b + 1, h2);
+    tiles(4, h2); set(4); grow(h2);
+    halve(h4); set(3);
+    tiles(2, h4); set(2); grow(h4);
+    tiles(1, h4); set(1); grow(h4);
+    halve(h8); set(0);
+}
+
+const WinPlan *window_plan(bugseg_ctx *ctx, int row0, int row1) {
+    Plan &pl = ctx->plan;
+    if (row0 < 0 || row1 > pl.H || row0 >= row1 || (row0 == 0 && row1 == pl.H)) return nullptr;
+    for (const WinPlan &w : pl.wins)
+        if (w.row0 == row0 && w.row1 == row1) return &w;
+    const int n = (int)pl.ops.size();
+    if (n < WIN_OPS + 1 || pl.cls_ok || std::getenv("BUGSEG_CLS_CONV")) return nullptr;
+    const Op *o = &pl.ops[(size_t)(n - WIN_OPS)];
+    auto reg = [&](const Op &q, int C, int h) {
+        return q.kind == 1 && q.bn_c == C && !q.bn_asym && q.bn_cin == 0 && q.bn.dt == 1 && q.bn.phases == 1 && q.bn.H == h;
+    };
+    const int H = pl.H;
+    if (!(o[0].kind == 2 && o[0].up.h == H / 8 && reg(o[1], 64, H / 4) && reg(o[2], 64, H / 4) && o[3].kind == 2 &&
+          o[3].up.h == H / 4 && reg(o[4], 16, H / 2) && o[5].kind == 0 && o[5].epi == EPI_CLASSES && cls_supported(o[5].a) &&
+          o[5].a.Hg == H / 2))
+        return nullptr;
+    WinPlan w;
+    w.row0 = row0; w.row1 = row1;
+    int win[WIN_OPS][2];
+    row_windows(H, row0, row1, [&](int k, int need0, int need1) {
+        const Op &q = o[k];
+        WinOp &r = w.op[k];
+        int ty = 0, tx = 0, tr = 0, rd = 0;
+        int v = pick_bneck_variant(ctx, q.bn_c, false, 1, pl.B, need1 - need0, q.bn.W, ty, tx, tr, rd);
+        if (v < 0 || rd) { v = q.bn_var; tr = q.bn.tr; }
+        int th, tw, nw;
+        bneck_shape(q.bn_c, v, th, tw, nw, nullptr);
+        r.var = v; r.tr = tr;
+        r.te = tr ? tw : th;
+        r.tiles_x = tr ? (q.bn.W + th - 1) / th : (q.bn.W + tw - 1) / tw;
+        return r.te;
+    }, win);
+    for (int k = 0; k < WIN_OPS; ++k) { w.op[k].y0 = win[k][0]; w.op[k].y1 = win[k][1]; }
+    if (pl.wins.size() >= 8) pl.wins.erase(pl.wins.begin());
+    pl.wins.push_back(w);
+    return &pl.wins.back();
 }
 
 void linear_coeffs(int dsize, int ssize, double scale, int *ofs, short *a01) {
@@ -1442,11 +1510,40 @@
     return a;
 }
 
-static hipError_t launch_op(const bugseg_ctx *ctx, int i, hipStream_t s) {
+static hipError_t launch_op(const bugseg_ctx *ctx, int i, hipStream_t s, const WinPlan *wp = nullptr) {
     const Plan &pl = ctx->plan;
     const Op &o = pl.ops[(size_t)i];
     const int rev = pl.tile_order == 2 ? 1 : pl.tile_order == 1 ? (o.pos & 1) : 0;
     unsigned long long *sp = ctx->spans && i < ctx->spans_ops ? ctx->spans + 512 * (size_t)i : nullptr;
+    const int wk = i - ((int)pl.ops.size() - WIN_OPS);
+    if (wp && wk >= 0) {
+        const WinOp &w = wp->op[wk];
+        const int rows = w.y1 - w.y0;
+        if (o.kind == 1) {
+            BneckArgs q = o.bn;
+            q.span = sp; q.rev = rev;
+            q.tr = w.tr; q.tiles_x = w.tiles_x;
+            q.tiles_y = (rows + w.te - 1) / w.te;
+            q.ntiles = q.B * q.tiles_y * q.tiles_x;
+            q.oy_base = w.y0;
+            return launch_bneck(ctx->prec, o.bn_c, false, w.var, q, s, 0);
+        }
+        if (o.kind == 2) {
+            UpArgs q = o.up;
+            q.span = sp; q.rev = rev;
+            q.y0 = w.y0; q.hwin = rows;
+            q.M = (q.M / q.h) * rows;
+            fastdiv((uint32_t)(rows * q.w), q.mHW, q.sHW);
+            return launch_up(ctx->prec, o.up_cin, o.up_it, o.up_cout, q, s);
+        }
+        ConvArgs q = o.a;
+        q.span = sp; q.rev = rev;
+        q.wy0 = w.y0; q.wrows = rows;
+        q.M = q.B * rows * q.Wg;
+        fastdiv((uint32_t)(rows * q.Wg), q.mHWg, q.sHWg);
+        q.orow0 = wp->row0; q.orow1 = wp->row1;
+        return launch_conv(ctx->prec, o.nr, o.epi, q, s);
+    }
     if (pl.cls_on && i + 2 == (int)pl.ops.size()) { BneckArgs q = cls_fused_args(pl); q.span = sp; q.rev = rev; return launch_bneck_cls(ctx->prec, q, s); }
     if (pl.cls_on && i + 1 == (int)pl.ops.size()) return hipSuccess;
     if (o.kind == 1) { BneckArgs q = o.bn; q.span = sp; q.rev = rev; return launch_bneck(ctx->prec, o.bn_c, o.bn_asym, o.bn_var, q, s, o.bn_cin); }
@@ -1458,7 +1555,7 @@
 }
 
 static int enet_forward(bugseg_ctx *ctx, const void *in, bool bgr, int B, int H, int W, int out_kind, void *out,
-                        void *stream, int first_op = 0, int last_op = -1) {
+                        void *stream, int first_op = 0, int last_op = -1, int row0 = 0, int row1 = 0) {
     if (!ctx || !in || !out) return fail(ctx, BUGSEG_EINVAL, "NULL argument");
     if (!ctx->loaded) return fail(ctx, BUGSEG_ESTATE, "no weights loaded");
     if (out_kind < BUGSEG_OUT_LOGITS_F32 || out_kind > BUGSEG_OUT_BINARY_U8) return fail(ctx, BUGSEG_EINVAL, "bad out_kind");
@@ -1493,8 +1590,9 @@
         if (e != hipSuccess) return fail(ctx, BUGSEG_EHIP, std::string("range words: ") + hipGetErrorString(e));
     }
     pl.cls_on = pl.cls_ok && out_kind != BUGSEG_OUT_LOGITS_F32 && first_op <= nops - 2 && last_op == nops;
+    const WinPlan *wp = window_plan(ctx, row0, row1);
     for (int i = first_op; i < last_op; ++i) {
-        hipError_t e = launch_op(ctx, i, (hipStream_t)stream);
+        hipError_t e = launch_op(ctx, i, (hipStream_t)stream, wp);
         if (e != hipSuccess) return fail(ctx, BUGSEG_EHIP, "conv launch " + std::to_string(i) + ": " + hipGetErrorString(e));
     }
     return BUGSEG_OK;
@@ -1512,6 +1610,11 @@
 int bugseg_enet_forward_bgr_ops(bugseg_ctx *ctx, const uint8_t *bgr, int B, int H, int W, int out_kind, void *out,
                                 int first_op, int last_op, void *stream) {
     return enet_forward(ctx, bgr, true, B, H, W, out_kind, out, stream, first_op, last_op);
+}
+
+int bugseg_enet_forward_bgr_rows(bugseg_ctx *ctx, const uint8_t *bgr, int B, int H, int W, int out_kind, void *out,
+                                 int row0, int row1, int first_op, int last_op, void *stream) {
+    return enet_forward(ctx, bgr, true, B, H, W, out_kind, out, stream, first_op, last_op, row0, row1);
 }
 
 }
@@ -1663,18 +1766,14 @@
     return BUGSEG_OK;
 }
 
-int bev_occgrid(bugseg_ctx *ctx, const uint8_t *seg, int B, const bugseg_bev_params *p, int8_t *out, bool own_ws,
-                void *ws, size_t ws_bytes, void *stream) {
-    if (!ctx || !seg || !p || !out) return fail(ctx, BUGSEG_EINVAL, "NULL argument");
-    if (B <= 0 || p->in_rows <= 0 || p->in_cols <= 0 || p->warp_w <= 0 || p->warp_h <= 0 || p->occ_w <= 0 ||
+int bev_geometry(bugseg_ctx *ctx, const bugseg_bev_params *p, BevArgs &a) {
+    if (p->in_rows <= 0 || p->in_cols <= 0 || p->warp_w <= 0 || p->warp_h <= 0 || p->occ_w <= 0 ||
         p->occ_h <= 0 || p->occ_w_px <= 0 || p->occ_h_px <= 0)
         return fail(ctx, BUGSEG_EINVAL, "bad BEV geometry");
     if (p->variant != 0 && p->variant != 1) return fail(ctx, BUGSEG_EINVAL, "variant must be 0 or 1");
     if (p->laserscan != 0 && p->laserscan != 1) return fail(ctx, BUGSEG_EINVAL, "laserscan must be 0 or 1");
-    DeviceGuard g(ctx->device);
-    BevArgs a;
     std::memset(&a, 0, sizeof(a));
-    a.seg = seg; a.B = B; a.in_rows = p->in_rows; a.in_cols = p->in_cols;
+    a.in_rows = p->in_rows; a.in_cols = p->in_cols;
     {
 #pragma clang fp contract(off)
         const double *S = p->M;
@@ -1701,14 +1800,10 @@
     a.ify = 1.0 / ((double)p->occ_h / p->occ_h_px);
     a.ros_layout = p->ros_layout;
     a.variant = p->variant;
-    a.out = out;
-    if (p->laserscan) {
-        int pw, ph;
-        if (!polar_dims(p, pw, ph)) return fail(ctx, BUGSEG_EINVAL, "laserscan grid too large for the polar tables");
-        if (!own_ws && (!ws || ws_bytes < ls_workspace_bytes(B, p, ph)))
-            return fail(ctx, BUGSEG_EINVAL, "laserscan workspace missing or smaller than bugseg_bev_workspace_bytes()");
-    }
-    const bool cap = stream_capturing(stream);
+    return BUGSEG_OK;
+}
+
+int bev_table(bugseg_ctx *ctx, BevArgs &a, bool cap, bugseg_ctx::BevTab *&hit, bool pin = true) {
     {
         std::vector<unsigned char> key(sizeof(double) * 11 + sizeof(int) * 12);
         unsigned char *kp = key.data();
@@ -1717,7 +1812,7 @@
         const int ik[12] = {a.in_rows, a.in_cols, a.bw0, a.warp_w, a.warp_h, a.occ_w_px, a.occ_h_px, a.occ_w, a.occ_h,
                             a.left_x, a.top_y, 0};
         put(ik, sizeof(ik));
-        bugseg_ctx::BevTab *hit = nullptr;
+        hit = nullptr;
         for (auto &t : ctx->bev_tabs) if (t.key == key) hit = &t;
         if (!hit) {
             const size_t cells = (size_t)a.occ_h * a.occ_w;
@@ -1754,6 +1849,13 @@
                     const int b = near_first ? nb - 1 - i : i;
                     for (int k = 0; k < std::max(1, std::min(BEV_BAND, rec[(size_t)b * BEV_BOXREC].x)); ++k) items.push_back(make_int2(b, k));
                 }
+                int lo = 1 << 30, hi = -(1 << 30);
+                for (int b = 0; b < nb; ++b) {
+                    const int4 h = rec[(size_t)b * BEV_BOXREC];
+                    if (h.z <= h.w) { lo = std::min(lo, h.z); hi = std::max(hi, h.w); }
+                }
+                t.row0 = lo <= hi ? std::max(lo, 0) : 0;
+                t.row1 = lo <= hi ? std::min(hi + 1, a.in_rows) : 0;
                 e = hipMemcpyAsync((unsigned char *)t.tab + bev_items_offset(a.occ_w, a.occ_h), items.data(),
                                    items.size() * sizeof(int2), hipMemcpyHostToDevice, s);
             }
@@ -1767,10 +1869,33 @@
             ctx->bev_tabs.push_back(std::move(t));
             hit = &ctx->bev_tabs.back();
         }
-        if (cap) hit->pinned = true;
+        if (cap && pin) hit->pinned = true;
         a.wtab = hit->tab;
         a.nitems = hit->nitems;
     }
+    return BUGSEG_OK;
+}
+
+int bev_occgrid(bugseg_ctx *ctx, const uint8_t *seg, int B, const bugseg_bev_params *p, int8_t *out, bool own_ws,
+                void *ws, size_t ws_bytes, void *stream) {
+    if (!ctx || !seg || !p || !out) return fail(ctx, BUGSEG_EINVAL, "NULL argument");
+    if (B <= 0) return fail(ctx, BUGSEG_EINVAL, "bad BEV geometry");
+    BevArgs a;
+    int rc0 = bev_geometry(ctx, p, a);
+    if (rc0 != BUGSEG_OK) return rc0;
+    DeviceGuard g(ctx->device);
+    a.seg = seg; a.B = B;
+    a.out = out;
+    if (p->laserscan) {
+        int pw, ph;
+        if (!polar_dims(p, pw, ph)) return fail(ctx, BUGSEG_EINVAL, "laserscan grid too large for the polar tables");
+        if (!own_ws && (!ws || ws_bytes < ls_workspace_bytes(B, p, ph)))
+            return fail(ctx, BUGSEG_EINVAL, "laserscan workspace missing or smaller than bugseg_bev_workspace_bytes()");
+    }
+    const bool cap = stream_capturing(stream);
+    bugseg_ctx::BevTab *hit = nullptr;
+    rc0 = bev_table(ctx, a, cap, hit);
+    if (rc0 != BUGSEG_OK) return rc0;
     if (p->laserscan) {
         int rc = prepare_polar(ctx, p, a, cap);
         if (rc != BUGSEG_OK) return rc;
@@ -1792,6 +1917,22 @@
 
 int bugseg_bev_occgrid(bugseg_ctx *ctx, const uint8_t *seg, int B, const bugseg_bev_params *p, int8_t *out, void *stream) {
     return bev_occgrid(ctx, seg, B, p, out, true, nullptr, 0, stream);
+}
+
+int bugseg_bev_source_rows(bugseg_ctx *ctx, const bugseg_bev_params *p, int in_rows, int in_cols, int *row0, int *row1) {
+    if (!ctx || !p || !row0 || !row1) return fail(ctx, BUGSEG_EINVAL, "NULL argument");
+    if (in_rows != p->in_rows || in_cols != p->in_cols)
+        return fail(ctx, BUGSEG_EINVAL, "source rows: the class map is not the size the parameters name");
+    BevArgs a;
+    int rc = bev_geometry(ctx, p, a);
+    if (rc != BUGSEG_OK) return rc;
+    DeviceGuard g(ctx->device);
+    bugseg_ctx::BevTab *hit = nullptr;
+    rc = bev_table(ctx, a, true, hit, false);
+    if (rc != BUGSEG_OK) return rc;
+    *row0 = hit->row0;
+    *row1 = hit->row1;
+    return BUGSEG_OK;
 }
 
 size_t bugseg_bev_workspace_bytes(const bugseg_bev_params *p, int B) {
@@ -1864,6 +2005,28 @@
     return per;
 }
 
+int bugseg_debug_row_windows(int H, int W, int row0, int row1, int tile_rows_c64, int tile_rows_c16, int32_t *win) {
+    (void)W;
+    if (!win) return fail(nullptr, BUGSEG_EINVAL, "NULL argument");
+    if (H <= 0 || H % 8 || W <= 0 || W % 8) return fail(nullptr, BUGSEG_EINVAL, "H and W must be positive multiples of 8");
+    if (row0 < 0 || row1 > H || row0 >= row1) return fail(nullptr, BUGSEG_EINVAL, "row windows: 0 <= row0 < row1 <= H");
+    if (tile_rows_c64 <= 0 || tile_rows_c16 <= 0) return fail(nullptr, BUGSEG_EINVAL, "row windows: tile rows must be positive");
+    int w[WIN_OPS][2];
+    row_windows(H, row0, row1, [&](int k, int, int) { return k == 4 ? tile_rows_c16 : tile_rows_c64; }, w);
+    for (int k = 0; k < WIN_OPS; ++k) { win[2 * k] = w[k][0]; win[2 * k + 1] = w[k][1]; }
+    return BUGSEG_OK;
+}
+
+int bugseg_debug_poison_arena(bugseg_ctx *ctx, int byte, void *stream) {
+    if (!ctx) return fail(ctx, BUGSEG_EINVAL, "NULL ctx");
+    Plan &pl = ctx->plan;
+    if (!pl.arena) return fail(ctx, BUGSEG_ESTATE, "no forward has run");
+    DeviceGuard g(ctx->device);
+    hipError_t e = hipMemsetAsync(pl.arena, byte & 255, pl.act_bytes, (hipStream_t)stream);
+    if (e != hipSuccess) return fail(ctx, BUGSEG_EHIP, std::string("poison arena: ") + hipGetErrorString(e));
+    return BUGSEG_OK;
+}
+
 int bugseg_debug_ctx_info(const bugseg_ctx *ctx, int what, int arg) {
     if (!ctx) return -1;
     switch (what) {
diff --git a/bugcar_image_segmentation_amd/csrc/cls_kernels.hip b/bugcar_image_segmentation_amd/csrc/cls_kernels.hip
--- a/bugcar_image_segmentation_amd/csrc/cls_kernels.hip
+++ b/bugcar_image_segmentation_amd/csrc/cls_kernels.hip
@@ -74,7 +74,8 @@
         }
     }
     const auto rin = mkbuf(a.in, a.in_bytes);
-    const int HWg = a.Hg * a.Wg;
+    const int HWg = a.wrows * a.Wg;
+    const uint32_t wskip = (uint32_t)((a.Hg - a.wrows) * a.Wg), woff = (uint32_t)(a.wy0 * a.Wg);
     const size_t plane = (size_t)a.Hout * a.Wout;
     const int groups = (a.M + 31) >> 5;
     const int xcd = blockIdx.x & 7, nw = (gridDim.x >> 3) * 4, wi = (blockIdx.x >> 3) * 4 + wave;
@@ -95,9 +96,10 @@
         const bool wrap = q.x >= a.Wg;
         q.x = wrap ? q.x - a.Wg : q.x;
         q.y = y0 + (wrap ? 1 : 0);
-        const bool wrapn = q.y >= a.Hg;
-        q.y = wrapn ? 0 : q.y;
+        const bool wrapn = q.y >= a.wrows;
+        q.y = (wrapn ? 0 : q.y) + a.wy0;
         q.n = n0 + (wrapn ? 1 : 0);
+        q.p += (uint32_t)q.n * wskip + woff;
         return q;
     };
     auto load = [&](int g, Raw (&xf)[CLS_TAPS], Px &q) {
@@ -172,7 +174,7 @@
                 }
             }
             if (!done) taps(b, acc, std::false_type());
-            if (LOGITS && q.ok) {
+            if (LOGITS && q.ok && 2 * q.y + b >= a.orow0 && 2 * q.y + b < a.orow1) {
                 float *lo = a.logits_out + (size_t)q.n * a.ncls * plane + (size_t)(2 * q.y + b) * a.Wout + 2 * q.x + h;
 #pragma unroll
                 for (int c = 0; c < 16; ++c)
@@ -190,8 +192,9 @@
             uint32_t c0 = (uint32_t)cls[0], c1 = (uint32_t)cls[1];
             pl32swap(c0, c1);
             const uint32_t o = 4u * q.p - 2u * (uint32_t)q.x + (uint32_t)(2 * h * a.Wg);
+            const bool wr = q.ok && 2 * q.y + h >= a.orow0 && 2 * q.y + h < a.orow1;
             if (!(CLS_ABL & 4) || c0 == 77)
-                __builtin_amdgcn_raw_buffer_store_b16((unsigned short)(c0 | (c1 << 8)), rcls, q.ok ? (int)o : (int)OOB, 0, CLS_AUX);
+                __builtin_amdgcn_raw_buffer_store_b16((unsigned short)(c0 | (c1 << 8)), rcls, wr ? (int)o : (int)OOB, 0, CLS_AUX);
         }
     };
     Raw xa[CLS_TAPS], xb[CLS_TAPS];
diff --git a/bugcar_image_segmentation_amd/csrc/up_kernels.hip b/bugcar_image_segmentation_amd/csrc/up_kernels.hip
--- a/bugcar_image_segmentation_amd/csrc/up_kernels.hip
+++ b/bugcar_image_segmentation_amd/csrc/up_kernels.hip
@@ -81,7 +81,8 @@
     const auto rx = mkbuf(a.x, a.x_bytes);
     const auto ri = mkbuf(a.idx, a.idx_bytes);
     const auto ro = mkbuf(a.out, a.out_bytes);
-    const int hw = a.h * a.w;
+    const int hw = a.hwin * a.w;
+    const int skip = (a.h - a.hwin) * a.w, off0 = a.y0 * a.w;
     const int nfrag = (a.M + 15) >> 4;
     const int gw = blockIdx.x * (NT / 64) + __builtin_amdgcn_readfirstlane(tid >> 6), nw = gridDim.x * (NT / 64);
     constexpr bool F32 = ES == 4;
@@ -110,8 +111,9 @@
     Raw xn[KS1];
     uint32_t idn[NM];
     auto load = [&](int f) {
-        const int p = f * 16 + col;
-        const bool pv = p < a.M;
+        const int pw = f * 16 + col;
+        const bool pv = pw < a.M;
+        const int p = pw + (int)fdiv(pv ? (uint32_t)pw : 0u, a.mHW, a.sHW) * skip + off0;
 #pragma unroll
         for (int s = 0; s < KS1; ++s) bld8(xn[s], rx, pv ? (uint32_t)(p * CIN + s * 32 + kq * 8) * ES : OOB);
 #pragma unroll
@@ -128,7 +130,7 @@
         const int p = f * 16 + col;
         const bool pv = p < a.M;
         const uint32_t pp = pv ? (uint32_t)p : 0u;
-        const int n = (int)fdiv(pp, a.mHW, a.sHW), rr = (int)pp - n * hw;
+        const int n = (int)fdiv(pp, a.mHW, a.sHW), rr = (int)pp - n * hw + off0;
         const int y = (int)fdiv((uint32_t)rr, a.mW, a.sW), x = rr - y * a.w;
 
         Raw xf[KS1];
@@ -174,7 +176,7 @@
             const int po = f * 16 + (col ^ 8);
             pv_o = po < a.M;
             const uint32_t ppo = pv_o ? (uint32_t)po : 0u;
-            const int no = (int)fdiv(ppo, a.mHW, a.sHW), rro = (int)ppo - no * hw;
+            const int no = (int)fdiv(ppo, a.mHW, a.sHW), rro = (int)ppo - no * hw + off0;
             const int yo = (int)fdiv((uint32_t)rro, a.mW, a.sW), xo = rro - yo * a.w;
             obase_o = pv_o ? (uint32_t)((no * 2 * a.h + 2 * yo) * (2 * a.w) + 2 * xo) : 0u;
         }
diff --git a/bugcar_image_segmentation_amd/hostio.py b/bugcar_image_segmentation_amd/hostio.py
--- a/bugcar_image_segmentation_amd/hostio.py
+++ b/bugcar_image_segmentation_amd/hostio.py
@@ -37,7 +37,7 @@
                 for s in range(n):
                     replay, _ = pipe.capture(self._dev_frames[s], out=self._dev_grids[s])
                     self._steps.append(replay)
-                self._keep = (pipe._x, pipe._seg, pipe._grid, dict(getattr(pipe, "_pairs", {})))
+                self._keep = (pipe._x, pipe._seg_raw, pipe._grid, dict(getattr(pipe, "_pairs", {})))
         self._in_done = [torch.cuda.Event() for _ in range(n)]
         self._in_used = [False] * n
         self._step_done = [torch.cuda.Event() for _ in range(n)]
diff --git a/bugcar_image_segmentation_amd/pipeline.py b/bugcar_image_segmentation_amd/pipeline.py
--- a/bugcar_image_segmentation_amd/pipeline.py
+++ b/bugcar_image_segmentation_amd/pipeline.py
@@ -12,7 +12,8 @@
 
     def __init__(self, model: ENET, bev: bev_transform_tools, grid_w_m: float, grid_h_m: float, cell_m: float,
                  model_hw: tuple[int, int] | None = None, ros_layout: bool = False, streams: int = 1,
-                 binary: bool = False, stream_priority: int = 0, chain_forwards: bool = False, shard_offset: int = 0):
+                 binary: bool = False, stream_priority: int = 0, chain_forwards: bool = False, shard_offset: int = 0,
+                 window_rows: bool = True):
         self.model = model
         self.binary = binary
         self.bev = bev
@@ -30,8 +31,12 @@
         self.shard_offset = int(shard_offset)
         self._ctxs = [model.ctx]
         self._streams = []
+        self.window_rows = bool(window_rows)
+        self._windowed = False
+        self._spans = {}
         self._x = None
-        self._seg = None
+        self._seg_raw = None
+        self._seg_partial = None
         self._grid = None
 
     def _shard_ctxs(self, dev: torch.device):
@@ -45,9 +50,21 @@
     def _bufs(self, B: int, dev: torch.device):
         if self._x is None or self._x.shape[0] != B or self._x.device != dev:
             self._x = torch.empty((B, self.H, self.W, 3), dtype=torch.uint8, device=dev)
-            self._seg = torch.empty((B, self.H, self.W), dtype=torch.uint8, device=dev)
+            self._seg_raw = torch.zeros((B, self.H, self.W), dtype=torch.uint8, device=dev)
+            self._seg_partial = None
             self._grid = torch.empty(self._grid_shape(B), dtype=torch.int8, device=dev)
-        return self._x, self._seg, self._grid
+        return self._x, self._seg_raw, self._grid
+
+    @property
+    def _seg(self):
+        part, self._seg_partial = self._seg_partial, None
+        if part is not None:
+            frames, bounds = part
+            st = torch.cuda.current_stream(frames.device)
+            for i in range(len(bounds) - 1):
+                s, e = bounds[i], bounds[i + 1]
+                self._run_forward(self._ctxs[i], frames[s:e], self._x[s:e], self._seg_raw[s:e], st, window=False)
+        return self._seg_raw
 
     def _params(self):
         return self.bev.occupancy_params(*self.grid, ros_layout=self.ros_layout, binary=self.binary)
@@ -69,8 +86,11 @@
         if tuple(out.shape) != tuple(grid.shape) or out.dtype != torch.int8 or not out.is_contiguous():
             raise ValueError(f"out must be a contiguous int8 tensor of shape {tuple(grid.shape)}")
         p = self._params()
+        self._seg_partial = None
         if self.streams == 1 or B < self.streams:
             self._run_shard(self.model.ctx, frames, x, seg, out, p, None)
+            if self._windowed:
+                self._seg_partial = (frames, [0, B])
             return out
         pair = self.binary and bool(p.laserscan)
         ctxs, streams = self._shard_ctxs(frames.device)
@@ -99,6 +119,8 @@
                     self._run_shard(ctxs[i], frames[s:e], x[s:e], seg[s:e], out[s:e], p, st, forward=not split_done)
         for st in streams[: self.streams - 1]:
             main.wait_stream(st)
+        if self._windowed:
+            self._seg_partial = (frames, bounds)
         return out
 
     def _pair_buf(self, i, shape, dev):
@@ -140,19 +162,41 @@
         hit[1].put(f)
         return hit[1].get(copy=True)
 
-    def _run_forward(self, ctx, frames, x, seg, stream, split=0):
+    def _source_rows(self, ctx):
+        if not self.window_rows:
+            return None
+        p = self._params()
+        key = (id(ctx), bytes(p))
+        if key not in self._spans:
+            r0, r1 = ctx.bev_source_rows(p, self.H, self.W)
+            self._spans[key] = None if (r0 <= 0 and r1 >= self.H) or r0 >= r1 else (r0, r1)
+        return self._spans[key]
+
+    def _run_forward(self, ctx, frames, x, seg, stream, split=0, window=True):
         B, H0, W0 = frames.shape[:3]
         if (H0, W0) != (self.H, self.W):
             ctx.preprocess(frames, B, H0, W0, self.H, self.W, N.PRE_BGR_U8, x, stream)
             frames = x
         kind = N.OUT_BINARY_U8 if self.binary else N.OUT_CLASS3_U8
+        rows = self._source_rows(ctx) if window else None
+        if window:
+            self._windowed = rows is not None
+
+        def ops(first, last):
+            if rows is not None:
+                ctx.forward_bgr_rows(frames, B, self.H, self.W, kind, seg, rows, first, last, stream)
+            elif (first, last) == (0, -1):
+                ctx.forward_bgr(frames, B, self.H, self.W, kind, seg, stream)
+            else:
+                ctx.forward_bgr_ops(frames, B, self.H, self.W, kind, seg, first, last, stream)
+
         if split <= 0:
-            ctx.forward_bgr(frames, B, self.H, self.W, kind, seg, stream)
+            ops(0, -1)
             return
-        ctx.forward_bgr_ops(frames, B, self.H, self.W, kind, seg, 0, split, stream)
+        ops(0, split)
         self._split_event = torch.cuda.Event()
         self._split_event.record(stream)
-        ctx.forward_bgr_ops(frames, B, self.H, self.W, kind, seg, split, -1, stream)
+        ops(split, -1)
 
     def _run_shard(self, ctx, frames, x, seg, out, p, stream, forward=True):
         if forward:
diff --git a/include/bugseg.h b/include/bugseg.h
--- a/include/bugseg.h
+++ b/include/bugseg.h
@@ -78,6 +78,12 @@
 int bugseg_enet_forward_bgr_ops(bugseg_ctx *ctx, const uint8_t *bgr_dev, int B, int H, int W, int out_kind,
                                 void *out_dev, int first_op, int last_op, void *stream);
 
+int bugseg_enet_forward_bgr_rows(bugseg_ctx *ctx, const uint8_t *bgr_dev, int B, int H, int W, int out_kind,
+                                 void *out_dev, int row0, int row1, int first_op, int last_op, void *stream);
+
+int bugseg_bev_source_rows(bugseg_ctx *ctx, const bugseg_bev_params *p, int in_rows, int in_cols, int *row0,
+                           int *row1);
+
 int bugseg_bev_occgrid(bugseg_ctx *ctx, const uint8_t *seg_dev, int B, const bugseg_bev_params *p,
                        int8_t *out_dev, void *stream);
 
@@ -98,6 +104,8 @@
 int bugseg_debug_polar_tables(int w, int h, int variant, int32_t *fmap, size_t fmap_n, int32_t *imap, size_t imap_n,
                               int *pw, int *ph);
 int bugseg_debug_tile_walk(int ntiles, int grid, int rev, int32_t *seq, size_t seq_n, int32_t *count);
+int bugseg_debug_row_windows(int H, int W, int row0, int row1, int tile_rows_c64, int tile_rows_c16, int32_t *win);
+int bugseg_debug_poison_arena(bugseg_ctx *ctx, int byte, void *stream);
 int bugseg_debug_ctx_info(const bugseg_ctx *ctx, int what, int arg);
 int bugseg_debug_set_spans(bugseg_ctx *ctx, void *spans, int n_ops);
 int bugseg_debug_pool_indices(bugseg_ctx *ctx, int B, int H, int W, int block, void *dst, size_t bytes, int *idx_cs,
```

After: 22470 frames/s (median of 6 runs). 1.12x the previous value.
